# hyx1999/SAM-Decoding

Measured on AMD Instinct MI355X. Metric: tokens/sec (+ mean accepted tokens), Vicuna-7B bs=1, samd_sam_only draft+verify, higher is better.
Workload: dtype f16

## Files before the change

include/samd_hip.h:

```cpp
#ifndef SAMD_HIP_H
#define SAMD_HIP_H

#include <stdint.h>

#ifdef __cplusplus
extern "C" {
#endif

#define SAMD_OK 0
#define SAMD_E_INVALID (-1)
#define SAMD_E_CAPACITY (-2)
#define SAMD_E_HIP (-3)
#define SAMD_E_IO (-4)
#define SAMD_E_NODEVICE (-5)

#define SAMD_MAX_DRAFT 128
#define SAMD_TOPK 8

#define SAMD_REP_DMETA 0
#define SAMD_REP_VERDICT 16
#define SAMD_REP_TOKENS 24
#define SAMD_REP_KVINDEX 152
#define SAMD_REP_COUNTERS 280
#define SAMD_REP_META 288
// ... 123 lines not shown
int samd_report_wait(const int32_t *h_report, int32_t last_seq, int64_t timeout_us);

int samd_session_report_async(samd_session_t *s, int32_t *h_dst, void *stream);

int samd_session_device_views(samd_session_t *s, void *out[16]);

int samd_tree_buffers(const int32_t *d_parent, int32_t n, int32_t reverse_leaves, int32_t *d_position, uint64_t *d_mask,
                      uint8_t *d_mask_bool, int32_t *d_retrieve, int32_t *d_shape, void *stream);


int samd_argmax_rows(const void *d_logits, int32_t dtype, int32_t rows, int64_t vocab, int64_t row_stride,
                     const int32_t *d_rows, int32_t *d_out, void *stream);

int samd_session_accept(samd_session_t *s, const int32_t *d_node_argmax, void *stream);
int samd_session_candidates(samd_session_t *s, int64_t *d_candidates, int32_t *d_rowmap, int32_t capacity, void *stream);
int samd_session_step_given(samd_session_t *s, const samd_static_t *sam, const samd_params_t *p, const int32_t *d_best_accept,
                            const int32_t *d_next_token, void *stream);
int samd_session_read_verdict(samd_session_t *s, samd_verdict_host_t *out, void *stream);
int samd_session_commit(samd_session_t *s, const samd_static_t *sam, void *stream);
int samd_session_step(samd_session_t *s, const samd_static_t *sam, const samd_params_t *p,
                      const int32_t *d_node_argmax, void *stream);

int samd_posterior_sampled(const void *d_probs, int32_t dtype, const int64_t *d_candidates, int32_t n_candidates, int32_t depth, int64_t vocab,
                           const double *d_uniforms, int32_t n_uniforms, void *d_work, int32_t *d_out, void *stream);
int samd_posterior_sampled_nodes(const void *d_probs, int32_t dtype, const int32_t *d_rowmap, int32_t n_rows, const int64_t *d_candidates,
                                 int32_t n_candidates, int32_t depth, int64_t vocab, const double *d_uniforms, int32_t n_uniforms,
                                 void *d_work, int32_t *d_out, void *stream);
int samd_kv_compact(samd_session_t *s, void *const *d_tensors, int32_t n_tensors, int32_t n_heads, int64_t max_len,
                    int32_t head_dim, int32_t elem_bytes, void *stream);

int samd_kv_compact_indices(void *const *d_tensors, int32_t n_tensors, int32_t n_heads, int64_t max_len, int32_t head_dim,
                            int32_t elem_bytes, int32_t start, const int32_t *d_indices, int32_t accept, void *stream);

int samd_session_set_cache_length(samd_session_t *s, int32_t length, void *stream);
int samd_session_get_cache_length(samd_session_t *s, int32_t *h_out, void *stream);

typedef struct samd_warm {
    const void *d_packed_w;
    int32_t N, K, splits;
    int32_t kb_per_workgroup;
    int32_t delay;
    int32_t where;
} samd_warm_t;

int64_t samd_tree_attention_workspace(int32_t n_q_pad, int32_t n_heads, int32_t head_dim);
int samd_tree_attention(const void *d_q, const void *d_k_cache, const void *d_v_cache, void *d_out, int32_t dtype,
                        int32_t n_q_pad, int32_t n_heads, int32_t n_kv_heads, int32_t head_dim, int64_t max_len,
                        const uint64_t *d_mask, const int32_t *d_cache_length, const int32_t *d_n, float scale,
                        void *d_workspace, int64_t workspace_bytes, void *stream);
int samd_tree_attention_vt(const void *d_q, const void *d_k_cache, const void *d_vt_cache, void *d_out, int32_t dtype,
                           int32_t n_q_pad, int32_t n_heads, int32_t n_kv_heads, int32_t head_dim, int64_t max_len,
                           const uint64_t *d_mask, const int32_t *d_cache_length, const int32_t *d_n, float scale,
                           void *d_workspace, int64_t workspace_bytes, const samd_warm_t *next, void *stream);
int samd_tree_attention_warm(const void *d_q, const void *d_k_cache, const void *d_v_cache, void *d_out, int32_t dtype,
                             int32_t n_q_pad, int32_t n_heads, int32_t n_kv_heads, int32_t head_dim, int64_t max_len,
                             const uint64_t *d_mask, const int32_t *d_cache_length, const int32_t *d_n, float scale,
                             void *d_workspace, int64_t workspace_bytes, const samd_warm_t *next, void *stream);

int samd_rope_rows(const int32_t *d_rel_pos, const int32_t *d_base, const float *d_cos, const float *d_sin, float *d_cs, int32_t rows,
                   int32_t head_dim, int32_t max_pos, void *stream);
int samd_attention_block(const void *d_qkv, int32_t n_partials, int64_t partial_stride, const float *d_cs, void *d_k_cache, void *d_vt_cache,
                         void *d_out, int32_t dtype, int32_t n_q_pad, int32_t n_heads, int32_t n_kv_heads, int32_t head_dim, int64_t max_len,
                         const uint64_t *d_mask, const int32_t *d_write_pos, const int32_t *d_visible_len, const int32_t *d_n, float scale,
                         void *stream);
int samd_rope_kv_write_cs(const void *d_qkv, const int32_t *d_rel_pos, const int32_t *d_cache_length, const int32_t *d_n,
                          const float *d_cs, void *d_q_out, void *d_k_cache, void *d_v_cache, int32_t rows,
                          int32_t n_heads, int32_t n_kv_heads, int32_t head_dim, int64_t max_len, int32_t dtype,
                          int32_t n_partials, int64_t partial_stride, void *stream);
int samd_rope_kv_write_cs_vt(const void *d_qkv, const int32_t *d_rel_pos, const int32_t *d_cache_length, const int32_t *d_n,
                             const float *d_cs, void *d_q_out, void *d_k_cache, void *d_vt_cache, int32_t rows,
                             int32_t n_heads, int32_t n_kv_heads, int32_t head_dim, int64_t max_len, int32_t dtype,
                             int32_t n_partials, int64_t partial_stride, void *stream);
int64_t samd_tree_attention_rope_workspace(int32_t n_q_pad, int32_t n_heads, int32_t head_dim);
int samd_tree_attention_rope(const void *d_qkv, int32_t n_partials, int64_t partial_stride, const float *d_cs, void *d_k_cache, void *d_v_cache,
                             void *d_out, int32_t dtype, int32_t n_q_pad, int32_t n_heads, int32_t n_kv_heads, int32_t head_dim, int64_t max_len,
                             const uint64_t *d_mask, const int32_t *d_cache_length, const int32_t *d_n, float scale, void *d_workspace,
                             int64_t workspace_bytes, void *stream);
int samd_rope_kv_write_vt(const void *d_qkv, const int32_t *d_rel_pos, const int32_t *d_cache_length, const int32_t *d_n,
                          const float *d_cos, const float *d_sin, void *d_q_out, void *d_k_cache, void *d_vt_cache, int32_t rows,
                          int32_t n_heads, int32_t n_kv_heads, int32_t head_dim, int64_t max_len, int32_t max_pos, int32_t dtype,
                          int32_t n_partials, int64_t partial_stride, void *stream);
typedef struct samd_qkv_epilogue {
    const void *d_bias;
    const void *d_q_norm;
    const void *d_k_norm;
    float eps;
} samd_qkv_epilogue_t;
int samd_rope_kv_write_epi(const void *d_qkv, const int32_t *d_rel_pos, const int32_t *d_cache_length, const int32_t *d_n,
                           const float *d_cos, const float *d_sin, const float *d_cs, void *d_q_out, void *d_k_cache, void *d_v_cache,
                           int32_t v_transposed, int32_t rows, int32_t n_heads, int32_t n_kv_heads, int32_t head_dim, int64_t max_len,
                           int32_t max_pos, int32_t dtype, int32_t n_partials, int64_t partial_stride, const samd_qkv_epilogue_t *epi, void *stream);
int samd_kv_compact_vt(samd_session_t *s, void *const *d_tensors, int32_t n_tensors, int32_t n_transposed, int32_t n_heads, int64_t max_len,
                       int32_t head_dim, int32_t elem_bytes, void *stream);
int samd_kv_compact_indices_vt(void *const *d_tensors, int32_t n_tensors, int32_t n_transposed, int32_t n_heads, int64_t max_len, int32_t head_dim,
                               int32_t elem_bytes, int32_t start, const int32_t *d_indices, int32_t accept, void *stream);

typedef struct samd_e2_state {
    float *row_lse; float *top_logp; int32_t *top_idx; float *scores; int32_t *cs_index; float *all_scores; int32_t *all_tokens;
    int32_t *parents_list; uint64_t *mask_rows; int32_t *row_src; int32_t *ids;
    float *rec_top_vals; int32_t *rec_top_idx; float *rec_best_vals; int32_t *rec_best_idx; float *rec_final_vals; int32_t *rec_final_idx;
} samd_e2_state_t;
int64_t samd_e2_rowstats_workspace(int64_t vocab);
int samd_e2_rowstats(const void *d_logits, int32_t dtype, int32_t rows, int64_t vocab, int64_t row_stride, const samd_e2_state_t *st, void *d_workspace,
                     int64_t workspace_bytes, void *stream);
int samd_e2_select(const samd_e2_state_t *st, int32_t level, const void *d_hidden, const void *d_embed, int32_t hidden, int32_t vocab, void *d_fc_in,
                   int32_t *d_rel_pos , int32_t *d_L, int32_t *d_Lw , int32_t *d_n ,
                   int32_t advance_L, int32_t dtype, void *stream);
int samd_e2_stage_extend(const void *d_hidden_rows, const int32_t *d_kv_index, const int32_t *d_acc_tokens, const int32_t *d_start_token, int32_t n_accepted,
                         int32_t n_rows, const void *d_embed, int32_t hidden, int32_t vocab, void *d_fc_in, int32_t *d_rel_pos, uint64_t *d_mask_rows, int32_t *d_n,
                         int64_t *d_sample_token, int32_t dtype, void *stream);
int samd_e2_finish(const samd_e2_state_t *st, int32_t depth, int32_t keep, const int64_t *d_sample_token, int32_t *d_tokens, int32_t *d_parents, void *stream);
int samd_sum_partials_bias(const float *d_part, int32_t n_partials, int64_t partial_stride, const void *d_bias, void *d_out, int32_t rows, int32_t N,
                           int32_t dtype, void *stream);

int samd_embed_rows(const int32_t *d_tokens, const void *d_table, void *d_out, int32_t rows, int32_t hidden, int32_t vocab,
                    int32_t dtype, void *stream);
int samd_rmsnorm(void *d_x, const void *d_delta, const void *d_weight, void *d_out, int32_t rows, int32_t hidden, float eps,
                 int32_t dtype, int32_t n_partials, int64_t partial_stride, void *stream);
int samd_rmsnorm_warm(void *d_x, const void *d_delta, const void *d_weight, void *d_out, int32_t rows, int32_t hidden, float eps,
                      int32_t dtype, int32_t n_partials, int64_t partial_stride, const samd_warm_t *next, void *stream);
int samd_rope_kv_write(const void *d_qkv, const int32_t *d_rel_pos, const int32_t *d_cache_length, const int32_t *d_n,
                       const float *d_cos, const float *d_sin, void *d_q_out, void *d_k_cache, void *d_v_cache, int32_t rows,
                       int32_t n_heads, int32_t n_kv_heads, int32_t head_dim, int64_t max_len, int32_t max_pos, int32_t dtype,
                       int32_t n_partials, int64_t partial_stride, void *stream);
int samd_prefill_attention(const void *d_q, const void *d_k_cache, const void *d_v_cache, void *d_out, int32_t dtype, int32_t rows, int32_t pos0,
                           int32_t n_heads, int32_t n_kv_heads, int32_t head_dim, int64_t max_len, float scale, void *stream);
int samd_prefill_attention_vt(const void *d_q, const void *d_k_cache, const void *d_vt_cache, void *d_out, int32_t dtype, int32_t rows, int32_t pos0,
                              int32_t n_heads, int32_t n_kv_heads, int32_t head_dim, int64_t max_len, float scale, void *stream);
int samd_silu_mul(const void *d_gate_up, void *d_out, int32_t rows, int32_t inter, int32_t dtype, int32_t n_partials,
                  int64_t partial_stride, void *stream);

int samd_gemm_pack_weights(const void *d_W, void *d_packed, int32_t N, int32_t K, void *stream);
int samd_gemm_skinny_silu(const void *d_A, const void *d_W, int32_t rows_pad, int32_t N, int32_t K, void *d_out, int32_t dtype,
                          void *stream);
int samd_gemm_splits(int32_t N, int32_t K, int32_t rows_pad);
int64_t samd_gemm_workspace(int32_t rows_pad, int32_t N, int32_t splits);
int samd_gemm_pack_groups(const void *d_W, void *d_packed, int32_t N, int32_t K, void *stream);
int samd_gemm_pairs_silu(const void *d_A, const void *d_Wg, int32_t rows_pad, int32_t inter, int32_t K, void *d_out, int32_t dtype, void *stream);
int samd_gemm_pack_qkv64(const void *d_W, void *d_packed, int32_t n_heads_total, int32_t K, void *stream);
int samd_embed_rows_ssq_rope(const int32_t *d_tokens, const void *d_table, void *d_out, float *d_ssq, int32_t rows, int32_t hidden, int32_t vocab,
                             int32_t dtype, const int32_t *d_rel_pos, const int32_t *d_base, const float *d_cos, const float *d_sin, float *d_cs,
                             int32_t rope_rows, int32_t head_dim, int32_t max_pos, void *stream);
int samd_embed_rows_ssq(const int32_t *d_tokens, const void *d_table, void *d_out, float *d_ssq, int32_t rows, int32_t hidden, int32_t vocab,
                        int32_t dtype, void *stream);
int samd_gemm_qkv_rope_norm(const void *d_x, const float *d_ssq, const void *d_norm_weight, float eps, const void *d_W64, int32_t rows_pad, int32_t K,
                            const float *d_cs, const int32_t *d_cache_length, const int32_t *d_n, void *d_q_out, void *d_k_cache, void *d_v_cache,
                            int32_t n_heads, int32_t n_kv_heads, int32_t head_dim, int64_t max_len, int32_t dtype, void *stream);
int samd_gemm_pairs_silu_norm(const void *d_x, const float *d_ssq, const void *d_norm_weight, float eps, const void *d_Wg, int32_t rows_pad, int32_t inter,
                              int32_t K, void *d_out, int32_t dtype, void *stream);
int samd_gemm_cs_residual(const void *d_A, const void *d_Wg, int32_t rows_pad, int32_t N, int32_t K, void *d_x, float *d_ssq, int32_t dtype, void *stream);
int samd_gemm_qkv_rope(const void *d_A, const void *d_W64, int32_t rows_pad, int32_t K, const float *d_cs, const int32_t *d_cache_length,
                       const int32_t *d_n, void *d_q_out, void *d_k_cache, void *d_v_cache, int32_t n_heads, int32_t n_kv_heads,
                       int32_t head_dim, int64_t max_len, int32_t dtype, void *stream);
int samd_gemm_qkv_rope_norm_vt(const void *d_x, const float *d_ssq, const void *d_norm_weight, float eps, const void *d_W64, int32_t rows_pad, int32_t K,
                               const float *d_cs, const int32_t *d_cache_length, const int32_t *d_n, void *d_q_out, void *d_k_cache, void *d_vt_cache,
                               int32_t n_heads, int32_t n_kv_heads, int32_t head_dim, int64_t max_len, int32_t dtype, void *stream);
int samd_gemm_qkv_rope_vt(const void *d_A, const void *d_W64, int32_t rows_pad, int32_t K, const float *d_cs, const int32_t *d_cache_length,
                          const int32_t *d_n, void *d_q_out, void *d_k_cache, void *d_vt_cache, int32_t n_heads, int32_t n_kv_heads,
                          int32_t head_dim, int64_t max_len, int32_t dtype, void *stream);
int samd_gemm_skinny(const void *d_A, const void *d_W, int32_t rows_pad, int32_t N, int32_t K, int32_t splits, float *d_partial,
                     void *d_out, int32_t dtype, void *stream);
int samd_gemm_skinny_groups(const void *d_A, const void *d_Wg, int32_t rows_pad, int32_t N, int32_t K, int32_t splits, float *d_partial,
                            void *d_out, int32_t dtype, void *stream);
int samd_gemm_pack_f8(const void *d_W8, void *d_out, int32_t N, int32_t K, void *stream);
int samd_gemm_skinny_f8(const void *d_A, const void *d_W8p, const float *d_scale, int32_t rows_pad, int32_t N, int32_t K, int32_t splits,
                        float *d_partial, void *d_out, int32_t dtype, void *stream);
int samd_gemm_pack_f4(const void *d_q, const void *d_e8, void *d_out, int32_t N, int32_t K, void *stream);
int samd_gemm_skinny_f4(const void *d_A, const void *d_W4p, int32_t rows_pad, int32_t N, int32_t K, int32_t splits, float *d_partial, void *d_out,
                        int32_t dtype, void *stream);
int32_t samd_moe_workspace_layout(int32_t field);
int64_t samd_moe_workspace(int32_t rows_pad, int32_t hidden, int32_t n_experts, int32_t top_k, int32_t dtype);
int samd_moe_pack_experts(const void *d_W, void *d_packed, int32_t n_experts, int32_t N, int32_t K, int32_t gate_up, void *stream);
int samd_moe_route(const void *d_h, const void *d_router, const int32_t *d_n, int32_t rows_pad, int32_t hidden, int32_t n_experts, int32_t top_k,
                   int32_t norm_topk, int32_t *d_topk_idx, void *d_topk_w, void *d_ws, int32_t dtype, void *stream);
int samd_moe_lists(const int32_t *d_topk_idx, const int32_t *d_n, int32_t rows_pad, int32_t n_experts, int32_t top_k, void *d_ws, void *stream);
int samd_moe_gate_up_silu(const void *d_h, const void *d_Wgu, const void *d_ws, int32_t rows_pad, int32_t hidden, int32_t moe_inter, int32_t n_experts,
                          int32_t top_k, void *d_act, int32_t dtype, void *stream);
int samd_moe_down_combine(const void *d_act, const void *d_Wdown, const int32_t *d_topk_idx, const void *d_topk_w, const int32_t *d_n, void *d_ws,
                          int32_t rows_pad, int32_t hidden, int32_t moe_inter, int32_t n_experts, int32_t top_k, void *d_out, int32_t dtype, void *stream);
int samd_moe_gate_up_silu_f4(const void *d_h, const void *d_Wgu4, const void *d_ws, int32_t rows_pad, int32_t hidden, int32_t moe_inter, int32_t n_experts,
                             int32_t top_k, void *d_act, int32_t dtype, void *stream);
int samd_moe_down_combine_f4(const void *d_act, const void *d_Wdown4, const int32_t *d_topk_idx, const void *d_topk_w, const int32_t *d_n, void *d_ws,
                             int32_t rows_pad, int32_t hidden, int32_t moe_inter, int32_t n_experts, int32_t top_k, void *d_out, int32_t dtype, void *stream);

int samd_scripted_argmax(samd_session_t *s, const int32_t *d_target, int32_t n_target, int32_t vocab, int32_t *d_out,
                         void *stream);

int samd_scripted_logits(samd_session_t *s, const int32_t *d_argmax, void *d_logits, int32_t dtype, int32_t rows, int64_t row_stride,
                         int32_t markov_vocab, void *stream);
int samd_scripted_logits_order1(samd_session_t *s, const int32_t *d_argmax, void *d_logits, int32_t dtype, int32_t rows, int64_t row_stride,
                                int32_t hot_vocab, void *stream);

int samd_recycle_create(int32_t vocab, const int32_t *h_child_offsets, const int32_t *h_children, int32_t n_nodes,
                        samd_recycle_t **out);
void samd_recycle_free(samd_recycle_t *t);
int samd_recycle_update(samd_recycle_t *t, const int32_t *d_tokens, const void *d_logits, int32_t dtype, int32_t n,
                        const int32_t *d_n, int64_t vocab, int64_t row_stride, void *stream);
int samd_recycle_draft(samd_recycle_t *t, const int32_t *d_start_token, int32_t *d_out, void *stream);
int samd_recycle_export(samd_recycle_t *t, int32_t *h_table, uint8_t *h_present, void *stream);

#ifdef __cplusplus
}
#endif
#endif
```

sam-decoding_amd/csrc/gemm_kernels.hip:

```cpp
#include <hip/hip_runtime.h>
#include <cstdlib>
#include "samd_common.h"

#define LAUNCHCHK() do { hipError_t e_ = hipGetLastError(); if (e_ != hipSuccess) { samd_set_error("kernel launch: %s", hipGetErrorString(e_)); return SAMD_E_HIP; } } while (0)

static int samd_cu_count() { return samd_device_cus(); }

typedef _Float16 half8 __attribute__((ext_vector_type(8)));
typedef __bf16 bf16x8 __attribute__((ext_vector_type(8)));
typedef float floatx4 __attribute__((ext_vector_type(4)));
typedef unsigned u32x4 __attribute__((ext_vector_type(4)));

struct GF16 { typedef _Float16 elem; typedef half8 vec8;
    static __device__ __forceinline__ floatx4 mfma(half8 a, half8 b, floatx4 c) { return __builtin_amdgcn_mfma_f32_16x16x32_f16(a, b, c, 0, 0, 0); } };
struct GBF16 { typedef __bf16 elem; typedef bf16x8 vec8;
    static __device__ __forceinline__ floatx4 mfma(bf16x8 a, bf16x8 b, floatx4 c) { return __builtin_amdgcn_mfma_f32_16x16x32_bf16(a, b, c, 0, 0, 0); } };

#define GEMM_KC 256
#define GEMM_WAVES 8
#define GEMM_COLS (16 * GEMM_WAVES)

typedef __attribute__((address_space(1))) const void *gptr_t;
typedef __attribute__((address_space(3))) void *lptr_t;

// ... 54 lines not shown
        if (DEPTH > 2 && younger_in_flight >= 2) asm volatile("s_waitcnt vmcnt(%0)" : : "n"(2 * (8 + XV)) : "memory");
        else if (younger_in_flight >= 1) asm volatile("s_waitcnt vmcnt(%0)" : : "n"(8 + XV) : "memory");
        else asm volatile("s_waitcnt vmcnt(0)" : : : "memory");
        __builtin_amdgcn_s_barrier();
        asm volatile("" ::: "memory");
    };
    auto phase = [&](u32x4 (&cur)[4][2], int c, int buf) {
        landed(c1 - 1 - c);
        const uint32_t xbase = lds_base + (uint32_t)buf * (R * GEMM_KC * 2) + (uint32_t)n * (GEMM_KC * 2);
#pragma unroll
        for (int b = 0; b < 4; b++) {
            const uint32_t u0 = (uint32_t)((8 * b + 2 * g) ^ n) * 16, u1 = (uint32_t)((8 * b + 2 * g + 1) ^ n) * 16;
            const uint32_t a0 = xbase + u0, a1 = xbase + u1;
            u32x4 r[RT][2];
            if constexpr (RT == 1)
                asm volatile("ds_read_b128 %0, %2\n\tds_read_b128 %1, %3\n\ts_waitcnt lgkmcnt(0)" : "=&v"(r[0][0]), "=&v"(r[0][1]) : "v"(a0), "v"(a1));
            else if constexpr (RT == 2)
                asm volatile("ds_read_b128 %0, %4\n\tds_read_b128 %1, %5\n\tds_read_b128 %2, %4 offset:8192\n\tds_read_b128 %3, %5 offset:8192\n\t"
                             "s_waitcnt lgkmcnt(0)" : "=&v"(r[0][0]), "=&v"(r[0][1]), "=&v"(r[1][0]), "=&v"(r[1][1]) : "v"(a0), "v"(a1));
            else if constexpr (RT == 3)
                asm volatile("ds_read_b128 %0, %6\n\tds_read_b128 %1, %7\n\tds_read_b128 %2, %6 offset:8192\n\tds_read_b128 %3, %7 offset:8192\n\t"
                             "ds_read_b128 %4, %6 offset:16384\n\tds_read_b128 %5, %7 offset:16384\n\ts_waitcnt lgkmcnt(0)"
                             : "=&v"(r[0][0]), "=&v"(r[0][1]), "=&v"(r[1][0]), "=&v"(r[1][1]), "=&v"(r[2][0]), "=&v"(r[2][1]) : "v"(a0), "v"(a1));
            else
                asm volatile("ds_read_b128 %0, %8\n\tds_read_b128 %1, %9\n\tds_read_b128 %2, %8 offset:8192\n\tds_read_b128 %3, %9 offset:8192\n\t"
                             "ds_read_b128 %4, %8 offset:16384\n\tds_read_b128 %5, %9 offset:16384\n\tds_read_b128 %6, %8 offset:24576\n\t"
                             "ds_read_b128 %7, %9 offset:24576\n\ts_waitcnt lgkmcnt(0)"
                             : "=&v"(r[0][0]), "=&v"(r[0][1]), "=&v"(r[1][0]), "=&v"(r[1][1]), "=&v"(r[2][0]), "=&v"(r[2][1]), "=&v"(r[3][0]), "=&v"(r[3][1])
                             : "v"(a0), "v"(a1));
#pragma unroll
            for (int mt = 0; mt < RT; mt++) {
                acc[mt] = TT::mfma(__builtin_bit_cast(V8, r[mt][0]), __builtin_bit_cast(V8, cur[b][0]), acc[mt]);
                acc[mt] = TT::mfma(__builtin_bit_cast(V8, r[mt][1]), __builtin_bit_cast(V8, cur[b][1]), acc[mt]);
            }
            if (RT >= 3 && c + DEPTH < c1) {
                load_wb(cur, c + DEPTH, b);
                if (b < XV) stage_xi(c + DEPTH, buf == 0 ? NB - 1 : buf - 1, b);
            }
        }
        if (RT < 3 && c + DEPTH < c1) { load_w(cur, c + DEPTH); stage_x(c + DEPTH, buf == 0 ? NB - 1 : buf - 1); }
    };
    if (c0 < c1) {
#pragma unroll
        for (int d = 0; d < DEPTH; d++)
            if (c0 + d < c1) { load_w(wr[d], c0 + d); stage_x(c0 + d, d); }
        int buf = 0;
        for (int c = c0; c < c1; c += DEPTH) {
#pragma unroll
            for (int d = 0; d < DEPTH; d++)
                if (c + d < c1) { phase(wr[d], c + d, buf); buf = buf == NB - 1 ? 0 : buf + 1; }
        }
    }
    if constexpr (EPI == 1) {
        float *ex = reinterpret_cast<float *>(gemm_lds);
        __syncthreads();
        if (w >= 4) {
#pragma unroll
            for (int mt = 0; mt < RT; mt++)
#pragma unroll
                for (int r = 0; r < 4; r++) ex[(16 * mt + 4 * g + r) * 64 + 16 * (w - 4) + n] = acc[mt][r];
        }
        __syncthreads();
        if (w < 4) {
#pragma unroll
            for (int mt = 0; mt < RT; mt++)
#pragma unroll
                for (int r = 0; r < 4; r++) {
                    const int m = 16 * mt + 4 * g + r;
                    const float gf = (float)(E)acc[mt][r], uf = (float)(E)ex[m * 64 + 16 * w + n];
                    const E sv = (E)(gf / (1.f + __expf(-gf)));
                    out[(size_t)m * (N / 2) + blockIdx.x * 64 + 16 * w + n] = (E)((float)sv * uf);
                }
        }
        return;
    }
#pragma unroll
    for (int mt = 0; mt < RT; mt++) {
#pragma unroll
        for (int r = 0; r < 4; r++) {
            const int m = 16 * mt + 4 * g + r;
            if (out) out[(size_t)m * N + n0 + n] = (E)acc[mt][r];
            else __hip_atomic_store(&partial[((size_t)split * R + m) * N + n0 + n], acc[mt][r], __ATOMIC_RELAXED, __HIP_MEMORY_SCOPE_AGENT);
        }
    }
}

struct NormArgs { const float *ssq; const void *g; int tiles; float inv_hidden; float eps; };

#define NORM_NS 16
template <int NT>
__device__ __forceinline__ void norm_issue(const NormArgs &na, float (&sv)[NORM_NS]) {
    const int tid = threadIdx.x, row = tid & 15, p = tid >> 4;
#pragma unroll
    for (int k = 0; k < NORM_NS; k++) {
        sv[k] = 0.f;
        if ((NT / 16) * k >= na.tiles) continue;
        int t = p + (NT / 16) * k;
        t = t < na.tiles ? t : na.tiles - 1;
        const float *src = na.ssq + (size_t)t * 16 + row;
        asm volatile("global_load_dword %0, %1, off" : "=v"(sv[k]) : "v"(src) : "memory");
    }
}
template <int NT>
__device__ __forceinline__ void norm_finish(const NormArgs &na, float (&sv)[NORM_NS], float *part , float *rs ) {
    const int tid = threadIdx.x, row = tid & 15, p = tid >> 4;
    static_assert(NORM_NS == 16, "");
    asm volatile("" : "+v"(sv[0]), "+v"(sv[1]), "+v"(sv[2]), "+v"(sv[3]), "+v"(sv[4]), "+v"(sv[5]), "+v"(sv[6]), "+v"(sv[7]),
                      "+v"(sv[8]), "+v"(sv[9]), "+v"(sv[10]), "+v"(sv[11]), "+v"(sv[12]), "+v"(sv[13]), "+v"(sv[14]), "+v"(sv[15]) : : "memory");
    float s = 0.f;
#pragma unroll
    for (int k = 0; k < NORM_NS; k++) s += (p + (NT / 16) * k < na.tiles) ? sv[k] : 0.f;
    part[p * 16 + row] = s;
    asm volatile("s_waitcnt lgkmcnt(0)" ::: "memory");
    __builtin_amdgcn_s_barrier();
    asm volatile("" ::: "memory");
    if (tid < 16) {
        float tot = 0.f;
        for (int k = 0; k < NT / 16; k++) tot += part[k * 16 + tid];
        rs[tid] = rsqrtf(tot * na.inv_hidden + na.eps);
    }
    asm volatile("s_waitcnt lgkmcnt(0)" ::: "memory");
    __builtin_amdgcn_s_barrier();
    asm volatile("" ::: "memory");
}

template <typename E>
__device__ __forceinline__ u32x4 norm_scale8(u32x4 xraw, u32x4 graw, float rs) {
    const E *xe = reinterpret_cast<const E *>(&xraw);
    const E *ge = reinterpret_cast<const E *>(&graw);
    u32x4 out;
    E *oe = reinterpret_cast<E *>(&out);
#pragma unroll
    for (int j = 0; j < 8; j++) { const E h = (E)((float)xe[j] * rs); oe[j] = (E)((float)ge[j] * (float)h); }
    return out;
}


template <int DEPTH, int PC>
__device__ __forceinline__ void gemm_wait_younger(int younger) {
    if constexpr (PC == 0) asm volatile("s_waitcnt vmcnt(0)" : : : "memory");
    else {
        if (DEPTH > 3 && younger >= 3) asm volatile("s_waitcnt vmcnt(%0)" : : "n"(3 * PC) : "memory");
        else if (DEPTH > 2 && younger >= 2) asm volatile("s_waitcnt vmcnt(%0)" : : "n"(2 * PC) : "memory");
        else if (younger >= 1) asm volatile("s_waitcnt vmcnt(%0)" : : "n"(PC) : "memory");
        else asm volatile("s_waitcnt vmcnt(0)" : : : "memory");
    }
}

template <typename TT, int RT, int DEPTH, int CG, bool NORM, int AR = 16>
__global__ __launch_bounds__(64 * GEMM_WAVES, RT >= 3 || NORM ? 2 : GEMM_WAVES / 2) void k_gemm_qkv_rope(
        const typename TT::elem *__restrict__ A, const typename TT::elem *__restrict__ W, int K, int n_chunks,
        const float *__restrict__ cs, const int *__restrict__ d_L, const int *__restrict__ d_n,
        typename TT::elem *__restrict__ q_out, typename TT::elem *__restrict__ k_cache, typename TT::elem *__restrict__ v_cache,
        int H, int Hkv, long long max_len, NormArgs na, int v_t) {
    typedef typename TT::elem E;
    typedef typename TT::vec8 V8;
    constexpr int R = 16 * RT;
    constexpr int NT = 64 * GEMM_WAVES;
    constexpr int XV = (R * 32) / NT;
    constexpr int NB = DEPTH + 1;
    constexpr int WL = 4;
    constexpr int TW = 16 * CG, PP = 8 * CG;
    constexpr int CH = CG * 8192;
    extern __shared__ __attribute__((aligned(1024))) char gemm_lds[];
    E (*xs)[R][GEMM_KC] = reinterpret_cast<E (*)[R][GEMM_KC]>(gemm_lds);

    const int tid = threadIdx.x, w = tid >> 6, l = tid & 63, n = l & 15, g = l >> 4;
    const bool streams = CG == 4 || w < 2 * CG;
    static_assert(AR == 16 || (AR == 8 && NORM && RT == 1), "8 activation rows: the norm-fold kernels only");
    const bool stager = AR == 16 || w < GEMM_WAVES / 2;
    const int cg = CG == 4 ? (w & 3) : (streams ? w % CG : 0), kh = CG == 4 ? (w >> 2) : (streams ? w / CG : 0);
    const char *wtile = reinterpret_cast<const char *>(W) + (size_t)blockIdx.x * n_chunks * CH;
    const uint32_t wlane = (uint32_t)(64 * (CG * kh + cg) + l) * 16;
    const uint32_t lds_base = (uint32_t)(uintptr_t)(lptr_t)&xs[0][0][0];
    const int n_rows = d_n[0], L = d_L[0];

    floatx4 acc[RT];
#pragma unroll
    for (int mt = 0; mt < RT; mt++) acc[mt] = (floatx4){0.f, 0.f, 0.f, 0.f};

    u32x4 wr[DEPTH][2][2];
    auto load_wb = [&](u32x4 (&dst)[2][2], int c, int bl) {
        const char *p = wtile + (size_t)c * CH;
#pragma unroll
        for (int j = 0; j < 2; j++)
            asm volatile("global_load_dwordx4 %0, %1, %2 nt" : "=v"(dst[bl][j]) : "v"(wlane), "s"(p + (CH / 4) * (2 * bl + j)) : "memory");
    };
    static_assert(!NORM || RT == 1, "the norm-fold path is built for the 16-row tile");
    constexpr int XL = NORM ? 2 * XV : XV;
    u32x4 xr[NORM ? DEPTH : 1][NORM ? XV : 1], gr[NORM ? DEPTH : 1][NORM ? XV : 1];
    __shared__ float norm_part[NORM ? (NT / 16) * 16 : 1], norm_rs[NORM ? 16 : 1];
    auto stage_xi = [&](int c, int buf, int i, int d) {
        const int slot = tid + NT * i, row = slot >> 5, pos = slot & 31, unit = pos ^ (row & 15);
        const E *src = A + (size_t)row * K + (size_t)c * GEMM_KC + 8 * unit;
        if constexpr (NORM) {
            const E *gsrc = reinterpret_cast<const E *>(na.g) + (size_t)c * GEMM_KC + 8 * unit;
            asm volatile("global_load_dwordx4 %0, %1, off" : "=v"(xr[d][i]) : "v"(src) : "memory");
            asm volatile("global_load_dwordx4 %0, %1, off" : "=v"(gr[d][i]) : "v"(gsrc) : "memory");
        } else {
            E *dst = &xs[buf][0][0] + (size_t)(NT * i + 64 * w) * 8;
            __builtin_amdgcn_global_load_lds((gptr_t)src, (lptr_t)dst, 16, 0, 0);
            asm volatile("" ::: "memory");
        }
    };
    auto issue = [&](u32x4 (&dst)[2][2], int c, int buf, int d) {
        if (streams) { load_wb(dst, c, 0); load_wb(dst, c, 1); }
        if (stager) {
#pragma unroll
            for (int i = 0; i < XV; i++) stage_xi(c, buf, i, d);
        }
    };
    auto scale_to_lds = [&](int buf, int d) {
        if constexpr (NORM) {
            if (!stager) return;
#pragma unroll
            for (int i = 0; i < XV; i++) {
                const int slot = tid + NT * i, row = slot >> 5;
                asm volatile("" : "+v"(xr[d][i]), "+v"(gr[d][i]) : : "memory");
                const u32x4 v = norm_scale8<E>(xr[d][i], gr[d][i], norm_rs[row]);
                *reinterpret_cast<u32x4 *>(&xs[buf][0][0] + (size_t)slot * 8) = v;
            }
        }
    };
    auto landed = [&](int younger, int buf, int d) {
        if (streams) { if (stager) gemm_wait_younger<DEPTH, WL + XL>(younger); else gemm_wait_younger<DEPTH, WL>(younger); }
        else { if (stager) gemm_wait_younger<DEPTH, XL>(younger); else gemm_wait_younger<DEPTH, 0>(younger); }
        if constexpr (NORM) { scale_to_lds(buf, d); asm volatile("s_waitcnt lgkmcnt(0)" ::: "memory"); }
        __builtin_amdgcn_s_barrier();
        asm volatile("" ::: "memory");
    };
    auto phase = [&](u32x4 (&cur)[2][2], int c, int buf, int d) {
        landed(n_chunks - 1 - c, buf, d);
        const uint32_t xbase = lds_base + (uint32_t)buf * (R * GEMM_KC * 2) + (uint32_t)n * (GEMM_KC * 2);
#pragma unroll
        for (int bl = 0; bl < 2; bl++) {
            if (!streams) break;
            const int b = 2 * kh + bl;
            const uint32_t a0 = xbase + (uint32_t)((8 * b + 2 * g) ^ n) * 16, a1 = xbase + (uint32_t)((8 * b + 2 * g + 1) ^ n) * 16;
            u32x4 r[RT][2];
            if constexpr (RT == 1)
                asm volatile("ds_read_b128 %0, %2\n\tds_read_b128 %1, %3\n\ts_waitcnt lgkmcnt(0)" : "=&v"(r[0][0]), "=&v"(r[0][1]) : "v"(a0), "v"(a1));
            else if constexpr (RT == 2)
                asm volatile("ds_read_b128 %0, %4\n\tds_read_b128 %1, %5\n\tds_read_b128 %2, %4 offset:8192\n\tds_read_b128 %3, %5 offset:8192\n\t"
                             "s_waitcnt lgkmcnt(0)" : "=&v"(r[0][0]), "=&v"(r[0][1]), "=&v"(r[1][0]), "=&v"(r[1][1]) : "v"(a0), "v"(a1));
            else if constexpr (RT == 3)
                asm volatile("ds_read_b128 %0, %6\n\tds_read_b128 %1, %7\n\tds_read_b128 %2, %6 offset:8192\n\tds_read_b128 %3, %7 offset:8192\n\t"
                             "ds_read_b128 %4, %6 offset:16384\n\tds_read_b128 %5, %7 offset:16384\n\ts_waitcnt lgkmcnt(0)"
                             : "=&v"(r[0][0]), "=&v"(r[0][1]), "=&v"(r[1][0]), "=&v"(r[1][1]), "=&v"(r[2][0]), "=&v"(r[2][1]) : "v"(a0), "v"(a1));
            else
                asm volatile("ds_read_b128 %0, %8\n\tds_read_b128 %1, %9\n\tds_read_b128 %2, %8 offset:8192\n\tds_read_b128 %3, %9 offset:8192\n\t"
                             "ds_read_b128 %4, %8 offset:16384\n\tds_read_b128 %5, %9 offset:16384\n\tds_read_b128 %6, %8 offset:24576\n\t"
                             "ds_read_b128 %7, %9 offset:24576\n\ts_waitcnt lgkmcnt(0)"
                             : "=&v"(r[0][0]), "=&v"(r[0][1]), "=&v"(r[1][0]), "=&v"(r[1][1]), "=&v"(r[2][0]), "=&v"(r[2][1]), "=&v"(r[3][0]), "=&v"(r[3][1])
                             : "v"(a0), "v"(a1));
#pragma unroll
            for (int mt = 0; mt < RT; mt++) {
                acc[mt] = TT::mfma(__builtin_bit_cast(V8, r[mt][0]), __builtin_bit_cast(V8, cur[bl][0]), acc[mt]);
                acc[mt] = TT::mfma(__builtin_bit_cast(V8, r[mt][1]), __builtin_bit_cast(V8, cur[bl][1]), acc[mt]);
            }
        }
        if (c + DEPTH < n_chunks) issue(cur, c + DEPTH, buf == 0 ? NB - 1 : buf - 1, d);
    };
    float norm_sv[NORM ? NORM_NS : 1];
    if constexpr (NORM) norm_issue<NT>(na, norm_sv);
#pragma unroll
    for (int d = 0; d < DEPTH; d++)
        if (d < n_chunks) issue(wr[d], d, d, d);
    if constexpr (AR == 8) {
        if (!stager) {
#pragma unroll
            for (int bz = 0; bz < NB; bz++) *reinterpret_cast<u32x4 *>(&xs[bz][0][0] + (size_t)tid * 8) = (u32x4){0u, 0u, 0u, 0u};
        }
    }
    if constexpr (NORM) {
        if (n_chunks >= DEPTH) {
            if (streams) { if (stager) asm volatile("s_waitcnt vmcnt(%0)" : : "n"(DEPTH * (WL + XL)) : "memory"); else asm volatile("s_waitcnt vmcnt(%0)" : : "n"(DEPTH * WL) : "memory"); }
            else { if (stager) asm volatile("s_waitcnt vmcnt(%0)" : : "n"(DEPTH * XL) : "memory"); else asm volatile("s_waitcnt vmcnt(0)" : : : "memory"); }
        } else asm volatile("s_waitcnt vmcnt(0)" : : : "memory");
        norm_finish<NT>(na, norm_sv, norm_part, norm_rs);
    }
    {
        int buf = 0;
        for (int c = 0; c < n_chunks; c += DEPTH) {
#pragma unroll
            for (int d = 0; d < DEPTH; d++)
                if (c + d < n_chunks) { phase(wr[d], c + d, buf, d); buf = buf == NB - 1 ? 0 : buf + 1; }
        }
    }
    float *ex = reinterpret_cast<float *>(gemm_lds);
    __syncthreads();
    if (streams) {
#pragma unroll
        for (int mt = 0; mt < RT; mt++)
#pragma unroll
            for (int r = 0; r < 4; r++) ex[(kh * R + 16 * mt + 4 * g + r) * TW + 16 * cg + n] = acc[mt][r];
    }
    __syncthreads();
    const bool vt_tile = v_t && ((PP * (int)blockIdx.x) >> 6) >= H + Hkv;
    for (int i = tid; i < R * PP; i += NT) {
        const int row = vt_tile ? i % R : i / PP, p = vt_tile ? i / R : i % PP;
        if (row >= n_rows || L + row >= max_len) continue;
        const float x1 = (float)(E)(ex[row * TW + p] + ex[(R + row) * TW + p]);
        const float x2 = (float)(E)(ex[row * TW + PP + p] + ex[(R + row) * TW + PP + p]);
        const int pair = PP * (int)blockIdx.x + p, head = pair >> 6, j = pair & 63;
        if (head >= H + Hkv) {
            if (v_t) {
                E *dst = v_cache + (size_t)(head - H - Hkv) * max_len * 128 + L + row;
                dst[(size_t)j * max_len] = (E)x1; dst[(size_t)(j + 64) * max_len] = (E)x2;
                continue;
            }
            E *dst = v_cache + ((size_t)(head - H - Hkv) * max_len + L + row) * 128;
            dst[j] = (E)x1; dst[j + 64] = (E)x2;
            continue;
        }
        const float c = cs[(size_t)row * 128 + j], sn = cs[(size_t)row * 128 + 64 + j];
        const E o1 = (E)(x1 * c - x2 * sn), o2 = (E)(x2 * c + x1 * sn);
        E *dst = head < H ? q_out + ((size_t)row * H + head) * 128 : k_cache + ((size_t)(head - H) * max_len + L + row) * 128;
        dst[j] = o1; dst[j + 64] = o2;
    }
}

template <int CG>
__global__ __launch_bounds__(256) void k_gemm_pack_qkv(const uint4 *__restrict__ W, uint4 *__restrict__ out, int N, int K) {
    const long long u = (long long)blockIdx.x * 256 + threadIdx.x;
    const long long total = (long long)N * K / 8;
    if (u >= total) return;
    constexpr int PP = 8 * CG;
    const int n_chunks = K / GEMM_KC;
    const long long blk = u / (512 * CG);
    const int in = (int)(u % (512 * CG)), jj = in / (128 * CG), x = in % (128 * CG), w = x >> 6, g = (x >> 4) & 3, n = x & 15, cg = w % CG, kh = w / CG;
    const int t = (int)(blk / n_chunks), c = (int)(blk % n_chunks), bl = jj >> 1, j = jj & 1;
    const int q = 16 * cg + n, pair = PP * t + (q < PP ? q : q - PP);
    const long long row = 128LL * (pair >> 6) + (pair & 63) + (q < PP ? 0 : 64), col = 256LL * c + 64 * (2 * kh + bl) + 16 * g + 8 * j;
    out[u] = W[(row * K + col) / 8];
}

static int qkv_tile_groups(int n_heads_total) {
    static const int env = [] { const char *e = getenv("SAMD_QKV_TILE"); return e ? atoi(e) : 0; }();
    const int n_cu = samd_cu_count();
    const int N = n_heads_total * 128;
    if (N % 48 != 0 || env == 64) return 4;
    if (env == 48) return 3;
    const int t48 = N / 48, t64 = N / 64;
    return ((t48 + n_cu - 1) / n_cu) * 48 < ((t64 + n_cu - 1) / n_cu) * 64 ? 3 : 4;
}

template <typename TT, int RT, int DEPTH, bool NORM, int AR = 16>
__global__ __launch_bounds__(64 * GEMM_WAVES, RT >= 3 || DEPTH > 2 ? 2 : GEMM_WAVES / 2) void k_gemm_pairs_silu(const typename TT::elem *__restrict__ A, const typename TT::elem *__restrict__ W,
                                                                                                     typename TT::elem *__restrict__ out, int K, int inter, int n_chunks, int n_pairs, NormArgs na) {
    typedef typename TT::elem E;
    typedef typename TT::vec8 V8;
    constexpr int R = 16 * RT;
    constexpr int NT = 64 * GEMM_WAVES;
    constexpr int XV = (R * 32) / NT;
    constexpr int NB = DEPTH + 1;
    extern __shared__ __attribute__((aligned(1024))) char gemm_lds[];
    E (*xs)[R][GEMM_KC] = reinterpret_cast<E (*)[R][GEMM_KC]>(gemm_lds);

    const int tid = threadIdx.x, w = __builtin_amdgcn_readfirstlane(tid >> 6), l = tid & 63, n = l & 15, g = l >> 4;
#ifdef SAMD_GEMM_ABLATE
    const int abl = samd_abl_flag;
#else
    constexpr int abl = 0;
#endif
    const int p0 = (int)((long long)blockIdx.x * n_pairs / gridDim.x), p1 = (int)((long long)(blockIdx.x + 1) * n_pairs / gridDim.x);
    const bool active = w < 2 * (p1 - p0);
    static_assert(AR == 16 || (AR == 8 && NORM && RT == 1), "8 activation rows: the norm-fold kernels only");
    const bool stager = AR == 16 || w < GEMM_WAVES / 2;
    const int gi = 2 * p0 + w;
    const char *wgrp = reinterpret_cast<const char *>(W) + (size_t)(active ? gi : 0) * n_chunks * 8192;
    const uint32_t wlane = (uint32_t)l * 16;
    const uint32_t lds_base = (uint32_t)(uintptr_t)(lptr_t)&xs[0][0][0];

    floatx4 acc[RT];
#pragma unroll
    for (int mt = 0; mt < RT; mt++) acc[mt] = (floatx4){0.f, 0.f, 0.f, 0.f};
    u32x4 wr[DEPTH][4][2];
    auto load_w = [&](u32x4 (&dst)[4][2], int c) {
        const char *p = wgrp + (size_t)c * 8192;
#pragma unroll
        for (int b = 0; b < 4; b++)
#pragma unroll
            for (int j = 0; j < 2; j++)
                asm volatile("global_load_dwordx4 %0, %1, %2 nt" : "=v"(dst[b][j]) : "v"(wlane), "s"(p + 1024 * (2 * b + j)) : "memory");
    };
    static_assert(!NORM || RT == 1, "the norm-fold path is built for the 16-row tile");
    constexpr int XL = NORM ? 2 * XV : XV;
    u32x4 xr[NORM ? DEPTH : 1][NORM ? XV : 1], gr[NORM ? DEPTH : 1][NORM ? XV : 1];
    __shared__ float norm_part[NORM ? (NT / 16) * 16 : 1], norm_rs[NORM ? 16 : 1];
    auto stage_x = [&](int c, int buf, int d) {
        if (!stager || (abl & 4)) return;
#pragma unroll
        for (int i = 0; i < XV; i++) {
            const int slot = tid + NT * i, row = slot >> 5, pos = slot & 31, unit = pos ^ (row & 15);
            const E *src = A + (size_t)((abl & 8) ? (row & 15) : row) * K + (size_t)c * GEMM_KC + 8 * unit;
            if constexpr (NORM) {
                const E *gsrc = reinterpret_cast<const E *>(na.g) + (size_t)c * GEMM_KC + 8 * unit;
                asm volatile("global_load_dwordx4 %0, %1, off" : "=v"(xr[d][i]) : "v"(src) : "memory");
                asm volatile("global_load_dwordx4 %0, %1, off" : "=v"(gr[d][i]) : "v"(gsrc) : "memory");
            } else {
                E *dst = &xs[buf][0][0] + (size_t)(NT * i + 64 * w) * 8;
                __builtin_amdgcn_global_load_lds((gptr_t)src, (lptr_t)dst, 16, 0, 0);
                asm volatile("" ::: "memory");
            }
        }
    };
    auto landed = [&](int younger, int buf, int d) {
        const bool stg = stager && !(abl & 4);
        if (active) { if (stg) gemm_wait_younger<DEPTH, 8 + XL>(younger); else gemm_wait_younger<DEPTH, 8>(younger); }
        else { if (stg) gemm_wait_younger<DEPTH, XL>(younger); else gemm_wait_younger<DEPTH, 0>(younger); }
        if constexpr (NORM) {
            if (stager) {
#pragma unroll
                for (int i = 0; i < XV; i++) {
                    const int slot = tid + NT * i, row = slot >> 5;
                    asm volatile("" : "+v"(xr[d][i]), "+v"(gr[d][i]) : : "memory");
                    const u32x4 v = norm_scale8<E>(xr[d][i], gr[d][i], norm_rs[row]);
                    *reinterpret_cast<u32x4 *>(&xs[buf][0][0] + (size_t)slot * 8) = v;
                }
            }
            asm volatile("s_waitcnt lgkmcnt(0)" ::: "memory");
        }
        if (!(abl & 1)) __builtin_amdgcn_s_barrier();
        asm volatile("" ::: "memory");
    };
    auto phase = [&](u32x4 (&cur)[4][2], int c, int buf, int d) {
        landed(n_chunks - 1 - c, buf, d);
        if (active && !(abl & 2)) {
            const uint32_t xbase = lds_base + (uint32_t)buf * (R * GEMM_KC * 2) + (uint32_t)n * (GEMM_KC * 2);
#pragma unroll
            for (int b = 0; b < 4; b++) {
                const uint32_t a0 = xbase + (uint32_t)((8 * b + 2 * g) ^ n) * 16, a1 = xbase + (uint32_t)((8 * b + 2 * g + 1) ^ n) * 16;
                u32x4 r[RT][2];
                if constexpr (RT == 1)
                    asm volatile("ds_read_b128 %0, %2\n\tds_read_b128 %1, %3\n\ts_waitcnt lgkmcnt(0)" : "=&v"(r[0][0]), "=&v"(r[0][1]) : "v"(a0), "v"(a1));
                else if constexpr (RT == 2)
                    asm volatile("ds_read_b128 %0, %4\n\tds_read_b128 %1, %5\n\tds_read_b128 %2, %4 offset:8192\n\tds_read_b128 %3, %5 offset:8192\n\t"
                                 "s_waitcnt lgkmcnt(0)" : "=&v"(r[0][0]), "=&v"(r[0][1]), "=&v"(r[1][0]), "=&v"(r[1][1]) : "v"(a0), "v"(a1));
                else if constexpr (RT == 3)
                    asm volatile("ds_read_b128 %0, %6\n\tds_read_b128 %1, %7\n\tds_read_b128 %2, %6 offset:8192\n\tds_read_b128 %3, %7 offset:8192\n\t"
                                 "ds_read_b128 %4, %6 offset:16384\n\tds_read_b128 %5, %7 offset:16384\n\ts_waitcnt lgkmcnt(0)"
                                 : "=&v"(r[0][0]), "=&v"(r[0][1]), "=&v"(r[1][0]), "=&v"(r[1][1]), "=&v"(r[2][0]), "=&v"(r[2][1]) : "v"(a0), "v"(a1));
                else
                    asm volatile("ds_read_b128 %0, %8\n\tds_read_b128 %1, %9\n\tds_read_b128 %2, %8 offset:8192\n\tds_read_b128 %3, %9 offset:8192\n\t"
                                 "ds_read_b128 %4, %8 offset:16384\n\tds_read_b128 %5, %9 offset:16384\n\tds_read_b128 %6, %8 offset:24576\n\t"
                                 "ds_read_b128 %7, %9 offset:24576\n\ts_waitcnt lgkmcnt(0)"
                                 : "=&v"(r[0][0]), "=&v"(r[0][1]), "=&v"(r[1][0]), "=&v"(r[1][1]), "=&v"(r[2][0]), "=&v"(r[2][1]), "=&v"(r[3][0]), "=&v"(r[3][1])
                                 : "v"(a0), "v"(a1));
#pragma unroll
                for (int mt = 0; mt < RT; mt++) {
                    acc[mt] = TT::mfma(__builtin_bit_cast(V8, r[mt][0]), __builtin_bit_cast(V8, cur[b][0]), acc[mt]);
                    acc[mt] = TT::mfma(__builtin_bit_cast(V8, r[mt][1]), __builtin_bit_cast(V8, cur[b][1]), acc[mt]);
                }
            }
        }
        if (c + DEPTH < n_chunks) { if (active) load_w(cur, c + DEPTH); stage_x(c + DEPTH, buf == 0 ? NB - 1 : buf - 1, d); }
    };
    float norm_sv[NORM ? NORM_NS : 1];
    if constexpr (NORM) norm_issue<NT>(na, norm_sv);
#pragma unroll
    for (int d = 0; d < DEPTH; d++)
        if (d < n_chunks) { if (active) load_w(wr[d], d); stage_x(d, d, d); }
    if constexpr (AR == 8) {
        if (!stager) {
#pragma unroll
            for (int bz = 0; bz < NB; bz++) *reinterpret_cast<u32x4 *>(&xs[bz][0][0] + (size_t)tid * 8) = (u32x4){0u, 0u, 0u, 0u};
        }
    }
    if constexpr (NORM) {
        if (n_chunks >= DEPTH) {
            if (active) { if (stager) asm volatile("s_waitcnt vmcnt(%0)" : : "n"(DEPTH * (8 + XL)) : "memory"); else asm volatile("s_waitcnt vmcnt(%0)" : : "n"(DEPTH * 8) : "memory"); }
            else { if (stager) asm volatile("s_waitcnt vmcnt(%0)" : : "n"(DEPTH * XL) : "memory"); else asm volatile("s_waitcnt vmcnt(0)" : : : "memory"); }
        } else asm volatile("s_waitcnt vmcnt(0)" : : : "memory");
        norm_finish<NT>(na, norm_sv, norm_part, norm_rs);
    }
    {
        int buf = 0;
        for (int c = 0; c < n_chunks; c += DEPTH) {
#pragma unroll
            for (int d = 0; d < DEPTH; d++)
                if (c + d < n_chunks) { phase(wr[d], c + d, buf, d); buf = buf == NB - 1 ? 0 : buf + 1; }
        }
    }
    float *ex = reinterpret_cast<float *>(gemm_lds);
    __syncthreads();
    if (active && (w & 1)) {
#pragma unroll
        for (int mt = 0; mt < RT; mt++)
#pragma unroll
            for (int r = 0; r < 4; r++) ex[((w >> 1) * R + 16 * mt + 4 * g + r) * 16 + n] = acc[mt][r];
    }
    __syncthreads();
    if (active && !(w & 1)) {
        const int col = 16 * (p0 + (w >> 1)) + n;
#pragma unroll
        for (int mt = 0; mt < RT; mt++)
#pragma unroll
            for (int r = 0; r < 4; r++) {
                const int m = 16 * mt + 4 * g + r;
                const float gf = (float)(E)acc[mt][r], uf = (float)(E)ex[((w >> 1) * R + m) * 16 + n];
                const E sv = (E)(gf / (1.f + __expf(-gf)));
                out[(size_t)m * inter + col] = (E)((float)sv * uf);
            }
    }
}

template <typename TT, int ROWS, bool EARLY = false>
__global__ __launch_bounds__(64 * GEMM_WAVES, 2) void k_gemm_cs_residual(const typename TT::elem *__restrict__ A, const typename TT::elem *__restrict__ W,
                                                                           typename TT::elem *__restrict__ x, float *__restrict__ ssq, int K, int N, int n_chunks,
                                                                           const int *__restrict__ counter = nullptr, int *__restrict__ epoch = nullptr,
                                                                           int arrivals = 0) {
    typedef typename TT::elem E;
    typedef typename TT::vec8 V8;
    constexpr int CSD = 2;
    extern __shared__ __attribute__((aligned(1024))) char gemm_lds[];
    const int tid = threadIdx.x, w = __builtin_amdgcn_readfirstlane(tid >> 6), l = tid & 63, n = l & 15, g = l >> 4;
    E *xs = reinterpret_cast<E *>(gemm_lds) + (size_t)w * CSD * 16 * GEMM_KC;
    const uint32_t lds_base = (uint32_t)(uintptr_t)(lptr_t)xs;
    const char *wgrp = reinterpret_cast<const char *>(W) + (size_t)blockIdx.x * n_chunks * 8192;
    const uint32_t wlane = (uint32_t)l * 16;

    static_assert(ROWS == 8 || ROWS == 16, "");
    constexpr int AL = ROWS / 2;
    if constexpr (ROWS == 8) {
#pragma unroll
        for (int buf = 0; buf < CSD; buf++)
#pragma unroll
            for (int i = 4; i < 8; i++)
                *reinterpret_cast<u32x4 *>(xs + (size_t)buf * 16 * GEMM_KC + (size_t)(64 * i + l) * 8) = (u32x4){0u, 0u, 0u, 0u};
        asm volatile("s_waitcnt lgkmcnt(0)" ::: "memory");
    }
    floatx4 acc = (floatx4){0.f, 0.f, 0.f, 0.f};
    u32x4 wr[CSD][4][2];
    auto issue_w = [&](u32x4 (&dst)[4][2], int c) {
        const char *p = wgrp + (size_t)c * 8192;
#pragma unroll
        for (int b = 0; b < 4; b++)
#pragma unroll
            for (int j = 0; j < 2; j++)
                asm volatile("global_load_dwordx4 %0, %1, %2 nt" : "=v"(dst[b][j]) : "v"(wlane), "s"(p + 1024 * (2 * b + j)) : "memory");
    };
    auto issue_a = [&](int c, int buf) {
#pragma unroll
        for (int i = 0; i < AL; i++) {
            const int slot = l + 64 * i, row = slot >> 5, pos = slot & 31, unit = pos ^ (row & 15);
            const E *src = A + (size_t)row * K + (size_t)c * GEMM_KC + 8 * unit;
            E *dst_l = xs + (size_t)buf * 16 * GEMM_KC + (size_t)(64 * i) * 8;
            __builtin_amdgcn_global_load_lds((gptr_t)src, (lptr_t)dst_l, 16, 0, 0);
            asm volatile("" ::: "memory");
        }
    };
    auto issue = [&](u32x4 (&dst)[4][2], int c, int buf) { issue_w(dst, c); issue_a(c, buf); };
    auto phase = [&](u32x4 (&cur)[4][2], int c, int buf, bool more) {
        if (more) { if constexpr (EARLY) asm volatile("s_waitcnt vmcnt(%0)" : : "n"(AL) : "memory"); else asm volatile("s_waitcnt vmcnt(%0)" : : "n"(8 + AL) : "memory"); }
        else asm volatile("s_waitcnt vmcnt(0)" ::: "memory");
        const uint32_t xbase = lds_base + (uint32_t)buf * (16 * GEMM_KC * 2) + (uint32_t)n * (GEMM_KC * 2);
#pragma unroll
        for (int b = 0; b < 4; b++) {
            const uint32_t a0 = xbase + (uint32_t)((8 * b + 2 * g) ^ n) * 16, a1 = xbase + (uint32_t)((8 * b + 2 * g + 1) ^ n) * 16;
            u32x4 r0, r1;
            asm volatile("ds_read_b128 %0, %2\n\tds_read_b128 %1, %3\n\ts_waitcnt lgkmcnt(0)" : "=&v"(r0), "=&v"(r1) : "v"(a0), "v"(a1));
            acc = TT::mfma(__builtin_bit_cast(V8, r0), __builtin_bit_cast(V8, cur[b][0]), acc);
            acc = TT::mfma(__builtin_bit_cast(V8, r1), __builtin_bit_cast(V8, cur[b][1]), acc);
        }
    };
    const int mine = (n_chunks - w + GEMM_WAVES - 1) / GEMM_WAVES;
    if constexpr (EARLY) {
        if (mine > 0) issue_w(wr[0], w);
        if (mine > 1) issue_w(wr[1], w + GEMM_WAVES);
        __shared__ int my_epoch;
        if (tid == 0) {
            const int e = epoch[blockIdx.x];
            const int target = (e + 1) * arrivals;
            for (int spin = 0; spin < (1 << 22); spin++) {
                if (__hip_atomic_load(counter, __ATOMIC_RELAXED, __HIP_MEMORY_SCOPE_AGENT) >= target) break;
                __builtin_amdgcn_s_sleep(4);
            }
            my_epoch = e;
        }
        __syncthreads();
        __builtin_amdgcn_fence(__ATOMIC_ACQUIRE, "agent");
        if (mine > 0) issue_a(w, 0);
        if (mine > 1) issue_a(w + GEMM_WAVES, 1);
        if (mine > 0) phase(wr[0], w, 0, mine > 1);
        if (mine > 1) phase(wr[1], w + GEMM_WAVES, 1, false);
        if (tid == 0) epoch[blockIdx.x] = my_epoch + 1;
    } else {
        if (mine > 0) issue(wr[0], w, 0);
        if (mine > 1) issue(wr[1], w + GEMM_WAVES, 1);
        for (int i = 0; i < mine; i += 2) {
            phase(wr[0], w + GEMM_WAVES * i, 0, i + 1 < mine);
            if (i + 2 < mine) issue(wr[0], w + GEMM_WAVES * (i + 2), 0);
            if (i + 1 < mine) {
                phase(wr[1], w + GEMM_WAVES * (i + 1), 1, i + 2 < mine);
                if (i + 3 < mine) issue(wr[1], w + GEMM_WAVES * (i + 3), 1);
            }
        }
    }
    __syncthreads();
    float *ex = reinterpret_cast<float *>(gemm_lds);
#pragma unroll
    for (int r = 0; r < 4; r++) ex[(w * 16 + 4 * g + r) * 16 + n] = acc[r];
    __syncthreads();
    if (tid < 16 * ROWS) {
        const int row = tid >> 4, col = tid & 15;
        float sum = 0.f;
#pragma unroll
        for (int k = 0; k < GEMM_WAVES; k++) sum += ex[(k * 16 + row) * 16 + col];
        E *xp = x + (size_t)row * N + 16 * blockIdx.x + col;
        const E o = (E)sum;
        const E y = (E)((float)*xp + (float)o);
        *xp = y;
        float q = (float)y * (float)y;
        q += __shfl_xor(q, 1); q += __shfl_xor(q, 2); q += __shfl_xor(q, 4); q += __shfl_xor(q, 8);
        if (col == 0) ssq[(size_t)blockIdx.x * 16 + row] = q;
    }
}

__global__ __launch_bounds__(256) void k_gemm_pack_groups(const uint4 *__restrict__ W, uint4 *__restrict__ out, int N, int K) {
    const long long u = (long long)blockIdx.x * 256 + threadIdx.x;
    const long long total = (long long)N * K / 8;
    if (u >= total) return;
    const int n_chunks = K / GEMM_KC;
    const long long blk = u >> 9;
    const int in = (int)(u & 511), jj = in >> 6, lane = in & 63, g = lane >> 4, n = lane & 15, b = jj >> 1, j = jj & 1;
    const long long gi = blk / n_chunks; const int c = (int)(blk % n_chunks);
    const long long row = 16 * gi + n, col = 256LL * c + 64 * b + 16 * g + 8 * j;
    out[u] = W[(row * K + col) / 8];
}

__global__ __launch_bounds__(256) void k_gemm_pack(const uint4 *__restrict__ W, uint4 *__restrict__ out, int N, int K) {
    const long long u = (long long)blockIdx.x * 256 + threadIdx.x;
    const long long total = (long long)N * K / 8;
    if (u >= total) return;
    const int n_chunks = K / GEMM_KC;
    const long long blk = u >> 12;
    const int in = (int)(u & 4095), jj = in >> 9, tid = in & 511, w = tid >> 6, g = (tid >> 4) & 3, n = tid & 15;
    const int t = (int)(blk / n_chunks), c = (int)(blk % n_chunks), b = jj >> 1, j = jj & 1;
    const long long row = 128LL * t + 16 * w + n, col = 256LL * c + 64 * b + 16 * g + 8 * j;
    out[u] = W[(row * K + col) / 8];
}

template <typename TT, int RT, int EPI, int DEPTH, bool GM = false>
static hipError_t gemm_launch(dim3 grid, hipStream_t st, const void *A, const void *W, float *partial, void *out, int K, int N, int chunks, int splits) {
    constexpr int lds = (DEPTH + 1) * 16 * RT * GEMM_KC * 2;
    if constexpr (lds > 65536) {
        static unsigned long long done = 0ull;
        const hipError_t attr = samd_reserve_lds((const void *)k_gemm_skinny<TT, RT, EPI, DEPTH, GM>, lds, &done);
        if (attr != hipSuccess) return attr;
    }
    hipLaunchKernelGGL((k_gemm_skinny<TT, RT, EPI, DEPTH, GM>), grid, dim3(64 * GEMM_WAVES), lds, st, (const typename TT::elem *)A, (const typename TT::elem *)W, partial,
                       (typename TT::elem *)out, K, N, chunks, splits);
    return hipSuccess;
}

template <int EPI, bool GM = false>
static hipError_t gemm_dispatch(int dtype, int rows_pad, dim3 grid, hipStream_t st, const void *A, const void *W, float *partial, void *out, int K, int N, int chunks,
                                int splits) {
#define GO(TT, RT, D) return gemm_launch<TT, RT, EPI, D, GM>(grid, st, A, W, partial, out, K, N, chunks, splits)
#define ROWS(TT) do { if (rows_pad == 16) GO(TT, 1, 2); else if (rows_pad == 32) GO(TT, 2, 2); else if (rows_pad == 48) GO(TT, 3, 2); else GO(TT, 4, 2); } while (0)
    if (dtype == SAMD_F16) ROWS(GF16); else ROWS(GBF16);
#undef ROWS
#undef GO
}

template <typename TT, int RT, int DEPTH, int CG, bool NORM = false, int AR = 16>
static hipError_t qkv_rope_launch(hipStream_t st, const void *A, const void *W, int K, int tiles, const float *cs, const int *d_L, const int *d_n, void *q, void *k, void *v,
                                  int H, int Hkv, long long max_len, int v_t, NormArgs na = NormArgs{nullptr, nullptr, 0, 0.f, 0.f}) {
    constexpr int lds_a = (DEPTH + 1) * 16 * RT * GEMM_KC * 2, lds_e = 2 * 16 * RT * 16 * CG * 4, lds = lds_a > lds_e ? lds_a : lds_e;
    if constexpr (lds > 60000) {
        static unsigned long long done = 0ull;
        const hipError_t attr = samd_reserve_lds((const void *)k_gemm_qkv_rope<TT, RT, DEPTH, CG, NORM, AR>, lds + 4096, &done);
        if (attr != hipSuccess) return attr;
    }
    hipLaunchKernelGGL((k_gemm_qkv_rope<TT, RT, DEPTH, CG, NORM, AR>), dim3(tiles), dim3(64 * GEMM_WAVES), lds, st, (const typename TT::elem *)A, (const typename TT::elem *)W, K, K / GEMM_KC,
                       cs, d_L, d_n, (typename TT::elem *)q, (typename TT::elem *)k, (typename TT::elem *)v, H, Hkv, max_len, na, v_t);
    return hipSuccess;
}

template <typename TT, int RT, int DEPTH, bool NORM = false, int AR = 16>
static hipError_t pairs_silu_launch(hipStream_t st, int grid, const void *A, const void *W, void *out, int K, int inter, int n_pairs,
                                    NormArgs na = NormArgs{nullptr, nullptr, 0, 0.f, 0.f}) {
    constexpr int lds_a = (DEPTH + 1) * 16 * RT * GEMM_KC * 2, lds_e = 4 * 16 * RT * 16 * 4, lds = lds_a > lds_e ? lds_a : lds_e;
    if constexpr (lds > 60000) {
        static unsigned long long done = 0ull;
        const hipError_t attr = samd_reserve_lds((const void *)k_gemm_pairs_silu<TT, RT, DEPTH, NORM, AR>, lds + 4096, &done);
        if (attr != hipSuccess) return attr;
    }
    hipLaunchKernelGGL((k_gemm_pairs_silu<TT, RT, DEPTH, NORM, AR>), dim3(grid), dim3(64 * GEMM_WAVES), lds, st, (const typename TT::elem *)A, (const typename TT::elem *)W,
                       (typename TT::elem *)out, K, inter, K / GEMM_KC, n_pairs, na);
    return hipSuccess;
}

extern "C" {

int samd_gemm_splits(int32_t N, int32_t K, int32_t rows_pad) {
    static const int env_cap = [] { const char *e = getenv("SAMD_GEMM_SPLIT_CAP"); const int v = e ? atoi(e) : 8; return v < 1 ? 1 : (v > 8 ? 8 : v); }();
    static const int env_fixed = [] { const char *e = getenv("SAMD_GEMM_SPLITS"); const int v = e ? atoi(e) : 0; return v < 0 ? 0 : (v > 8 ? 8 : v); }();
    const int cols = N / GEMM_COLS, chunks = K / GEMM_KC;
    (void)rows_pad;
    if (env_fixed) return env_fixed > chunks ? (chunks < 1 ? 1 : chunks) : env_fixed;
    int s = 256 / (cols > 0 ? cols : 1);
    if (s > env_cap) s = env_cap;
    if (s > chunks) s = chunks;
    return s < 1 ? 1 : s;
}

int64_t samd_gemm_workspace(int32_t rows_pad, int32_t N, int32_t splits) { return (int64_t)splits * rows_pad * N * 4; }

int samd_gemm_skinny_silu(const void *d_A, const void *d_W, int32_t rows_pad, int32_t N, int32_t K, void *d_out, int32_t dtype, void *stream) {
    if (!d_A || !d_W || !d_out || (rows_pad != 16 && rows_pad != 32 && rows_pad != 48 && rows_pad != 64) || N < GEMM_COLS || N % GEMM_COLS != 0 || K < GEMM_KC ||
        K % GEMM_KC != 0 || (dtype != SAMD_F16 && dtype != SAMD_BF16)) {
        samd_set_error("samd_gemm_skinny_silu: unsupported shape (rows 16/32/48/64, N %% 128 == 0, K %% 256 == 0) or null pointer"); return SAMD_E_INVALID;
    }
    const hipError_t e = gemm_dispatch<1>(dtype, rows_pad, dim3(N / GEMM_COLS, 1), (hipStream_t)stream, d_A, d_W, nullptr, d_out, K, N, K / GEMM_KC, 1);
    if (e != hipSuccess) { samd_set_error("samd_gemm_skinny_silu: %s", hipGetErrorString(e)); return SAMD_E_HIP; }
    LAUNCHCHK();
    return SAMD_OK;
}

int samd_gemm_pack_weights(const void *d_W, void *d_packed, int32_t N, int32_t K, void *stream) {
    if (!d_W || !d_packed || d_W == d_packed || N < GEMM_COLS || N % GEMM_COLS != 0 || K < GEMM_KC || K % GEMM_KC != 0) {
        samd_set_error("samd_gemm_pack_weights: needs N %% 128 == 0, K %% 256 == 0 and distinct buffers"); return SAMD_E_INVALID;
    }
    const long long units = (long long)N * K / 8;
    hipLaunchKernelGGL(k_gemm_pack, dim3((unsigned)((units + 255) / 256)), dim3(256), 0, (hipStream_t)stream, (const uint4 *)d_W, (uint4 *)d_packed, N, K);
    LAUNCHCHK();
    return SAMD_OK;
}

int samd_gemm_pack_groups(const void *d_W, void *d_packed, int32_t N, int32_t K, void *stream) {
    if (!d_W || !d_packed || d_W == d_packed || N < 16 || N % 16 != 0 || K < GEMM_KC || K % GEMM_KC != 0) {
        samd_set_error("samd_gemm_pack_groups: needs N %% 16 == 0, K %% 256 == 0 and distinct buffers"); return SAMD_E_INVALID;
    }
    const long long units = (long long)N * K / 8;
    hipLaunchKernelGGL(k_gemm_pack_groups, dim3((unsigned)((units + 255) / 256)), dim3(256), 0, (hipStream_t)stream, (const uint4 *)d_W, (uint4 *)d_packed, N, K);
    LAUNCHCHK();
    return SAMD_OK;
}

int samd_gemm_pairs_silu_norm(const void *d_x, const float *d_ssq, const void *d_norm_weight, float eps, const void *d_Wg, int32_t rows_pad, int32_t inter, int32_t K,
                              void *d_out, int32_t dtype, void *stream) {
    if (!d_x || !d_ssq || !d_norm_weight || !d_Wg || !d_out || (rows_pad != 16 && rows_pad != 8) || inter < 16 || inter % 16 != 0 || K < GEMM_KC || K % GEMM_KC != 0 ||
        K / 16 > 32 * NORM_NS || (dtype != SAMD_F16 && dtype != SAMD_BF16)) {
        samd_set_error("samd_gemm_pairs_silu_norm: unsupported shape (8 or 16 rows, inter %% 16 == 0, K %% 256 == 0, K <= 8192, f16/bf16) or null pointer"); return SAMD_E_INVALID;
    }
    const int n_cu = samd_cu_count();
    const int n_pairs = inter / 16;
    int grid = n_pairs < n_cu ? n_pairs : n_cu;
    while ((n_pairs + grid - 1) / grid > 4) grid += n_cu;
    const NormArgs na{d_ssq, d_norm_weight, K / 16, 1.f / (float)K, eps};
    hipStream_t st = (hipStream_t)stream;
    const hipError_t e = rows_pad == 8
        ? (dtype == SAMD_F16 ? pairs_silu_launch<GF16, 1, 3, true, 8>(st, grid, d_x, d_Wg, d_out, K, inter, n_pairs, na)
                             : pairs_silu_launch<GBF16, 1, 3, true, 8>(st, grid, d_x, d_Wg, d_out, K, inter, n_pairs, na))
        : (dtype == SAMD_F16 ? pairs_silu_launch<GF16, 1, 3, true>(st, grid, d_x, d_Wg, d_out, K, inter, n_pairs, na)
                             : pairs_silu_launch<GBF16, 1, 3, true>(st, grid, d_x, d_Wg, d_out, K, inter, n_pairs, na));
    if (e != hipSuccess) { samd_set_error("samd_gemm_pairs_silu_norm: %s", hipGetErrorString(e)); return SAMD_E_HIP; }
    LAUNCHCHK();
    return SAMD_OK;
}

int samd_gemm_cs_residual(const void *d_A, const void *d_Wg, int32_t rows_pad, int32_t N, int32_t K, void *d_x, float *d_ssq, int32_t dtype, void *stream) {
    if (!d_A || !d_Wg || !d_x || !d_ssq || (rows_pad != 16 && rows_pad != 8) || N < 16 || N % 16 != 0 || K < GEMM_KC || K % GEMM_KC != 0 || (dtype != SAMD_F16 && dtype != SAMD_BF16)) {
        samd_set_error("samd_gemm_cs_residual: unsupported shape (8 or 16 rows, N %% 16 == 0, K %% 256 == 0, f16/bf16) or null pointer"); return SAMD_E_INVALID;
    }
    constexpr int lds = GEMM_WAVES * 2 * 16 * GEMM_KC * 2;
    hipStream_t st = (hipStream_t)stream;
    hipError_t e = hipSuccess;
#define GO(TT, ROWS, ET) do { static unsigned long long done = 0ull; \
        e = samd_reserve_lds((const void *)k_gemm_cs_residual<TT, ROWS>, lds, &done); \
        if (e == hipSuccess) hipLaunchKernelGGL((k_gemm_cs_residual<TT, ROWS>), dim3(N / 16), dim3(64 * GEMM_WAVES), lds, st, (const ET *)d_A, (const ET *)d_Wg, (ET *)d_x, d_ssq, K, N, K / GEMM_KC, (const int *)nullptr, (int *)nullptr, 0); } while (0)
    if (dtype == SAMD_F16) { if (rows_pad == 8) GO(GF16, 8, _Float16); else GO(GF16, 16, _Float16); }
    else { if (rows_pad == 8) GO(GBF16, 8, __bf16); else GO(GBF16, 16, __bf16); }
#undef GO
    if (e != hipSuccess) { samd_set_error("samd_gemm_cs_residual: %s", hipGetErrorString(e)); return SAMD_E_HIP; }
    LAUNCHCHK();
    return SAMD_OK;
}

int samd_gemm_cs_residual_early(const void *d_A, const void *d_Wg, int32_t N, int32_t K, void *d_x, float *d_ssq, int32_t dtype, const int32_t *d_counter,
                                int32_t *d_epoch, int32_t arrivals, void *stream) {
    if (!d_A || !d_Wg || !d_x || !d_ssq || !d_counter || !d_epoch || arrivals < 1 || N < 16 || N % 16 != 0 || K != 2 * GEMM_WAVES * GEMM_KC ||
        (dtype != SAMD_F16 && dtype != SAMD_BF16)) {
        samd_set_error("samd_gemm_cs_residual_early: unsupported shape (K must be 4096, N %% 16 == 0, f16/bf16) or null pointer"); return SAMD_E_INVALID;
    }
    constexpr int lds = GEMM_WAVES * 2 * 16 * GEMM_KC * 2;
    hipStream_t st = (hipStream_t)stream;
    hipError_t e = hipSuccess;
    if (dtype == SAMD_F16) {
        static unsigned long long done = 0ull;
        e = samd_reserve_lds((const void *)k_gemm_cs_residual<GF16, 8, true>, lds, &done);
        if (e == hipSuccess) hipLaunchKernelGGL((k_gemm_cs_residual<GF16, 8, true>), dim3(N / 16), dim3(64 * GEMM_WAVES), lds, st, (const _Float16 *)d_A, (const _Float16 *)d_Wg,
                                                (_Float16 *)d_x, d_ssq, K, N, K / GEMM_KC, d_counter, d_epoch, arrivals);
    } else {
        static unsigned long long done = 0ull;
        e = samd_reserve_lds((const void *)k_gemm_cs_residual<GBF16, 8, true>, lds, &done);
        if (e == hipSuccess) hipLaunchKernelGGL((k_gemm_cs_residual<GBF16, 8, true>), dim3(N / 16), dim3(64 * GEMM_WAVES), lds, st, (const __bf16 *)d_A, (const __bf16 *)d_Wg,
                                                (__bf16 *)d_x, d_ssq, K, N, K / GEMM_KC, d_counter, d_epoch, arrivals);
    }
    if (e != hipSuccess) { samd_set_error("samd_gemm_cs_residual_early: %s", hipGetErrorString(e)); return SAMD_E_HIP; }
    LAUNCHCHK();
    return SAMD_OK;
}

int samd_gemm_pairs_silu(const void *d_A, const void *d_Wg, int32_t rows_pad, int32_t inter, int32_t K, void *d_out, int32_t dtype, void *stream) {
    if (!d_A || !d_Wg || !d_out || (rows_pad != 16 && rows_pad != 32 && rows_pad != 48 && rows_pad != 64) || inter < 16 || inter % 16 != 0 || K < GEMM_KC ||
        K % GEMM_KC != 0 || (dtype != SAMD_F16 && dtype != SAMD_BF16)) {
        samd_set_error("samd_gemm_pairs_silu: unsupported shape (rows 16/32/48/64, inter %% 16 == 0, K %% 256 == 0, f16/bf16) or null pointer"); return SAMD_E_INVALID;
    }
    const int n_cu = samd_cu_count();
    const int n_pairs = inter / 16;
    int grid = n_pairs < n_cu ? n_pairs : n_cu;
    while ((n_pairs + grid - 1) / grid > 4) grid += n_cu;
    hipStream_t st = (hipStream_t)stream;
    hipError_t e;
    static const int depth_env = [] { const char *e = getenv("SAMD_PAIRS_DEPTH"); return e ? atoi(e) : 0; }();
#ifdef SAMD_GEMM_ABLATE
    static const int abl_set = [] { const char *e = getenv("SAMD_GEMM_ABL"); const int v = e ? atoi(e) : 0; return hipMemcpyToSymbol(HIP_SYMBOL(samd_abl_flag), &v, 4) == hipSuccess ? 1 : -1; }();
    (void)abl_set;
#endif
#define ARGS st, grid, d_A, d_Wg, d_out, K, inter, n_pairs
#define GO(TT) (rows_pad == 16 ? (depth_env == 2 ? pairs_silu_launch<TT, 1, 2>(ARGS) : depth_env == 4 ? pairs_silu_launch<TT, 1, 4>(ARGS) : pairs_silu_launch<TT, 1, 3>(ARGS)) \
                : rows_pad == 32 ? (depth_env == 2 ? pairs_silu_launch<TT, 2, 2>(ARGS) : pairs_silu_launch<TT, 2, 3>(ARGS)) \
                : rows_pad == 48 ? pairs_silu_launch<TT, 3, 2>(ARGS) : pairs_silu_launch<TT, 4, 2>(ARGS))
    e = dtype == SAMD_F16 ? GO(GF16) : GO(GBF16);
#undef GO
#undef ARGS
    if (e != hipSuccess) { samd_set_error("samd_gemm_pairs_silu: %s", hipGetErrorString(e)); return SAMD_E_HIP; }
    LAUNCHCHK();
    return SAMD_OK;
}

int samd_gemm_pack_qkv64(const void *d_W, void *d_packed, int32_t n_heads_total, int32_t K, void *stream) {
    if (!d_W || !d_packed || d_W == d_packed || n_heads_total < 1 || K < GEMM_KC || K % GEMM_KC != 0) {
        samd_set_error("samd_gemm_pack_qkv64: needs K %% 256 == 0, whole 128-column heads and distinct buffers"); return SAMD_E_INVALID;
    }
    const long long units = (long long)n_heads_total * 128 * K / 8;
    if (qkv_tile_groups(n_heads_total) == 3)
        hipLaunchKernelGGL(k_gemm_pack_qkv<3>, dim3((unsigned)((units + 255) / 256)), dim3(256), 0, (hipStream_t)stream, (const uint4 *)d_W, (uint4 *)d_packed, n_heads_total * 128, K);
    else
        hipLaunchKernelGGL(k_gemm_pack_qkv<4>, dim3((unsigned)((units + 255) / 256)), dim3(256), 0, (hipStream_t)stream, (const uint4 *)d_W, (uint4 *)d_packed, n_heads_total * 128, K);
    LAUNCHCHK();
    return SAMD_OK;
}

static int gemm_qkv_rope_impl(const void *d_A, const void *d_W64, int32_t rows_pad, int32_t K, const float *d_cs, const int32_t *d_cache_length, const int32_t *d_n,
                              void *d_q_out, void *d_k_cache, void *d_v_cache, int32_t n_heads, int32_t n_kv_heads, int32_t head_dim, int64_t max_len,
                              int32_t dtype, void *stream, int v_t) {
    if (!d_A || !d_W64 || !d_cs || !d_cache_length || !d_n || !d_q_out || !d_k_cache || !d_v_cache || head_dim != 128 || n_heads < 1 || n_kv_heads < 1 ||
        (rows_pad != 16 && rows_pad != 32 && rows_pad != 48 && rows_pad != 64) || K < GEMM_KC || K % GEMM_KC != 0 || (dtype != SAMD_F16 && dtype != SAMD_BF16)) {
        samd_set_error("samd_gemm_qkv_rope: unsupported shape (rows 16/32/48/64, head_dim 128, K %% 256 == 0, f16/bf16) or null pointer"); return SAMD_E_INVALID;
    }
    static const int depth_env = [] { const char *e = getenv("SAMD_QKV_DEPTH"); return e ? atoi(e) : 0; }();
    const int groups = qkv_tile_groups(n_heads + 2 * n_kv_heads);
    const int tiles = (n_heads + 2 * n_kv_heads) * 128 / (16 * groups);
    hipStream_t st = (hipStream_t)stream;
    hipError_t e = hipSuccess;
#define GO(TT, RT, D, CG) e = qkv_rope_launch<TT, RT, D, CG>(st, d_A, d_W64, K, tiles, d_cs, d_cache_length, d_n, d_q_out, d_k_cache, d_v_cache, n_heads, n_kv_heads, (long long)max_len, v_t)
#define ROWS(TT, CG) do { if (rows_pad == 16) { if (depth_env == 2) GO(TT, 1, 2, CG); else if (depth_env == 3) GO(TT, 1, 3, CG); else GO(TT, 1, 4, CG); } \
                          else if (rows_pad == 32) { if (depth_env == 2) GO(TT, 2, 2, CG); else GO(TT, 2, 4, CG); } \
                          else if (rows_pad == 48) GO(TT, 3, 3, CG); else GO(TT, 4, 3, CG); } while (0)
    if (groups == 3) { if (dtype == SAMD_F16) ROWS(GF16, 3); else ROWS(GBF16, 3); }
    else { if (dtype == SAMD_F16) ROWS(GF16, 4); else ROWS(GBF16, 4); }
#undef ROWS
#undef GO
    if (e != hipSuccess) { samd_set_error("samd_gemm_qkv_rope: %s", hipGetErrorString(e)); return SAMD_E_HIP; }
    LAUNCHCHK();
    return SAMD_OK;
}

int samd_gemm_qkv_rope(const void *d_A, const void *d_W64, int32_t rows_pad, int32_t K, const float *d_cs, const int32_t *d_cache_length, const int32_t *d_n,
                       void *d_q_out, void *d_k_cache, void *d_v_cache, int32_t n_heads, int32_t n_kv_heads, int32_t head_dim, int64_t max_len,
                       int32_t dtype, void *stream) {
    return gemm_qkv_rope_impl(d_A, d_W64, rows_pad, K, d_cs, d_cache_length, d_n, d_q_out, d_k_cache, d_v_cache, n_heads, n_kv_heads, head_dim, max_len, dtype, stream, 0);
}

int samd_gemm_qkv_rope_vt(const void *d_A, const void *d_W64, int32_t rows_pad, int32_t K, const float *d_cs, const int32_t *d_cache_length, const int32_t *d_n,
                          void *d_q_out, void *d_k_cache, void *d_vt_cache, int32_t n_heads, int32_t n_kv_heads, int32_t head_dim, int64_t max_len,
                          int32_t dtype, void *stream) {
    return gemm_qkv_rope_impl(d_A, d_W64, rows_pad, K, d_cs, d_cache_length, d_n, d_q_out, d_k_cache, d_vt_cache, n_heads, n_kv_heads, head_dim, max_len, dtype, stream, 1);
}

static int gemm_qkv_rope_norm_impl(const void *d_x, const float *d_ssq, const void *d_norm_weight, float eps, const void *d_W64, int32_t rows_pad, int32_t K,
                                   const float *d_cs, const int32_t *d_cache_length, const int32_t *d_n, void *d_q_out, void *d_k_cache, void *d_v_cache,
                                   int32_t n_heads, int32_t n_kv_heads, int32_t head_dim, int64_t max_len, int32_t dtype, void *stream, int v_t) {
    if (!d_x || !d_ssq || !d_norm_weight || !d_W64 || !d_cs || !d_cache_length || !d_n || !d_q_out || !d_k_cache || !d_v_cache || head_dim != 128 || n_heads < 1 ||
        n_kv_heads < 1 || (rows_pad != 16 && rows_pad != 8) || K < GEMM_KC || K % GEMM_KC != 0 || K / 16 > 32 * NORM_NS || (dtype != SAMD_F16 && dtype != SAMD_BF16)) {
        samd_set_error("samd_gemm_qkv_rope_norm: unsupported shape (8 or 16 rows, head_dim 128, K %% 256 == 0, K <= 8192, f16/bf16) or null pointer"); return SAMD_E_INVALID;
    }
    const int groups = qkv_tile_groups(n_heads + 2 * n_kv_heads);
    const int tiles = (n_heads + 2 * n_kv_heads) * 128 / (16 * groups);
    const NormArgs na{d_ssq, d_norm_weight, K / 16, 1.f / (float)K, eps};
    hipStream_t st = (hipStream_t)stream;
    hipError_t e = hipSuccess;
#define GO(TT, CG, AR) e = qkv_rope_launch<TT, 1, 4, CG, true, AR>(st, d_x, d_W64, K, tiles, d_cs, d_cache_length, d_n, d_q_out, d_k_cache, d_v_cache, n_heads, n_kv_heads, (long long)max_len, v_t, na)
    if (rows_pad == 8) {
        if (groups == 3) { if (dtype == SAMD_F16) GO(GF16, 3, 8); else GO(GBF16, 3, 8); }
        else { if (dtype == SAMD_F16) GO(GF16, 4, 8); else GO(GBF16, 4, 8); }
    } else {
        if (groups == 3) { if (dtype == SAMD_F16) GO(GF16, 3, 16); else GO(GBF16, 3, 16); }
        else { if (dtype == SAMD_F16) GO(GF16, 4, 16); else GO(GBF16, 4, 16); }
    }
#undef GO
    if (e != hipSuccess) { samd_set_error("samd_gemm_qkv_rope_norm: %s", hipGetErrorString(e)); return SAMD_E_HIP; }
    LAUNCHCHK();
    return SAMD_OK;
}

int samd_gemm_qkv_rope_norm(const void *d_x, const float *d_ssq, const void *d_norm_weight, float eps, const void *d_W64, int32_t rows_pad, int32_t K,
                            const float *d_cs, const int32_t *d_cache_length, const int32_t *d_n, void *d_q_out, void *d_k_cache, void *d_v_cache,
                            int32_t n_heads, int32_t n_kv_heads, int32_t head_dim, int64_t max_len, int32_t dtype, void *stream) {
    return gemm_qkv_rope_norm_impl(d_x, d_ssq, d_norm_weight, eps, d_W64, rows_pad, K, d_cs, d_cache_length, d_n, d_q_out, d_k_cache, d_v_cache, n_heads, n_kv_heads, head_dim,
                                   max_len, dtype, stream, 0);
}

int samd_gemm_qkv_rope_norm_vt(const void *d_x, const float *d_ssq, const void *d_norm_weight, float eps, const void *d_W64, int32_t rows_pad, int32_t K,
                               const float *d_cs, const int32_t *d_cache_length, const int32_t *d_n, void *d_q_out, void *d_k_cache, void *d_vt_cache,
                               int32_t n_heads, int32_t n_kv_heads, int32_t head_dim, int64_t max_len, int32_t dtype, void *stream) {
    return gemm_qkv_rope_norm_impl(d_x, d_ssq, d_norm_weight, eps, d_W64, rows_pad, K, d_cs, d_cache_length, d_n, d_q_out, d_k_cache, d_vt_cache, n_heads, n_kv_heads, head_dim,
                                   max_len, dtype, stream, 1);
}

int samd_gemm_skinny(const void *d_A, const void *d_W, int32_t rows_pad, int32_t N, int32_t K, int32_t splits, float *d_partial,
                     void *d_out, int32_t dtype, void *stream) {
    if (!d_A || !d_W || (rows_pad != 16 && rows_pad != 32 && rows_pad != 48 && rows_pad != 64) || N < GEMM_COLS || N % GEMM_COLS != 0 || K < GEMM_KC ||
        K % GEMM_KC != 0 || splits < 1 || splits > K / GEMM_KC || (splits == 1 ? !d_out : !d_partial) || (dtype != SAMD_F16 && dtype != SAMD_BF16)) {
        samd_set_error("samd_gemm_skinny: unsupported shape (rows 16/32/48/64, N %% 128 == 0, K %% 256 == 0) or null pointer"); return SAMD_E_INVALID;
    }
    const hipError_t e = gemm_dispatch<0>(dtype, rows_pad, dim3(N / GEMM_COLS, splits), (hipStream_t)stream, d_A, d_W, d_partial, splits == 1 ? d_out : nullptr, K, N,
                                          K / GEMM_KC, splits);
    if (e != hipSuccess) { samd_set_error("samd_gemm_skinny: %s", hipGetErrorString(e)); return SAMD_E_HIP; }
    LAUNCHCHK();
    return SAMD_OK;
}

int samd_gemm_skinny_groups(const void *d_A, const void *d_Wg, int32_t rows_pad, int32_t N, int32_t K, int32_t splits, float *d_partial,
                            void *d_out, int32_t dtype, void *stream) {
    if (!d_A || !d_Wg || (rows_pad != 16 && rows_pad != 32 && rows_pad != 48 && rows_pad != 64) || N < GEMM_COLS || N % GEMM_COLS != 0 || K < GEMM_KC ||
        K % GEMM_KC != 0 || splits < 1 || splits > K / GEMM_KC || (splits == 1 ? !d_out : !d_partial) || (dtype != SAMD_F16 && dtype != SAMD_BF16)) {
        samd_set_error("samd_gemm_skinny_groups: unsupported shape (rows 16/32/48/64, N %% 128 == 0, K %% 256 == 0) or null pointer"); return SAMD_E_INVALID;
    }
    const hipError_t e = gemm_dispatch<0, true>(dtype, rows_pad, dim3(N / GEMM_COLS, splits), (hipStream_t)stream, d_A, d_Wg, d_partial, splits == 1 ? d_out : nullptr, K, N,
                                                K / GEMM_KC, splits);
    if (e != hipSuccess) { samd_set_error("samd_gemm_skinny_groups: %s", hipGetErrorString(e)); return SAMD_E_HIP; }
    LAUNCHCHK();
    return SAMD_OK;
}

}

template <typename TT> struct F8Widen;
template <> struct F8Widen<GF16> {
    static __device__ __forceinline__ half8 cvt(unsigned w0, unsigned w1) {
        const auto a = __builtin_amdgcn_cvt_scalef32_pk_f16_fp8(w0, 1.0f, false), b = __builtin_amdgcn_cvt_scalef32_pk_f16_fp8(w0, 1.0f, true);
        const auto c = __builtin_amdgcn_cvt_scalef32_pk_f16_fp8(w1, 1.0f, false), d = __builtin_amdgcn_cvt_scalef32_pk_f16_fp8(w1, 1.0f, true);
        return __builtin_bit_cast(half8, (u32x4){__builtin_bit_cast(unsigned, a), __builtin_bit_cast(unsigned, b), __builtin_bit_cast(unsigned, c), __builtin_bit_cast(unsigned, d)});
    }
};
template <> struct F8Widen<GBF16> {
    static __device__ __forceinline__ bf16x8 cvt(unsigned w0, unsigned w1) {
        const auto a = __builtin_amdgcn_cvt_scalef32_pk_bf16_fp8(w0, 1.0f, false), b = __builtin_amdgcn_cvt_scalef32_pk_bf16_fp8(w0, 1.0f, true);
        const auto c = __builtin_amdgcn_cvt_scalef32_pk_bf16_fp8(w1, 1.0f, false), d = __builtin_amdgcn_cvt_scalef32_pk_bf16_fp8(w1, 1.0f, true);
        return __builtin_bit_cast(bf16x8, (u32x4){__builtin_bit_cast(unsigned, a), __builtin_bit_cast(unsigned, b), __builtin_bit_cast(unsigned, c), __builtin_bit_cast(unsigned, d)});
    }
};

template <typename TT, int RT, int DEPTH>
__global__ __launch_bounds__(64 * GEMM_WAVES, 2) void k_gemm_skinny_f8(const typename TT::elem *__restrict__ A, const unsigned char *__restrict__ W8,
                                                                     const float *__restrict__ scale, float *__restrict__ partial,
                                                                     typename TT::elem *__restrict__ out, int K, int N, int n_chunks, int n_splits) {
    typedef typename TT::elem E;
    constexpr int R = 16 * RT;
    constexpr int NT = 64 * GEMM_WAVES;
    constexpr int XV = (R * 32) / NT;
    constexpr int NB = DEPTH + 1;
    constexpr int PC = 4 + XV;
    constexpr size_t WCH = 32768, WU = 8192;
    extern __shared__ __attribute__((aligned(1024))) char gemm_lds[];
    E (*xs)[R][GEMM_KC] = reinterpret_cast<E (*)[R][GEMM_KC]>(gemm_lds);

    const int tid = threadIdx.x, w = tid >> 6, l = tid & 63, n = l & 15, g = l >> 4;
    const int n0 = blockIdx.x * GEMM_COLS + 16 * w;
    const int split = blockIdx.y;
    const int c0 = (int)((long long)split * n_chunks / n_splits), c1 = (int)((long long)(split + 1) * n_chunks / n_splits);
    const char *wtile = reinterpret_cast<const char *>(W8) + (size_t)blockIdx.x * n_chunks * WCH;
    const uint32_t wlane = (uint32_t)tid * 16;
    const uint32_t lds_base = (uint32_t)(uintptr_t)(lptr_t)&xs[0][0][0];
    const float sc = scale[n0 + n];

    floatx4 acc[RT];
#pragma unroll
    for (int mt = 0; mt < RT; mt++) acc[mt] = (floatx4){0.f, 0.f, 0.f, 0.f};

    u32x4 wr[DEPTH][4];
    auto load_wb = [&](u32x4 (&dst)[4], int c, int b) {
        const char *p = wtile + (size_t)c * WCH;
        asm volatile("global_load_dwordx4 %0, %1, %2 nt" : "=v"(dst[b]) : "v"(wlane), "s"(p + WU * b) : "memory");
    };
    auto stage_xi = [&](int c, int buf, int i) {
        const int slot = tid + NT * i, row = slot >> 5, pos = slot & 31, unit = pos ^ (row & 15);
        const E *src = A + (size_t)row * K + (size_t)c * GEMM_KC + 8 * unit;
        E *dst = &xs[buf][0][0] + (size_t)(NT * i + 64 * w) * 8;
        __builtin_amdgcn_global_load_lds((gptr_t)src, (lptr_t)dst, 16, 0, 0);
        asm volatile("" ::: "memory");
    };
    auto load_w = [&](u32x4 (&dst)[4], int c) {
#pragma unroll
        for (int b = 0; b < 4; b++) load_wb(dst, c, b);
    };
    auto stage_x = [&](int c, int buf) {
#pragma unroll
        for (int i = 0; i < XV; i++) stage_xi(c, buf, i);
    };
    auto phase = [&](u32x4 (&cur)[4], int c, int buf) {
        gemm_wait_younger<DEPTH, PC>(c1 - 1 - c);
        __builtin_amdgcn_s_barrier();
        asm volatile("" ::: "memory");
        const uint32_t xbase = lds_base + (uint32_t)buf * (R * GEMM_KC * 2) + (uint32_t)n * (GEMM_KC * 2);
#pragma unroll
        for (int b = 0; b < 4; b++) {
            const uint32_t a0 = xbase + (uint32_t)((8 * b + 2 * g) ^ n) * 16, a1 = xbase + (uint32_t)((8 * b + 2 * g + 1) ^ n) * 16;
            u32x4 r[RT][2];
            if constexpr (RT == 1)
                asm volatile("ds_read_b128 %0, %2\n\tds_read_b128 %1, %3\n\ts_waitcnt lgkmcnt(0)" : "=&v"(r[0][0]), "=&v"(r[0][1]) : "v"(a0), "v"(a1));
            else if constexpr (RT == 2)
                asm volatile("ds_read_b128 %0, %4\n\tds_read_b128 %1, %5\n\tds_read_b128 %2, %4 offset:8192\n\tds_read_b128 %3, %5 offset:8192\n\t"
                             "s_waitcnt lgkmcnt(0)" : "=&v"(r[0][0]), "=&v"(r[0][1]), "=&v"(r[1][0]), "=&v"(r[1][1]) : "v"(a0), "v"(a1));
            else if constexpr (RT == 3)
                asm volatile("ds_read_b128 %0, %6\n\tds_read_b128 %1, %7\n\tds_read_b128 %2, %6 offset:8192\n\tds_read_b128 %3, %7 offset:8192\n\t"
                             "ds_read_b128 %4, %6 offset:16384\n\tds_read_b128 %5, %7 offset:16384\n\ts_waitcnt lgkmcnt(0)"
                             : "=&v"(r[0][0]), "=&v"(r[0][1]), "=&v"(r[1][0]), "=&v"(r[1][1]), "=&v"(r[2][0]), "=&v"(r[2][1]) : "v"(a0), "v"(a1));
            else
                asm volatile("ds_read_b128 %0, %8\n\tds_read_b128 %1, %9\n\tds_read_b128 %2, %8 offset:8192\n\tds_read_b128 %3, %9 offset:8192\n\t"
                             "ds_read_b128 %4, %8 offset:16384\n\tds_read_b128 %5, %9 offset:16384\n\tds_read_b128 %6, %8 offset:24576\n\t"
                             "ds_read_b128 %7, %9 offset:24576\n\ts_waitcnt lgkmcnt(0)"
                             : "=&v"(r[0][0]), "=&v"(r[0][1]), "=&v"(r[1][0]), "=&v"(r[1][1]), "=&v"(r[2][0]), "=&v"(r[2][1]), "=&v"(r[3][0]), "=&v"(r[3][1])
                             : "v"(a0), "v"(a1));
            asm volatile("" : "+v"(cur[b]) : : "memory");
            const auto lo = F8Widen<TT>::cvt(cur[b][0], cur[b][1]), hi = F8Widen<TT>::cvt(cur[b][2], cur[b][3]);
#pragma unroll
            for (int mt = 0; mt < RT; mt++) {
                acc[mt] = TT::mfma(__builtin_bit_cast(typename TT::vec8, r[mt][0]), lo, acc[mt]);
                acc[mt] = TT::mfma(__builtin_bit_cast(typename TT::vec8, r[mt][1]), hi, acc[mt]);
            }
            if (RT >= 3 && c + DEPTH < c1) {
                load_wb(cur, c + DEPTH, b);
                if (b < XV) stage_xi(c + DEPTH, buf == 0 ? NB - 1 : buf - 1, b);
            }
        }
        if (RT < 3 && c + DEPTH < c1) { load_w(cur, c + DEPTH); stage_x(c + DEPTH, buf == 0 ? NB - 1 : buf - 1); }
    };
    if (c0 < c1) {
#pragma unroll
        for (int d = 0; d < DEPTH; d++)
            if (c0 + d < c1) { load_w(wr[d], c0 + d); stage_x(c0 + d, d); }
        int buf = 0;
        for (int c = c0; c < c1; c += DEPTH) {
#pragma unroll
            for (int d = 0; d < DEPTH; d++)
                if (c + d < c1) { phase(wr[d], c + d, buf); buf = buf == NB - 1 ? 0 : buf + 1; }
        }
    }
#pragma unroll
    for (int mt = 0; mt < RT; mt++) {
#pragma unroll
        for (int r = 0; r < 4; r++) {
            const int m = 16 * mt + 4 * g + r;
            const float v = acc[mt][r] * sc;
            if (out) out[(size_t)m * N + n0 + n] = (E)v;
            else __hip_atomic_store(&partial[((size_t)split * R + m) * N + n0 + n], v, __ATOMIC_RELAXED, __HIP_MEMORY_SCOPE_AGENT);
        }
    }
}
// ... 940 lines not shown
```

sam-decoding_amd/samd_hip/__init__.py:

```python
import ctypes as C
import os

import numpy as np

_HERE = os.path.dirname(os.path.abspath(__file__))
LIB_PATH = os.environ.get("SAMD_HIP_LIB") or os.path.join(_HERE, "libsamd_hip.so")
MAX_DRAFT = 128
TILE_ROWS = 64
TOPK = 8
REP_DMETA, REP_VERDICT, REP_TOKENS, REP_KVINDEX, REP_COUNTERS, REP_META, REPORT_INTS = 0, 16, 24, 152, 280, 288, 304
KIND_COUNT, KIND_ENDPOS = 0, 1
F16, BF16, F32 = 0, 1, 2

_lib = None


class SamdError(RuntimeError):
    pass


class Params(C.Structure):
    _fields_ = [("variant", C.c_int32), ("max_predicts", C.c_int32), ("alpha", C.c_double), ("K", C.c_int32),
                ("len_bias", C.c_int32), ("n_predicts", C.c_int32), ("len_threshold", C.c_int32),
                ("static_null", C.c_int32), ("reserved", C.c_int32)]


class DraftHost(C.Structure):
    _fields_ = [("type", C.c_int32), ("n", C.c_int32), ("n_leaves", C.c_int32), ("max_depth", C.c_int32),
                ("index_dyn", C.c_int32), ("match_dyn", C.c_int32), ("index_static", C.c_int32),
                ("match_static", C.c_int32), ("tokens", C.c_int32 * MAX_DRAFT), ("parent", C.c_int32 * MAX_DRAFT),
                ("position", C.c_int32 * MAX_DRAFT), ("mask", C.c_uint64 * MAX_DRAFT), ("mask_hi", C.c_uint64 * MAX_DRAFT),
                ("retrieve", C.c_int32 * (MAX_DRAFT * MAX_DRAFT))]


class E2State(C.Structure):
    _NAMES = ("row_lse", "top_logp", "top_idx", "scores", "cs_index", "all_scores", "all_tokens", "parents_list", "mask_rows", "row_src", "ids",
              "rec_top_vals", "rec_top_idx", "rec_best_vals", "rec_best_idx", "rec_final_vals", "rec_final_idx")
    _fields_ = [(n, C.c_void_p) for n in _NAMES]


class Warm(C.Structure):
    _fields_ = [("d_packed_w", C.c_void_p), ("N", C.c_int32), ("K", C.c_int32), ("splits", C.c_int32), ("kb_per_workgroup", C.c_int32),
                ("delay", C.c_int32), ("where", C.c_int32)]


class QkvEpilogue(C.Structure):
    _fields_ = [("d_bias", C.c_void_p), ("d_q_norm", C.c_void_p), ("d_k_norm", C.c_void_p), ("eps", C.c_float)]


class VerdictHost(C.Structure):
    _fields_ = [("best", C.c_int32), ("accept", C.c_int32), ("next_node", C.c_int32), ("next_token", C.c_int32),
                ("tokens", C.c_int32 * MAX_DRAFT), ("kv_index", C.c_int32 * MAX_DRAFT)]


_VP, _I32, _I64, _F32 = C.c_void_p, C.c_int32, C.c_int64, C.c_float
_PROTOS = {
    "samd_last_error": (C.c_char_p, []),
    "samd_device_count": (C.c_int, []),
    "samd_host_wait_spin": (C.c_int, [_I32]),
    "samd_device_info": (C.c_int, [_VP]),
    "samd_static_build": (C.c_int, [_VP, _VP, _I64, _I32, _I32, _VP]),
    "samd_static_from_tables": (C.c_int, [_I32, _I64, _VP, _VP, _VP, _VP, _VP, _VP, _VP, _I64, _VP]),
    "samd_static_save": (C.c_int, [_VP, C.c_char_p]),
    "samd_static_load": (C.c_int, [C.c_char_p, _VP]),
    "samd_static_free": (None, [_VP]),
    "samd_static_upload": (C.c_int, [_VP]),
    "samd_static_info": (C.c_int, [_VP, _VP]),
    "samd_static_from_pickle": (C.c_int, [C.c_char_p, _I32, _VP, _VP]),
    "samd_static_derived_info": (C.c_int, [_VP, _VP]),
    "samd_static_edge_blocks_info": (C.c_int, [_VP, _VP]),
    "samd_static_set_bigram_slots": (C.c_int, [_VP, _I32, _VP]),
    "samd_static_export": (C.c_int, [_VP, _VP, _VP, _VP, _VP, _VP, _VP]),
    "samd_static_device_image": (C.c_int, [_VP, _VP, _VP]),
    "samd_static_alloc_like": (C.c_int, [_VP, _VP]),
    "samd_static_host_image": (C.c_int, [_VP, _VP, _VP]),
    "samd_static_from_host_image": (C.c_int, [_VP, _VP, _VP]),
    "samd_static_adopt_device": (C.c_int, [_VP, _VP, _VP]),
    "samd_static_walk": (C.c_int, [_VP, _VP, _VP, _I32, _I32, _I32, _VP, _VP]),
    "samd_static_walk_counted": (C.c_int, [_VP, _VP, _VP, _I32, _I32, _I32, _VP, _VP]),
    "samd_static_lookup_batch": (C.c_int, [_VP, _VP, _VP, _I32, _I32, _VP, _VP, _VP]),
    "samd_static_walk_streams": (C.c_int, [_VP, _VP, _VP, _I32, _I32, _I32, _VP, _VP]),
    "samd_static_walk_streams_counted": (C.c_int, [_VP, _VP, _VP, _I32, _I32, _I32, _VP, _VP]),
    "samd_session_create": (C.c_int, [_I32, _VP]),
    "samd_session_free": (None, [_VP]),
    "samd_session_reset": (C.c_int, [_VP, _VP]),
    "samd_dyn_add_tokens": (C.c_int, [_VP, _VP, _I32, _VP, _VP]),
    "samd_dyn_walk": (C.c_int, [_VP, _VP, _I32, _I32, _VP, _VP]),
    "samd_session_static_walk": (C.c_int, [_VP, _VP, _VP, _I32, _VP, _I32, _VP, _VP]),
    "samd_session_export": (C.c_int, [_VP, _VP, _VP, _VP, _VP, _VP, _VP, _VP, _VP, _VP]),
    "samd_session_set_cursors": (C.c_int, [_VP, _I32, _I32, _I32, _I32, _VP]),
    "samd_session_draft": (C.c_int, [_VP, _VP, _VP, _VP, _VP]),
    "samd_session_draft_seq": (C.c_int, [_VP, _VP, _I32, _I32, _I32, _VP]),
    "samd_session_draft_tree": (C.c_int, [_VP, _VP, _VP, _I32, _I32, _I32, _VP]),
    "samd_session_draft_fixed": (C.c_int, [_VP, _VP, _VP, _I32, _I32, _I32, _VP]),
    "samd_session_set_draft": (C.c_int, [_VP, _VP, _VP, _I32, _I32, _VP]),
    "samd_session_read_draft": (C.c_int, [_VP, _VP, _VP]),
    "samd_session_set_draft_if_deferred": (C.c_int, [_VP, _VP, _VP, _I32, _I32, _VP]),
    "samd_session_report_async": (C.c_int, [_VP, _VP, _VP]),
    "samd_session_set_start_token": (C.c_int, [_VP, _VP, _VP]),
    "samd_scripted_argmax": (C.c_int, [_VP, _VP, _I32, _I32, _VP, _VP]),
    "samd_embed_rows_ssq": (C.c_int, [_VP, _VP, _VP, _VP, _I32, _I32, _I32, _I32, _VP]),
    "samd_embed_rows_ssq_rope": (C.c_int, [_VP, _VP, _VP, _VP, _I32, _I32, _I32, _I32, _VP, _VP, _VP, _VP, _VP, _I32, _I32, _I32, _VP]),
    "samd_gemm_qkv_rope_norm": (C.c_int, [_VP, _VP, _VP, C.c_float, _VP, _I32, _I32, _VP, _VP, _VP, _VP, _VP, _VP, _I32, _I32, _I32, _I64, _I32, _VP]),
    "samd_gemm_qkv_rope_norm_vt": (C.c_int, [_VP, _VP, _VP, C.c_float, _VP, _I32, _I32, _VP, _VP, _VP, _VP, _VP, _VP, _I32, _I32, _I32, _I64, _I32, _VP]),
    "samd_gemm_pairs_silu_norm": (C.c_int, [_VP, _VP, _VP, C.c_float, _VP, _I32, _I32, _I32, _VP, _I32, _VP]),
    "samd_gemm_cs_residual": (C.c_int, [_VP, _VP, _I32, _I32, _I32, _VP, _VP, _I32, _VP]),
    "samd_gemm_cs_residual_early": (C.c_int, [_VP, _VP, _I32, _I32, _VP, _VP, _I32, _VP, _VP, _I32, _VP]),
    "samd_tree_attention_signal": (C.c_int, [_VP, _VP, _VP, _VP, _I32, _I32, _I32, _I32, _I32, _I64, _VP, _VP, _VP, _F32, _VP, _I64, _VP, _VP]),
    "samd_session_report_target": (C.c_int, [_VP, C.POINTER(_VP)]),
    "samd_report_wait": (C.c_int, [_VP, _I32, _I64]),
    "samd_scripted_logits": (C.c_int, [_VP, _VP, _VP, _I32, _I32, _I64, _I32, _VP]),
    "samd_scripted_logits_order1": (C.c_int, [_VP, _VP, _VP, _I32, _I32, _I64, _I32, _VP]),
    "samd_session_device_views": (C.c_int, [_VP, _VP]),
    "samd_tree_buffers": (C.c_int, [_VP, _I32, _I32, _VP, _VP, _VP, _VP, _VP, _VP]),
    "samd_argmax_rows": (C.c_int, [_VP, _I32, _I32, _I64, _I64, _VP, _VP, _VP]),
    "samd_session_accept": (C.c_int, [_VP, _VP, _VP]),
    "samd_session_read_verdict": (C.c_int, [_VP, _VP, _VP]),
    "samd_session_commit": (C.c_int, [_VP, _VP, _VP]),
    "samd_session_step": (C.c_int, [_VP, _VP, _VP, _VP, _VP]),
    "samd_session_step_given": (C.c_int, [_VP, _VP, _VP, _VP, _VP, _VP]),
    "samd_session_candidates": (C.c_int, [_VP, _VP, _VP, _I32, _VP]),
    "samd_session_set_cache_length": (C.c_int, [_VP, _I32, _VP]),
    "samd_session_get_cache_length": (C.c_int, [_VP, _VP, _VP]),
    "samd_kv_compact": (C.c_int, [_VP, _VP, _I32, _I32, _I64, _I32, _I32, _VP]),
    "samd_kv_compact_indices": (C.c_int, [_VP, _I32, _I32, _I64, _I32, _I32, _I32, _VP, _I32, _VP]),
    "samd_tree_attention_workspace": (_I64, [_I32, _I32, _I32]),
    "samd_tree_attention": (C.c_int, [_VP, _VP, _VP, _VP, _I32, _I32, _I32, _I32, _I32, _I64, _VP, _VP, _VP, _F32,
                                      _VP, _I64, _VP]),
    "samd_tree_attention_vt": (C.c_int, [_VP, _VP, _VP, _VP, _I32, _I32, _I32, _I32, _I32, _I64, _VP, _VP, _VP, _F32,
                                         _VP, _I64, _VP, _VP]),
    "samd_tree_attention_warm": (C.c_int, [_VP, _VP, _VP, _VP, _I32, _I32, _I32, _I32, _I32, _I64, _VP, _VP, _VP, _F32,
                                           _VP, _I64, _VP, _VP]),
    "samd_rope_rows": (C.c_int, [_VP, _VP, _VP, _VP, _VP, _I32, _I32, _I32, _VP]),
    "samd_attention_block": (C.c_int, [_VP, _I32, _I64, _VP, _VP, _VP, _VP, _I32, _I32, _I32, _I32, _I32, _I64, _VP, _VP, _VP, _VP, _F32, _VP]),
    "samd_tree_attention_rope_workspace": (_I64, [_I32, _I32, _I32]),
    "samd_tree_attention_rope": (C.c_int, [_VP, _I32, _I64, _VP, _VP, _VP, _VP, _I32, _I32, _I32, _I32, _I32, _I64, _VP, _VP, _VP, _F32, _VP, _I64, _VP]),
    "samd_rope_kv_write_cs": (C.c_int, [_VP, _VP, _VP, _VP, _VP, _VP, _VP, _VP, _I32, _I32, _I32, _I32, _I64, _I32, _I32, _I64, _VP]),
    "samd_rope_kv_write_cs_vt": (C.c_int, [_VP, _VP, _VP, _VP, _VP, _VP, _VP, _VP, _I32, _I32, _I32, _I32, _I64, _I32, _I32, _I64, _VP]),
    "samd_rope_kv_write_vt": (C.c_int, [_VP, _VP, _VP, _VP, _VP, _VP, _VP, _VP, _VP, _I32, _I32, _I32, _I32, _I64, _I32, _I32, _I32, _I64, _VP]),
    "samd_rope_kv_write_epi": (C.c_int, [_VP, _VP, _VP, _VP, _VP, _VP, _VP, _VP, _VP, _VP, _I32, _I32, _I32, _I32, _I32, _I64, _I32, _I32, _I32, _I64,
                                         _VP, _VP]),
    "samd_kv_compact_vt": (C.c_int, [_VP, _VP, _I32, _I32, _I32, _I64, _I32, _I32, _VP]),
    "samd_kv_compact_indices_vt": (C.c_int, [_VP, _I32, _I32, _I32, _I64, _I32, _I32, _I32, _VP, _I32, _VP]),
    "samd_posterior_sampled": (C.c_int, [_VP, _I32, _VP, _I32, _I32, _I64, _VP, _I32, _VP, _VP, _VP]),
    "samd_posterior_sampled_nodes": (C.c_int, [_VP, _I32, _VP, _I32, _VP, _I32, _I32, _I64, _VP, _I32, _VP, _VP, _VP]),
    "samd_e2_rowstats_workspace": (C.c_int64, [_I64]),
    "samd_e2_stage_extend": (C.c_int, [_VP, _VP, _VP, _VP, _I32, _I32, _VP, _I32, _I32, _VP, _VP, _VP, _VP, _VP, _I32, _VP]),
    "samd_e2_rowstats": (C.c_int, [_VP, _I32, _I32, _I64, _I64, _VP, _VP, _I64, _VP]),
    "samd_e2_select": (C.c_int, [_VP, _I32, _VP, _VP, _I32, _I32, _VP, _VP, _VP, _VP, _VP, _I32, _I32, _VP]),
    "samd_e2_finish": (C.c_int, [_VP, _I32, _I32, _VP, _VP, _VP, _VP]),
    "samd_sum_partials_bias": (C.c_int, [_VP, _I32, _I64, _VP, _VP, _I32, _I32, _I32, _VP]),
    "samd_embed_rows": (C.c_int, [_VP, _VP, _VP, _I32, _I32, _I32, _I32, _VP]),
    "samd_rmsnorm": (C.c_int, [_VP, _VP, _VP, _VP, _I32, _I32, _F32, _I32, _I32, _I64, _VP]),
    "samd_rmsnorm_warm": (C.c_int, [_VP, _VP, _VP, _VP, _I32, _I32, _F32, _I32, _I32, _I64, _VP, _VP]),
    "samd_rope_kv_write": (C.c_int, [_VP, _VP, _VP, _VP, _VP, _VP, _VP, _VP, _VP, _I32, _I32, _I32, _I32, _I64, _I32, _I32, _I32, _I64, _VP]),
    "samd_silu_mul": (C.c_int, [_VP, _VP, _I32, _I32, _I32, _I32, _I64, _VP]),
    "samd_prefill_attention": (C.c_int, [_VP, _VP, _VP, _VP, _I32, _I32, _I32, _I32, _I32, _I32, _I64, C.c_float, _VP]),
    "samd_prefill_attention_vt": (C.c_int, [_VP, _VP, _VP, _VP, _I32, _I32, _I32, _I32, _I32, _I32, _I64, C.c_float, _VP]),
    "samd_gemm_splits": (C.c_int, [_I32, _I32, _I32]),
    "samd_gemm_workspace": (_I64, [_I32, _I32, _I32]),
    "samd_gemm_pack_weights": (C.c_int, [_VP, _VP, _I32, _I32, _VP]),
    "samd_gemm_skinny_silu": (C.c_int, [_VP, _VP, _I32, _I32, _I32, _VP, _I32, _VP]),
    "samd_gemm_skinny": (C.c_int, [_VP, _VP, _I32, _I32, _I32, _I32, _VP, _VP, _I32, _VP]),
    "samd_gemm_skinny_groups": (C.c_int, [_VP, _VP, _I32, _I32, _I32, _I32, _VP, _VP, _I32, _VP]),
    "samd_gemm_pack_f8": (C.c_int, [_VP, _VP, _I32, _I32, _VP]),
    "samd_gemm_skinny_f8": (C.c_int, [_VP, _VP, _VP, _I32, _I32, _I32, _I32, _VP, _VP, _I32, _VP]),
    "samd_gemm_pack_f4": (C.c_int, [_VP, _VP, _VP, _I32, _I32, _VP]),
    "samd_gemm_skinny_f4": (C.c_int, [_VP, _VP, _I32, _I32, _I32, _I32, _VP, _VP, _I32, _VP]),
    "samd_moe_workspace_layout": (_I32, [_I32]),
    "samd_moe_workspace": (_I64, [_I32, _I32, _I32, _I32, _I32]),
    "samd_moe_pack_experts": (C.c_int, [_VP, _VP, _I32, _I32, _I32, _I32, _VP]),
    "samd_moe_route": (C.c_int, [_VP, _VP, _VP, _I32, _I32, _I32, _I32, _I32, _VP, _VP, _VP, _I32, _VP]),
    "samd_moe_lists": (C.c_int, [_VP, _VP, _I32, _I32, _I32, _VP, _VP]),
    "samd_moe_gate_up_silu": (C.c_int, [_VP, _VP, _VP, _I32, _I32, _I32, _I32, _I32, _VP, _I32, _VP]),
    "samd_moe_down_combine": (C.c_int, [_VP, _VP, _VP, _VP, _VP, _VP, _I32, _I32, _I32, _I32, _I32, _VP, _I32, _VP]),
    "samd_moe_gate_up_silu_f4": (C.c_int, [_VP, _VP, _VP, _I32, _I32, _I32, _I32, _I32, _VP, _I32, _VP]),
    "samd_moe_down_combine_f4": (C.c_int, [_VP, _VP, _VP, _VP, _VP, _VP, _I32, _I32, _I32, _I32, _I32, _VP, _I32, _VP]),
    "samd_gemm_pack_qkv64": (C.c_int, [_VP, _VP, _I32, _I32, _VP]),
    "samd_gemm_pack_groups": (C.c_int, [_VP, _VP, _I32, _I32, _VP]),
    "samd_gemm_pairs_silu": (C.c_int, [_VP, _VP, _I32, _I32, _I32, _VP, _I32, _VP]),
    "samd_gemm_qkv_rope": (C.c_int, [_VP, _VP, _I32, _I32, _VP, _VP, _VP, _VP, _VP, _VP, _I32, _I32, _I32, _I64, _I32, _VP]),
    "samd_gemm_qkv_rope_vt": (C.c_int, [_VP, _VP, _I32, _I32, _VP, _VP, _VP, _VP, _VP, _VP, _I32, _I32, _I32, _I64, _I32, _VP]),
    "samd_recycle_create": (C.c_int, [_I32, _VP, _VP, _I32, _VP]),
    "samd_recycle_free": (None, [_VP]),
    "samd_recycle_update": (C.c_int, [_VP, _VP, _VP, _I32, _I32, _VP, _I64, _I64, _VP]),
    "samd_recycle_draft": (C.c_int, [_VP, _VP, _VP, _VP]),
    "samd_recycle_export": (C.c_int, [_VP, _VP, _VP, _VP]),
}


def lib():
    global _lib
    if _lib is None:
        if not os.path.exists(LIB_PATH):
            raise SamdError(f"{LIB_PATH} is missing: build it with `python __graft_entry__.py build` "
                            "(hipcc --offload-arch=gfx950); there is no CPU fallback")
        L = C.CDLL(LIB_PATH)
        for name, (res, args) in _PROTOS.items():
            fn = getattr(L, name)
            fn.restype = res
            fn.argtypes = args
        _lib = L
    return _lib


def check(rc):
    if rc != 0:
        msg = lib().samd_last_error()
        raise SamdError(f"libsamd_hip error {rc}: {msg.decode() if msg else ''}")


def host_waits_by_spinning(device_index=None):
    if os.environ.get("SAMD_SPIN_WAIT", "1") == "0":
        return False
    import logging
    log = logging.getLogger("samd_hip")
    try:
        import torch
        rc = lib().samd_host_wait_spin(-1 if device_index is None else int(device_index))
    except (ImportError, OSError, AttributeError, SamdError) as e:
        log.warning("host_waits_by_spinning: not applied (%s)", e)
        return False
    if rc != 0:
        msg = lib().samd_last_error()
        log.warning("host_waits_by_spinning: not applied (rc %d: %s)", rc, msg.decode() if msg else "")
    return rc == 0


def require_gpu():
    if lib().samd_device_count() < 1:
        raise SamdError("no MI355X / HIP device visible: the SAM-Decoding hot path has no CPU fallback")


def _np_i32(a):
    return np.ascontiguousarray(a, dtype=np.int32)


def _ptr(a):
    if a is None:
        return None
    if isinstance(a, C.c_void_p):
        return a
    if isinstance(a, np.ndarray):
        return a.ctypes.data_as(C.c_void_p)
    if hasattr(a, "data_ptr"):
        return C.c_void_p(a.data_ptr())
    return C.c_void_p(int(a))


def current_stream():
    import torch
    return C.c_void_p(torch.cuda.current_stream().cuda_stream)


def torch_dtype_code(dtype):
    import torch
    return {torch.float16: F16, torch.bfloat16: BF16, torch.float32: F32}[dtype]


# ... 319 lines not shown
```

sam-decoding_amd/samd_hip/llama.py:

```python
import ctypes as C
import math
import os

import torch

from . import (F16, BF16, MAX_DRAFT, TILE_ROWS, QkvEpilogue, SamdError, Session, Warm, _ptr, check, current_stream, lib, require_gpu,
               torch_dtype_code)
from . import fp8 as F8
from . import mxfp4 as MX
from . import moe as MOE


def _env_weight_format(weight_format):
    return weight_format if weight_format is not None else (os.environ.get("SAMD_WEIGHT_FORMAT") or None)


def _weight_format(weight_format, weights, dtype):
    has_f8 = any(l[k].dtype == torch.float8_e4m3fn for l in weights["layers"] for k in F8.PROJECTIONS if k in l)
    has_f4 = any(_is_f4_tensor(l[k]) for l in weights["layers"] for k in MX.PROJECTIONS if k in l)
    names = {torch.float16: ("fp16", "float16", "half"), torch.bfloat16: ("bf16", "bfloat16")}.get(dtype, ())
    if weight_format is None:
        fmt = "fp8" if has_f8 else ("mxfp4" if has_f4 else None)
    elif weight_format in ("fp8", "mxfp4"):
        fmt = weight_format
    elif weight_format == dtype or (isinstance(weight_format, str) and weight_format.lower() in names):
        fmt = None
    else:
        raise SamdError(f"weight_format {weight_format!r}: expected None, 'fp8', 'mxfp4' or the model dtype ({dtype})")
    if has_f8 and fmt != "fp8":
        raise SamdError(f"the weights carry float8_e4m3fn projections; weight_format {weight_format!r} would need them dequantised (pass None or 'fp8')")
    if has_f4 and fmt != "mxfp4":
        raise SamdError(f"the weights carry MXFP4 projections; weight_format {weight_format!r} would need them dequantised (pass None or 'mxfp4')")
    return fmt


def _is_f4_tensor(t):
    return t.dtype == torch.uint8 or MX.is_fp4_dtype(t.dtype)


def _cfg_get(cfg, name, default=None):
    if isinstance(cfg, dict):
        return cfg.get(name, default)
    return getattr(cfg, name, default)


class LlamaShape:

    def __init__(self, cfg, qkv_bias=None, qk_norm=None):
        self.hidden = int(_cfg_get(cfg, "hidden_size"))
        self.inter = int(_cfg_get(cfg, "intermediate_size"))
        self.layers = int(_cfg_get(cfg, "num_hidden_layers"))
        self.heads = int(_cfg_get(cfg, "num_attention_heads"))
        kv = _cfg_get(cfg, "num_key_value_heads")
        self.kv_heads = int(kv) if kv is not None else self.heads
        hd = _cfg_get(cfg, "head_dim")
        self.head_dim = int(hd) if hd else self.hidden // self.heads
        self.vocab = int(_cfg_get(cfg, "vocab_size"))
        self.eps = float(_cfg_get(cfg, "rms_norm_eps", 1e-6))
        self.max_pos = int(_cfg_get(cfg, "max_position_embeddings", 2048))
        rp = _cfg_get(cfg, "rope_parameters") or _cfg_get(cfg, "rope_scaling") or {}
        theta = _cfg_get(cfg, "rope_theta")
        if theta is None and isinstance(rp, dict):
            theta = rp.get("rope_theta")
        self.rope_theta = float(theta if theta is not None else 10000.0)
        self.rope_scaling = dict(rp) if isinstance(rp, dict) else {}
        if self.head_dim != 128:
            raise SamdError("the gfx950 tree-attention kernel is specialised for head_dim 128 (Vicuna-7B / Llama-3-8B)")
        self.model_type = str(_cfg_get(cfg, "model_type", None) or "llama")
        layer_types = _cfg_get(cfg, "layer_types", None) or ()
        if _cfg_get(cfg, "use_sliding_window", False) or any(t != "full_attention" for t in layer_types):
            raise SamdError("sliding-window attention layers are not supported (use_sliding_window / layer_types)")
        if _cfg_get(cfg, "attention_bias", False):
            raise SamdError("attention_bias=True puts a bias on o_proj, which the runner does not support (q|k|v biases alone are)")
        if _cfg_get(cfg, "mlp_bias", False):
            raise SamdError("MLP projection biases (mlp_bias=True) are not supported")
        self.qkv_bias = (self.model_type == "qwen2") if qkv_bias is None else bool(qkv_bias)
        self.qk_norm = (self.model_type in ("qwen3", "qwen3_moe")) if qk_norm is None else bool(qk_norm)
        self.n_experts = self.top_k = self.moe_inter = 0
        self.norm_topk = False
        self.sparse = [False] * self.layers
        if self.model_type == "qwen3_moe":
            self.n_experts = int(_cfg_get(cfg, "num_experts", 0) or 0)
            self.top_k = int(_cfg_get(cfg, "num_experts_per_tok", 0) or 0)
            self.moe_inter = int(_cfg_get(cfg, "moe_intermediate_size", 0) or 0)
            self.norm_topk = bool(_cfg_get(cfg, "norm_topk_prob", False))
            self.sparse = MOE.sparse_layer_map(self.layers, self.n_experts, _cfg_get(cfg, "mlp_only_layers"), _cfg_get(cfg, "decoder_sparse_step", 1))
        self.moe = any(self.sparse)
        if self.moe:
            MOE.check_shape(self.hidden, self.moe_inter, self.n_experts, self.top_k)

    def inv_freq(self):
        d = self.head_dim
        inv = 1.0 / (self.rope_theta ** (torch.arange(0, d, 2, dtype=torch.float64) / d))
        rs = self.rope_scaling
        kind = rs.get("rope_type", rs.get("type", "default")) if rs else "default"
        if kind == "llama3":
            factor, lo, hi = rs["factor"], rs["low_freq_factor"], rs["high_freq_factor"]
            old = rs["original_max_position_embeddings"]
            wavelen = 2 * math.pi / inv
            scaled = torch.where(wavelen > old / lo, inv / factor, inv)
            smooth = (old / wavelen - lo) / (hi - lo)
            mid = (1 - smooth) * inv / factor + smooth * inv
            is_mid = (wavelen <= old / lo) & (wavelen >= old / hi)
            inv = torch.where(is_mid, mid, scaled)
        elif kind == "linear":
            inv = inv / rs["factor"]
        elif kind not in ("default", None):
            raise SamdError(f"unsupported rope scaling '{kind}'")
        return inv


class LlamaRunner:

    BUCKETS = (1, 8, 16, 32, 48, 64, 128)

    def __init__(self, shape, weights, max_cache_len, dtype=torch.float16, device="cuda", kv=None, native_gemm=True, packed_lm_head=None,
                 attention=None, weight_format=None, draft_head=False, expert_format=MOE.AUTO):
        experts4 = [MOE.is_4bit(l["experts_gu"]) or MOE.is_4bit(l["experts_down"]) for l in weights["layers"] if "experts_gu" in l]
        self.expert_format = MOE.resolve_expert_format(expert_format, any(experts4), shape.moe)
        if shape.moe:
            MOE.reject_unsupported(_weight_format(weight_format, weights, dtype), native_gemm, draft_head)
        if any(experts4):
            if not all(experts4):
                raise SamdError(f"a mix of 4-bit and model-dtype sparse layers ({sum(experts4)} of {len(experts4)} carry MXFP4 experts): "
                                "the runner takes the experts of all sparse layers in one format")
            for i, l in enumerate(weights["layers"]):
                if "experts_gu" in l:
                    MOE.check_quantised_experts(l["experts_gu"], l.get("experts_gu_scale"), l["experts_down"], l.get("experts_down_scale"), dtype,
                                                f"layer {i} experts")
        self.draft_head = bool(draft_head)
        require_gpu()
        self.shape, self.dtype, self.device = shape, dtype, torch.device(device)
        self.dt = torch_dtype_code(dtype)
        if self.dt not in (F16, BF16):
            raise SamdError("LlamaRunner computes in fp16 or bf16")
        self.weight_format = _weight_format(weight_format, weights, dtype)
        f8, f4 = self.weight_format == "fp8", self.weight_format == "mxfp4"
        quant = f8 or f4
        if f8 and not native_gemm:
            raise SamdError("FP8 projections exist only in the streaming kernel's packed form: native_gemm=False is not available with weight_format 'fp8'")
        if f4 and not native_gemm:
            raise SamdError("MXFP4 projections exist only in the streaming kernel's packed form: native_gemm=False is not available with weight_format 'mxfp4'")
        s = shape
        self.w = weights
        streams = lambda t: bool(native_gemm) and t.shape[0] % 128 == 0 and t.shape[1] % 256 == 0
        self.native_gemm_max_rows = int(os.environ.get("SAMD_NATIVE_GEMM_MAX_ROWS", 64))
        moe = shape.moe
        self.route_log = None
        if quant or moe:
            self.native_gemm_max_rows = TILE_ROWS
        self.layer_hook = None
        self.warm_kb = int(os.environ.get("SAMD_L2_WARM_KB", 0))
        self.warm_delay = int(os.environ.get("SAMD_L2_WARM_DELAY", 0))
        self.warm_where = int(os.environ.get("SAMD_L2_WARM_WHERE", 0))
        self.attention = attention or os.environ.get("SAMD_ATTENTION", "split")
        if self.attention not in ("split", "split2", "split3", "block"):
            raise SamdError(f"unknown attention mode '{self.attention}'")
        self.qkv_epilogue = bool(s.qkv_bias or s.qk_norm)
        if self.qkv_epilogue and self.attention not in ("split", "split3"):
            raise SamdError(f"attention mode '{self.attention}' rotates q / k inside its own kernel, which has no q|k|v bias or q / k norm: "
                            f"use 'split' or 'split3' for this model")
        self.v_layout_t = self.attention == "block" or (self.attention in ("split", "split3") and s.head_dim == 128
                                                        and os.environ.get("SAMD_V_LAYOUT", "t") != "rows")
        self.v_transposed = self.v_layout_t
        def pack(t):
            if not streams(t):
                return None
            out = torch.empty_like(t)
            check(lib().samd_gemm_pack_weights(_ptr(t), _ptr(out), t.shape[0], t.shape[1], current_stream()))
            return out
        def pack_gate_up(t):
            if s.inter % 16 != 0 or not streams(t):
                return None
            gate, up = t[:s.inter].view(s.inter // 16, 16, -1), t[s.inter:].view(s.inter // 16, 16, -1)
            w = torch.stack([gate, up], dim=1).reshape(2 * s.inter, -1).contiguous()
            out = torch.empty_like(w)
            check(lib().samd_gemm_pack_groups(_ptr(w), _ptr(out), 2 * s.inter, w.shape[1], current_stream()))
            return out
        def pack_qkv64(t):
            heads_total = s.heads + 2 * s.kv_heads
            mode = os.environ.get("SAMD_QKV_FUSED", "1")
            n_cols = heads_total * 128
            enough = n_cols // 64 >= 128 or (n_cols % 48 == 0 and n_cols // 48 >= 128)
            if (not streams(t) or self.attention != "split" or (not enough and mode != "force") or s.head_dim != 128 or mode == "0"
                    or self.qkv_epilogue):
                return None
            out = torch.empty_like(t)
            check(lib().samd_gemm_pack_qkv64(_ptr(t), _ptr(out), heads_total, t.shape[1], current_stream()))
            return out
        def pack_groups(t, fold):
            if not fold or t.shape[0] % 16 != 0 or t.shape[1] % 256 != 0:
                return None
            out = torch.empty_like(t)
            check(lib().samd_gemm_pack_groups(_ptr(t), _ptr(out), t.shape[0], t.shape[1], current_stream()))
            return out
        def pack_f8(l, k):
            t = l[k]
            N, K = t.shape
            if N % 128 != 0 or K % 256 != 0:
                raise SamdError(f"FP8 projection {k} of shape {tuple(t.shape)}: the FP8 kernel needs N % 128 == 0 and K % 256 == 0")
            if t.dtype == torch.float8_e4m3fn:
                q, scale = t.to(self.device).contiguous(), l.pop(k + "_scale").to(device=self.device, dtype=torch.float32).contiguous()
            else:
                q, scale = F8.quantize_rows(t)
            l[k] = torch.empty(t.shape, dtype=torch.float8_e4m3fn, device="meta")
            del t
            out = torch.empty_like(q)
            check(lib().samd_gemm_pack_f8(_ptr(q), _ptr(out), N, K, current_stream()))
            return out, scale
        def pack_f4(l, k):
            t = l[k]
            N, K = (t.shape[0], 2 * t.shape[1]) if _is_f4_tensor(t) else t.shape
            if N % 128 != 0 or K % 256 != 0:
                raise SamdError(f"MXFP4 projection {k} of shape ({N}, {K}): the MXFP4 kernel needs N % 128 == 0 and K % 256 == 0")
            if _is_f4_tensor(t):
                q, e8 = MX.fuse_mxfp4([(t, l.pop(k + "_e8"))], self.device)
                if tuple(e8.shape) != (N, K // 32):
                    raise SamdError(f"MXFP4 projection {k}: block scales of shape {tuple(e8.shape)} for a ({N}, {K}) matrix")
                MX.check_exponents(e8, dtype, f"MXFP4 projection {k}")
            else:
                q, e8 = MX.quantize_blocks(t, dtype)
            l[k] = torch.empty((N, K), dtype=torch.uint8, device="meta")
            del t
            out = torch.empty(MX.packed_bytes(N, K), dtype=torch.uint8, device=self.device)
            check(lib().samd_gemm_pack_f4(_ptr(q), _ptr(e8), _ptr(out), N, K, current_stream()))
            return out
        layers = []
        for l in weights["layers"]:
            if f4:
                lp = dict(wqkv=None, wqkv64=None, wo=None, wo_g=None, wgu=None, wdown=None, wdown_g=None)
                for k in MX.PROJECTIONS:
                    lp[k + "_f4"] = pack_f4(l, k)
                layers.append(lp)
                continue
            if f8:
                lp = dict(wqkv=None, wqkv64=None, wo=None, wo_g=None, wgu=None, wdown=None, wdown_g=None)
                for k in F8.PROJECTIONS:
                    lp[k + "_f8"] = pack_f8(l, k)
                layers.append(lp)
                continue
            sparse = "experts_gu" in l
            lp = dict(wgu=None if sparse else pack_gate_up(l["wgu"]), wqkv64=pack_qkv64(l["wqkv"]))
            lp["wqkv"] = pack(l["wqkv"]) if lp["wqkv64"] is None else None
            fold = (lp["wqkv64"] is not None and lp["wgu"] is not None and s.hidden <= 8192 and os.environ.get("SAMD_NORM_FOLD", "1") != "0"
                    and not moe)
            if sparse:
                gu_cols = s.hidden // 2 if MOE.is_4bit(l["experts_gu"]) else s.hidden
                if tuple(l["router"].shape) != (s.n_experts, s.hidden) or tuple(l["experts_gu"].shape) != (s.n_experts, 2 * s.moe_inter, gu_cols):
                    raise SamdError(f"sparse layer weights of shapes {tuple(l['router'].shape)}, {tuple(l['experts_gu'].shape)} do not match the shape")
                if self.expert_format == "mxfp4":
                    ekeys = ("experts_gu", "experts_gu_scale", "experts_down", "experts_down_scale")
                    if MOE.is_4bit(l["experts_gu"]):
                        quad = tuple(MX._bytes(l[k]).to(self.device).contiguous() for k in ekeys)
                    else:
                        quad = MOE.quantize_experts(l["experts_gu"], l["experts_down"], dtype, f"layer {len(layers)} experts")
                    lp["moe_gu"], lp["moe_down"] = MOE.pack_experts_mxfp4(*quad)
                    for k, t in zip(ekeys, quad):
                        l[k] = torch.empty(t.shape, dtype=torch.uint8, device="meta")
                    del quad
                else:
                    lp["moe_gu"], lp["moe_down"] = MOE.pack_experts(l["experts_gu"], l["experts_down"])
                    for k in ("experts_gu", "experts_down"):
                        l[k] = torch.empty(l[k].shape, dtype=l[k].dtype, device="meta")
                lp["wo_g"], lp["wdown_g"], lp["wdown"] = pack_groups(l["wo"], fold), None, None
                lp["wo"] = pack(l["wo"])
                layers.append(lp)
                continue
            lp["wo_g"], lp["wdown_g"] = pack_groups(l["wo"], fold), pack_groups(l["wdown"], fold)
            both = os.environ.get("SAMD_GEMM_ONE_COPY", "0") != "1"
            for k in ("wo", "wdown"):
                gm_ok = lp[k + "_g"] is not None and l[k].shape[0] % 128 == 0
                lp[k] = pack(l[k]) if (both or not gm_ok) else None
            layers.append(lp)
        self.wp = dict(lm_head=packed_lm_head if packed_lm_head is not None else pack(weights["lm_head"]), layers=layers)
        self.native_gemm = self.wp["lm_head"] is not None or any(v is not None for l in self.wp["layers"] for v in l.values())
        if not self.native_gemm:
            self.wp = None
        self.fused_mlp = self.wp is not None and all(l["wgu"] is not None for l in self.wp["layers"] if "moe_gu" not in l)
        self.norm_fold = (self.wp is not None and self.attention == "split"
                          and all(l.get("wo_g") is not None and l.get("wdown_g") is not None for l in self.wp["layers"]))
        self.scale = 1.0 / math.sqrt(s.head_dim)
        self.epi = self.epi_nobias = None
        if self.qkv_epilogue:
            def epi(l, bias):
                return QkvEpilogue(l["bqkv"].data_ptr() if bias and l.get("bqkv") is not None else None,
                                   l["q_norm"].data_ptr() if l.get("q_norm") is not None else None,
                                   l["k_norm"].data_ptr() if l.get("k_norm") is not None else None, s.eps)
            for l in weights["layers"]:
                if s.qkv_bias != (l.get("bqkv") is not None) or s.qk_norm != (l.get("q_norm") is not None and l.get("k_norm") is not None):
                    raise SamdError("the layer weights do not match the shape's qkv_bias / qk_norm")
                if s.qkv_bias and tuple(l["bqkv"].shape) != ((s.heads + 2 * s.kv_heads) * s.head_dim,):
                    raise SamdError(f"q|k|v bias of shape {tuple(l['bqkv'].shape)}")
                if s.qk_norm and (tuple(l["q_norm"].shape) != (s.head_dim,) or tuple(l["k_norm"].shape) != (s.head_dim,)):
                    raise SamdError("q_norm / k_norm weights must have head_dim elements")
                for k in ("bqkv", "q_norm", "k_norm"):
                    t = l.get(k)
                    if t is not None and (t.dtype != dtype or t.device.type != self.device.type or not t.is_contiguous()):
                        raise SamdError(f"{k} must be a contiguous {dtype} tensor on the GPU")
            self.epi = [epi(l, True) for l in weights["layers"]]
            self.epi_nobias = [epi(l, False) for l in weights["layers"]]
        self.row_major_released = quant or moe
        if moe and self.wp:
            for l, lp in zip(self.w["layers"], self.wp["layers"]):
                for k in ("wqkv", "wo", "wgu", "wdown"):
# ... 331 lines not shown
                                cs=torch.zeros((MAX_DRAFT, s.head_dim), dtype=torch.float32, device=dev),
                                ssq=torch.zeros((max(s.hidden // 16, 1), 16), dtype=torch.float32, device=dev))
            if s.moe:
                self._buf[R]["moe"] = MOE.MoeBuffers(RP, s.hidden, s.moe_inter, s.n_experts, s.top_k, dt, self.dt, dev)
        return self._buf[R]

    def max_draft_rows(self):
        wide_ok = (not self.row_major_released) and self.attention in ("split", "split3") and not getattr(self, "draft_head", False)
        return MAX_DRAFT if wide_ok else min(MAX_DRAFT, 64)

    def bucket(self, n):
        for b in self.BUCKETS:
            if n <= b:
                return b
        raise SamdError(f"draft of {n} nodes exceeds {MAX_DRAFT}")

    def forward_rows(self, R, d_tokens, d_relpos, d_mask, d_L, d_n, x_in=None, d_vis=None):
        if self.shape.moe:
            MOE.reject_unsupported(draft_head=getattr(self, "draft_head", False))
        if self._rows_pad(R) > self.native_gemm_max_rows and self.row_major_released:
            raise SamdError(f"a {R}-row forward needs the row-major projection matrices (released: SAMD_RELEASE_ROW_MAJOR / release_row_major()); "
                            f"drafts above {self.native_gemm_max_rows} nodes and the library-GEMM path are unavailable on this runner")
        L, s, b, dt, st = lib(), self.shape, self._buffers(R), self.dt, current_stream()
        RP, part = b["rows_pad"], b["part"]
        if (self.norm_fold and RP == 16 and x_in is None and d_vis is None and not getattr(self, "draft_head", False)
                and RP <= self.native_gemm_max_rows):
            return self._forward_rows_fold(R, b, d_tokens, d_relpos, d_mask, d_L, d_n)

        def hint(w, wp, fused=False, is_head=False):
            if wp is None or RP > self.native_gemm_max_rows or self.warm_kb <= 0:
                return None
            n, k = w.shape
            sp = 1 if (fused or is_head) else L.samd_gemm_splits(n, k, RP)
            return C.byref(Warm(wp.data_ptr(), n, k, sp, self.warm_kb, self.warm_delay, self.warm_where))

        def gemm(a, w, wp, out, wg=None, f8=None, f4=None):
            n, k = w.shape
            if f4 is not None:
                sp = L.samd_gemm_splits(n, k, RP)
                check(L.samd_gemm_skinny_f4(_ptr(a), _ptr(f4), RP, n, k, sp, _ptr(part), _ptr(out), dt, st))
                return (out, 0, 0) if sp == 1 else (part, sp, RP * n)
            if f8 is not None:
                sp = L.samd_gemm_splits(n, k, RP)
                check(L.samd_gemm_skinny_f8(_ptr(a), _ptr(f8[0]), _ptr(f8[1]), RP, n, k, sp, _ptr(part), _ptr(out), dt, st))
                return (out, 0, 0) if sp == 1 else (part, sp, RP * n)
            if (wp is None and wg is None) or RP > self.native_gemm_max_rows:
                torch.mm(a[:R], w.t(), out=out[:R])
                return out, 0, 0
            sp = L.samd_gemm_splits(n, k, RP) if out is not b["logits"] else 1
            if wp is not None and os.environ.get("SAMD_GEMM_PREFER_GROUPS", "0") != "1":
                check(L.samd_gemm_skinny(_ptr(a), _ptr(wp), RP, n, k, sp, _ptr(part), _ptr(out), dt, st))
            else:
                check(L.samd_gemm_skinny_groups(_ptr(a), _ptr(wg if wg is not None else wp), RP, n, k, sp, _ptr(part), _ptr(out), dt, st))
            return (out, 0, 0) if sp == 1 else (part, sp, RP * n)

        if x_in is None:
            check(L.samd_embed_rows(_ptr(d_tokens), _ptr(self.w["embed"]), _ptr(b["x"]), R, s.hidden, s.vocab, dt, st))
        else:
            rows_in = min(R, x_in.shape[0])
            if x_in.data_ptr() != b["x"].data_ptr():
                b["x"][:rows_in].copy_(x_in[:rows_in])
        head = getattr(self, "draft_head", False)
        log_routes = s.moe and self.route_log is not None and not torch.cuda.is_current_stream_capturing()
        block = self.attention == "block"
        vt = self.v_transposed and not block
        if self.attention != "split3":
            check(L.samd_rope_rows(_ptr(d_relpos), _ptr(d_vis if d_vis is not None else d_L), _ptr(self.cos), _ptr(self.sin), _ptr(b["cs"]), R,
                                   s.head_dim, self.rope_rows, st))
        if d_vis is not None and not block:
            raise SamdError("a visible length different from the write position needs attention mode 'block'")
        delta, dn, dstride = None, 0, 0
        packed = self.wp["layers"] if self.wp else [{}] * len(self.w["layers"])
        for li, w in enumerate(self.w["layers"]):
            if self.layer_hook is not None:
                self.layer_hook(li)
            wp = packed[li]
            raw_in = head and li == 0
            if not raw_in:
                check(L.samd_rmsnorm_warm(_ptr(b["x"]), _ptr(delta), _ptr(w["ln1"]), _ptr(b["h"]), R, s.hidden, s.eps, dt, dn, dstride,
                                          hint(w["wqkv"], wp.get("wqkv")), st))
            fused_qkv = wp.get("wqkv64") is not None and self.attention == "split" and RP <= self.native_gemm_max_rows and d_vis is None
            if fused_qkv:
                check((L.samd_gemm_qkv_rope_vt if vt else L.samd_gemm_qkv_rope)(
                    _ptr(b["x"] if raw_in else b["h"]), _ptr(wp["wqkv64"]), RP, s.hidden, _ptr(b["cs"]), _ptr(d_L), _ptr(d_n),
                    _ptr(b["q"]), _ptr(self.kv[li, 0]), _ptr(self.kv[li, 1]), s.heads, s.kv_heads, s.head_dim, self.max_len, dt, st))
            else:
                src, n_p, stride = gemm(b["x"] if raw_in else b["h"], w["wqkv"], wp.get("wqkv"), b["qkv"], f8=wp.get("wqkv_f8"), f4=wp.get("wqkv_f4"))
            if block:
                check(L.samd_attention_block(_ptr(src), n_p, stride, _ptr(b["cs"]), _ptr(self.kv[li, 0]), _ptr(self.kv[li, 1]), _ptr(b["attn"]), dt, R,
                                             s.heads, s.kv_heads, s.head_dim, self.max_len, _ptr(d_mask), _ptr(d_L), _ptr(d_vis), _ptr(d_n), self.scale, st))
            elif self.attention == "split2":
                check(L.samd_tree_attention_rope(_ptr(src), n_p, stride, _ptr(b["cs"]), _ptr(self.kv[li, 0]), _ptr(self.kv[li, 1]), _ptr(b["attn"]), dt, R,
                                                 s.heads, s.kv_heads, s.head_dim, self.max_len, _ptr(d_mask), _ptr(d_L), _ptr(d_n), self.scale,
                                                 _ptr(b["ws"]), b["ws_bytes"], st))
            else:
                if fused_qkv:
                    pass
                elif self.epi is not None:
                    cs_form = self.attention == "split"
                    check(L.samd_rope_kv_write_epi(
                        _ptr(src), _ptr(d_relpos), _ptr(d_L), _ptr(d_n), None if cs_form else _ptr(self.cos), None if cs_form else _ptr(self.sin),
                        _ptr(b["cs"]) if cs_form else None, _ptr(b["q"]), _ptr(self.kv[li, 0]), _ptr(self.kv[li, 1]), int(vt), R, s.heads,
                        s.kv_heads, s.head_dim, self.max_len, self.rope_rows, dt, n_p, stride, C.byref(self.epi[li]), st))
                elif self.attention == "split":
                    check((L.samd_rope_kv_write_cs_vt if vt else L.samd_rope_kv_write_cs)(
                        _ptr(src), _ptr(d_relpos), _ptr(d_L), _ptr(d_n), _ptr(b["cs"]), _ptr(b["q"]), _ptr(self.kv[li, 0]),
                        _ptr(self.kv[li, 1]), R, s.heads, s.kv_heads, s.head_dim, self.max_len, dt, n_p, stride, st))
                else:
                    check((L.samd_rope_kv_write_vt if vt else L.samd_rope_kv_write)(
                        _ptr(src), _ptr(d_relpos), _ptr(d_L), _ptr(d_n), _ptr(self.cos), _ptr(self.sin),
                        _ptr(b["q"]), _ptr(self.kv[li, 0]), _ptr(self.kv[li, 1]), R, s.heads, s.kv_heads,
                        s.head_dim, self.max_len, self.rope_rows, dt, n_p, stride, st))
                check((L.samd_tree_attention_vt if vt else L.samd_tree_attention_warm)(
                    _ptr(b["q"]), _ptr(self.kv[li, 0]), _ptr(self.kv[li, 1]), _ptr(b["attn"]), dt, R, s.heads,
                    s.kv_heads, s.head_dim, self.max_len, _ptr(d_mask), _ptr(d_L), _ptr(d_n), self.scale,
                    _ptr(b["ws"]), b["ws_bytes"], hint(w["wo"], wp.get("wo")), st))
            src, n_p, stride = gemm(b["attn"].view(b["attn"].shape[0], -1), w["wo"], wp.get("wo"), b["o"], wg=wp.get("wo_g"), f8=wp.get("wo_f8"), f4=wp.get("wo_f4"))
            check(L.samd_rmsnorm_warm(_ptr(b["x"]), _ptr(src), _ptr(w["ln2"]), _ptr(b["h"]), R, s.hidden, s.eps, dt, n_p, stride,
                                      None, st))
            if "moe_gu" in wp:
                mb = b["moe"]
                mb.route(b["h"], w["router"], d_n, s.norm_topk)
                if log_routes:
                    idx = mb.topk_idx.clone()
                    self.route_log.append((li, int((idx[:, 0] >= 0).sum()), idx, mb.topk_w.clone()))
                delta, dn, dstride = mb.experts(b["h"], wp["moe_gu"], wp["moe_down"], d_n, self.expert_format), 0, 0
                continue
            if wp.get("wgu") is not None and RP <= self.native_gemm_max_rows:
                check(L.samd_gemm_pairs_silu(_ptr(b["h"]), _ptr(wp["wgu"]), RP, s.inter, s.hidden, _ptr(b["act"]), dt, st))
            else:
                src, n_p, stride = gemm(b["h"], w["wgu"], None, b["gu"], f8=wp.get("wgu_f8"), f4=wp.get("wgu_f4"))
                check(L.samd_silu_mul(_ptr(src), _ptr(b["act"]), R, s.inter, dt, n_p, stride, st))
            delta, dn, dstride = gemm(b["act"], w["wdown"], wp.get("wdown"), b["d"], wg=wp.get("wdown_g"), f8=wp.get("wdown_f8"), f4=wp.get("wdown_f4"))
        check(L.samd_rmsnorm_warm(_ptr(b["x"]), _ptr(delta), _ptr(self.w["norm"]), _ptr(b["h"]), R, s.hidden, s.eps, dt, dn, dstride,
                                  hint(self.w["lm_head"], self.wp["lm_head"] if self.wp else None, is_head=True), st))
        gemm(b["x"] if head else b["h"], self.w["lm_head"], self.wp["lm_head"] if self.wp else None, b["logits"])
        if not head:
            check(L.samd_argmax_rows(_ptr(b["logits"]), dt, R, s.vocab, s.vocab, None, _ptr(b["argmax"]), st))
        return b

    def _forward_rows_fold(self, R, b, d_tokens, d_relpos, d_mask, d_L, d_n):
        L, s, dt, st = lib(), self.shape, self.dt, current_stream()
        x, ssq = b["x"], b["ssq"]
        rows_cs = 8 if R <= 8 else 16
        rows_a = rows_cs if os.environ.get("SAMD_NORM_ROWS8", "1") != "0" else 16
        if s.head_dim == 128 and os.environ.get("SAMD_FUSE_EMBED_ROPE", "1") != "0":
            check(L.samd_embed_rows_ssq_rope(_ptr(d_tokens), _ptr(self.w["embed"]), _ptr(x), _ptr(ssq), 16, s.hidden, s.vocab, dt, _ptr(d_relpos), _ptr(d_L),
                                             _ptr(self.cos), _ptr(self.sin), _ptr(b["cs"]), R, s.head_dim, self.rope_rows, st))
        else:
            check(L.samd_embed_rows_ssq(_ptr(d_tokens), _ptr(self.w["embed"]), _ptr(x), _ptr(ssq), 16, s.hidden, s.vocab, dt, st))
            check(L.samd_rope_rows(_ptr(d_relpos), _ptr(d_L), _ptr(self.cos), _ptr(self.sin), _ptr(b["cs"]), R, s.head_dim, self.rope_rows, st))
        attn2d = b["attn"].view(b["attn"].shape[0], -1)
        qkv_launch = L.samd_gemm_qkv_rope_norm_vt if self.v_transposed else L.samd_gemm_qkv_rope_norm
        attn_launch = L.samd_tree_attention_vt if self.v_transposed else L.samd_tree_attention_warm
        for li, (w, wp) in enumerate(zip(self.w["layers"], self.wp["layers"])):
            if self.layer_hook is not None:
                self.layer_hook(li)
            check(qkv_launch(_ptr(x), _ptr(ssq), _ptr(w["ln1"]), s.eps, _ptr(wp["wqkv64"]), rows_a, s.hidden, _ptr(b["cs"]), _ptr(d_L), _ptr(d_n),
                             _ptr(b["q"]), _ptr(self.kv[li, 0]), _ptr(self.kv[li, 1]), s.heads, s.kv_heads, s.head_dim, self.max_len, dt, st))
            check(attn_launch(_ptr(b["q"]), _ptr(self.kv[li, 0]), _ptr(self.kv[li, 1]), _ptr(b["attn"]), dt, R, s.heads,
                              s.kv_heads, s.head_dim, self.max_len, _ptr(d_mask), _ptr(d_L), _ptr(d_n), self.scale,
                              _ptr(b["ws"]), b["ws_bytes"], None, st))
            check(L.samd_gemm_cs_residual(_ptr(attn2d), _ptr(wp["wo_g"]), rows_cs, s.hidden, attn2d.shape[1], _ptr(x), _ptr(ssq), dt, st))
            check(L.samd_gemm_pairs_silu_norm(_ptr(x), _ptr(ssq), _ptr(w["ln2"]), s.eps, _ptr(wp["wgu"]), rows_a, s.inter, s.hidden, _ptr(b["act"]), dt, st))
            check(L.samd_gemm_cs_residual(_ptr(b["act"]), _ptr(wp["wdown_g"]), rows_cs, s.hidden, s.inter, _ptr(x), _ptr(ssq), dt, st))
        check(L.samd_rmsnorm(_ptr(x), None, _ptr(self.w["norm"]), _ptr(b["h"]), R, s.hidden, s.eps, dt, 0, 0, st))
        wl = self.wp["lm_head"]
        if wl is not None:
            check(L.samd_gemm_skinny(_ptr(b["h"]), _ptr(wl), 16, s.vocab, s.hidden, 1, _ptr(b["part"]), _ptr(b["logits"]), dt, st))
        else:
            torch.mm(b["h"][:R], self.w["lm_head"].t(), out=b["logits"][:R])
        check(L.samd_argmax_rows(_ptr(b["logits"]), dt, R, s.vocab, s.vocab, None, _ptr(b["argmax"]), st))
        return b

    def prefill(self, session: Session, input_ids, on_chunk=None):
        ids = input_ids.reshape(-1).to(device=self.device, dtype=torch.int32)
        N = ids.numel()
        if N < 1 or N > self.max_len:
            raise SamdError(f"prompt of {N} tokens does not fit max_cache_len {self.max_len}")
        if N >= 2 * TILE_ROWS and os.environ.get("SAMD_PREFILL", "wide") != "chunked" and not self.row_major_released:
            return self._prefill_wide(session, ids, on_chunk)
        v = session.device_views()
        b = None
        for c0 in range(0, N, TILE_ROWS):
            n = min(TILE_ROWS, N - c0)
            self.pf_tokens.zero_()
            self.pf_tokens[:n] = ids[c0:c0 + n]
            self.pf_n.fill_(n)
            session.set_cache_length(c0)
            b = self.forward_rows(TILE_ROWS, self.pf_tokens, self.pf_relpos, self.pf_mask, v["cache_length"], self.pf_n)
            if on_chunk is not None:
                on_chunk(self.pf_tokens, b["logits"], n, b["h"])
        session.set_cache_length(N)
        session.set_start_token(b["argmax"][(N - 1) % TILE_ROWS:])
        return b["logits"][(N - 1) % TILE_ROWS]

    PF_SPLIT_MIN_ROWS = 1024
    PF_ATTN_PAD = 128

    def _is_gfx950(self):
        if not hasattr(self, "_gfx950"):
            name = getattr(torch.cuda.get_device_properties(self.device), "gcnArchName", "") or ""
            self._gfx950 = name.split(":")[0] == "gfx950"
        return self._gfx950

    def _time_mm(self, x, wt, out, reps=3):
        best = float("inf")
        torch.mm(x, wt, out=out)
        for _ in range(reps):
            e0, e1 = torch.cuda.Event(enable_timing=True), torch.cuda.Event(enable_timing=True)
            e0.record()
            torch.mm(x, wt, out=out)
            e1.record()
            e1.synchronize()
            best = min(best, e0.elapsed_time(e1))
        return best

    def tune_prefill(self, max_rows=None):
        self._pf_plan = {}
        if os.environ.get("SAMD_PREFILL_SPLIT", "1") == "0" or self.row_major_released:
            return self._pf_plan
        max_rows = min(int(max_rows or self.max_len), 4096)
        w0 = self.w["layers"][0]
        try:
            for key in ("wqkv", "wo", "wgu", "wdown"):
                wt = w0[key].t()
                K, N = wt.shape
                x = torch.zeros((max_rows + 64, K), dtype=self.dtype, device=self.device)
                out = torch.empty((max_rows + 64, N), dtype=self.dtype, device=self.device)
                small = {r: self._time_mm(x[:r], wt, out[:r]) for r in (64, 128, 192, 256)}
                plan = {}
                for R in range(max(256, (self.PF_SPLIT_MIN_ROWS // 256) * 256), max_rows, 256):
                    t_at = self._time_mm(x[:R], wt, out[:R])
                    t_past = self._time_mm(x[:R + 64], wt, out[:R + 64])
                    plan[R] = {r: t_at + small[r] < 0.95 * t_past for r in small}
                self._pf_plan[key] = plan
                del x, out
        except RuntimeError as e:
            import warnings
            warnings.warn(f"tune_prefill: measurement failed ({str(e)[:120]}); projections of long prompts stay single library calls", RuntimeWarning)
            self._pf_plan = {}
        return self._pf_plan

    def prefill_plan_summary(self):
        plan = getattr(self, "_pf_plan", None) or {}
        return {k: [R for R, d in sorted(v.items()) if any(d.values())] for k, v in plan.items()}

    def _pf_split(self, key, M):
        if M <= self.PF_SPLIT_MIN_ROWS:
            return 0
        if getattr(self, "_pf_plan", None) is None:
            self.tune_prefill()
        R = ((M - 1) // 256) * 256
        rest = -(-(M - R) // 64) * 64
        return R if self._pf_plan.get(key, {}).get(R, {}).get(rest, False) else 0

    def _pf_mm(self, x, w, out, key, bias=None):
        R = self._pf_split(key, x.shape[0])
        mm = torch.mm if bias is None else (lambda a, b, out: torch.addmm(bias, a, b, out=out))
        if R:
            mm(x[:R], w.t(), out=out[:R])
            mm(x[R:], w.t(), out=out[R:])
        else:
            mm(x, w.t(), out=out)

    def _prefill_wide(self, session: Session, ids, on_chunk=None):
        L, s, dt, st, N = lib(), self.shape, self.dt, current_stream(), ids.numel()
        dev, ty = self.device, self.dtype
        z = lambda *sz: torch.empty(sz, dtype=ty, device=dev)
        x, h = z(N, s.hidden), z(N, s.hidden)
        own_attn = (s.head_dim == 128 and os.environ.get("SAMD_PREFILL_ATTENTION", "own") != "sdpa"
                    and self._is_gfx950())
        Np = N if own_attn else -(-N // self.PF_ATTN_PAD) * self.PF_ATTN_PAD
        if Np > self.max_len:
            Np = N
        ao = z(N, s.heads * s.head_dim) if own_attn else None
        qkv_p, qp = z(Np, (s.heads + 2 * s.kv_heads) * s.head_dim), z(Np, s.heads, s.head_dim)
        qkv, q = qkv_p[:N], qp[:N]
        if Np > N:
            qp[N:].zero_()
            if self.v_transposed:
                qkv_p[N:].zero_()
                self.kv[:, 0, :, N:Np].zero_()
            else:
                self.kv[:, :, :, N:Np].zero_()
        o, gu, act, d = z(N, s.hidden), z(N, 2 * s.inter), z(N, s.inter), z(N, s.hidden)
        relpos = torch.arange(N, dtype=torch.int32, device=dev)
        d_L = torch.zeros(1, dtype=torch.int32, device=dev)
        d_n = torch.full((1,), N, dtype=torch.int32, device=dev)
        check(L.samd_embed_rows(_ptr(ids), _ptr(self.w["embed"]), _ptr(x), N, s.hidden, s.vocab, dt, st))
        delta = None
        for li, w in enumerate(self.w["layers"]):
            check(L.samd_rmsnorm(_ptr(x), _ptr(delta), _ptr(w["ln1"]), _ptr(h), N, s.hidden, s.eps, dt, 0, 0, st))
            self._pf_mm(h, w["wqkv"], qkv, "wqkv", bias=w.get("bqkv"))
            if self.epi is not None:
                check(L.samd_rope_kv_write_epi(_ptr(qkv), _ptr(relpos), _ptr(d_L), _ptr(d_n), _ptr(self.cos), _ptr(self.sin), None, _ptr(q),
                                               _ptr(self.kv[li, 0]), _ptr(self.kv[li, 1]), int(self.v_transposed), N, s.heads, s.kv_heads,
                                               s.head_dim, self.max_len, self.rope_rows, dt, 0, 0, C.byref(self.epi_nobias[li]), st))
                if self.v_transposed:
                    vv = qkv_p[:, (s.heads + s.kv_heads) * s.head_dim:].view(Np, s.kv_heads, s.head_dim).transpose(0, 1)
                else:
                    vv = self.kv[li, 1][:, :Np]
            elif self.v_transposed:
                check(L.samd_rope_kv_write_vt(_ptr(qkv), _ptr(relpos), _ptr(d_L), _ptr(d_n), _ptr(self.cos), _ptr(self.sin), _ptr(q),
                                              _ptr(self.kv[li, 0]), _ptr(self.kv[li, 1]), N, s.heads, s.kv_heads, s.head_dim, self.max_len,
                                              self.rope_rows, dt, 0, 0, st))
                vv = qkv_p[:, (s.heads + s.kv_heads) * s.head_dim:].view(Np, s.kv_heads, s.head_dim).transpose(0, 1)
            else:
                check(L.samd_rope_kv_write(_ptr(qkv), _ptr(relpos), _ptr(d_L), _ptr(d_n), _ptr(self.cos), _ptr(self.sin), _ptr(q),
                                           _ptr(self.kv[li, 0]), _ptr(self.kv[li, 1]), N, s.heads, s.kv_heads, s.head_dim, self.max_len,
                                           self.rope_rows, dt, 0, 0, st))
                vv = self.kv[li, 1][:, :Np]
            if own_attn:
                check((L.samd_prefill_attention_vt if self.v_transposed else L.samd_prefill_attention)(
                    _ptr(q), _ptr(self.kv[li, 0]), _ptr(self.kv[li, 1]), _ptr(ao), dt, N, 0, s.heads, s.kv_heads,
# ... 58 lines not shown
```

Baseline: 814.4.

## Size fused decode GEMM activation staging to the device-side live row count

Adds _n variants of the fused QKV-rope-norm, gate/up SiLU-norm and o/down residual GEMMs that read the live row count from device memory. They skip activation and norm-weight loads for padded rows and zero those LDS slots instead. The residual GEMM also issues weight loads before activation loads and dispatches on a compile-time activation-load count. The goal is to cut memory traffic and epilogue work when only a few draft rows are live, at the cost of more kernel variants and per-row branching. The new path is on by default through SAMD_ROWS_N.

```diff
diff --git a/include/samd_hip.h b/include/samd_hip.h
--- a/include/samd_hip.h
+++ b/include/samd_hip.h
@@ -299,6 +299,16 @@
 int samd_gemm_qkv_rope(const void *d_A, const void *d_W64, int32_t rows_pad, int32_t K, const float *d_cs, const int32_t *d_cache_length,
                        const int32_t *d_n, void *d_q_out, void *d_k_cache, void *d_v_cache, int32_t n_heads, int32_t n_kv_heads,
                        int32_t head_dim, int64_t max_len, int32_t dtype, void *stream);
+int samd_gemm_qkv_rope_norm_n(const void *d_x, const float *d_ssq, const void *d_norm_weight, float eps, const void *d_W64, int32_t rows_pad, int32_t K,
+                              const float *d_cs, const int32_t *d_cache_length, const int32_t *d_n, void *d_q_out, void *d_k_cache, void *d_v_cache,
+                              int32_t n_heads, int32_t n_kv_heads, int32_t head_dim, int64_t max_len, int32_t dtype, void *stream);
+int samd_gemm_qkv_rope_norm_n_vt(const void *d_x, const float *d_ssq, const void *d_norm_weight, float eps, const void *d_W64, int32_t rows_pad, int32_t K,
+                                 const float *d_cs, const int32_t *d_cache_length, const int32_t *d_n, void *d_q_out, void *d_k_cache, void *d_vt_cache,
+                                 int32_t n_heads, int32_t n_kv_heads, int32_t head_dim, int64_t max_len, int32_t dtype, void *stream);
+int samd_gemm_pairs_silu_norm_n(const void *d_x, const float *d_ssq, const void *d_norm_weight, float eps, const void *d_Wg, int32_t rows_pad, int32_t inter,
+                                int32_t K, const int32_t *d_n, void *d_out, int32_t dtype, void *stream);
+int samd_gemm_cs_residual_n(const void *d_A, const void *d_Wg, int32_t rows_pad, int32_t N, int32_t K, const int32_t *d_n, void *d_x, float *d_ssq,
+                            int32_t dtype, void *stream);
 int samd_gemm_qkv_rope_norm_vt(const void *d_x, const float *d_ssq, const void *d_norm_weight, float eps, const void *d_W64, int32_t rows_pad, int32_t K,
                                const float *d_cs, const int32_t *d_cache_length, const int32_t *d_n, void *d_q_out, void *d_k_cache, void *d_vt_cache,
                                int32_t n_heads, int32_t n_kv_heads, int32_t head_dim, int64_t max_len, int32_t dtype, void *stream);
diff --git a/sam-decoding_amd/csrc/gemm_kernels.hip b/sam-decoding_amd/csrc/gemm_kernels.hip
--- a/sam-decoding_amd/csrc/gemm_kernels.hip
+++ b/sam-decoding_amd/csrc/gemm_kernels.hip
@@ -230,7 +230,7 @@
         const typename TT::elem *__restrict__ A, const typename TT::elem *__restrict__ W, int K, int n_chunks,
         const float *__restrict__ cs, const int *__restrict__ d_L, const int *__restrict__ d_n,
         typename TT::elem *__restrict__ q_out, typename TT::elem *__restrict__ k_cache, typename TT::elem *__restrict__ v_cache,
-        int H, int Hkv, long long max_len, NormArgs na, int v_t) {
+        int H, int Hkv, long long max_len, NormArgs na, int v_t, int rows_cap) {
     typedef typename TT::elem E;
     typedef typename TT::vec8 V8;
     constexpr int R = 16 * RT;
@@ -245,13 +245,15 @@
 
     const int tid = threadIdx.x, w = tid >> 6, l = tid & 63, n = l & 15, g = l >> 4;
     const bool streams = CG == 4 || w < 2 * CG;
-    static_assert(AR == 16 || (AR == 8 && NORM && RT == 1), "8 activation rows: the norm-fold kernels only");
-    const bool stager = AR == 16 || w < GEMM_WAVES / 2;
+    static_assert(AR == 16 || ((AR == 8 || AR == 0) && NORM && RT == 1), "fewer than 16 activation rows: the norm-fold kernels only");
     const int cg = CG == 4 ? (w & 3) : (streams ? w % CG : 0), kh = CG == 4 ? (w >> 2) : (streams ? w / CG : 0);
     const char *wtile = reinterpret_cast<const char *>(W) + (size_t)blockIdx.x * n_chunks * CH;
     const uint32_t wlane = (uint32_t)(64 * (CG * kh + cg) + l) * 16;
     const uint32_t lds_base = (uint32_t)(uintptr_t)(lptr_t)&xs[0][0][0];
-    const int n_rows = d_n[0], L = d_L[0];
+    const int n_raw = d_n[0], L = d_L[0];
+    const int n_rows = AR == 0 ? (n_raw < 0 ? 0 : (n_raw > rows_cap ? rows_cap : n_raw)) : n_raw;
+    const int a_rows = AR == 0 ? n_rows : AR;
+    const bool stager = AR == 16 || 2 * w < a_rows;
 
     floatx4 acc[RT];
 #pragma unroll
@@ -273,8 +275,10 @@
         const E *src = A + (size_t)row * K + (size_t)c * GEMM_KC + 8 * unit;
         if constexpr (NORM) {
             const E *gsrc = reinterpret_cast<const E *>(na.g) + (size_t)c * GEMM_KC + 8 * unit;
-            asm volatile("global_load_dwordx4 %0, %1, off" : "=v"(xr[d][i]) : "v"(src) : "memory");
-            asm volatile("global_load_dwordx4 %0, %1, off" : "=v"(gr[d][i]) : "v"(gsrc) : "memory");
+            if (AR != 0 || row < a_rows) {
+                asm volatile("global_load_dwordx4 %0, %1, off" : "=v"(xr[d][i]) : "v"(src) : "memory");
+                asm volatile("global_load_dwordx4 %0, %1, off" : "=v"(gr[d][i]) : "v"(gsrc) : "memory");
+            }
         } else {
             E *dst = &xs[buf][0][0] + (size_t)(NT * i + 64 * w) * 8;
             __builtin_amdgcn_global_load_lds((gptr_t)src, (lptr_t)dst, 16, 0, 0);
@@ -296,7 +300,7 @@
                 const int slot = tid + NT * i, row = slot >> 5;
                 asm volatile("" : "+v"(xr[d][i]), "+v"(gr[d][i]) : : "memory");
                 const u32x4 v = norm_scale8<E>(xr[d][i], gr[d][i], norm_rs[row]);
-                *reinterpret_cast<u32x4 *>(&xs[buf][0][0] + (size_t)slot * 8) = v;
+                *reinterpret_cast<u32x4 *>(&xs[buf][0][0] + (size_t)slot * 8) = (AR != 0 || row < a_rows) ? v : (u32x4){0u, 0u, 0u, 0u};
             }
         }
     };
@@ -344,7 +348,7 @@
 #pragma unroll
     for (int d = 0; d < DEPTH; d++)
         if (d < n_chunks) issue(wr[d], d, d, d);
-    if constexpr (AR == 8) {
+    if constexpr (AR != 16) {
         if (!stager) {
 #pragma unroll
             for (int bz = 0; bz < NB; bz++) *reinterpret_cast<u32x4 *>(&xs[bz][0][0] + (size_t)tid * 8) = (u32x4){0u, 0u, 0u, 0u};
@@ -425,7 +429,8 @@
 
 template <typename TT, int RT, int DEPTH, bool NORM, int AR = 16>
 __global__ __launch_bounds__(64 * GEMM_WAVES, RT >= 3 || DEPTH > 2 ? 2 : GEMM_WAVES / 2) void k_gemm_pairs_silu(const typename TT::elem *__restrict__ A, const typename TT::elem *__restrict__ W,
-                                                                                                     typename TT::elem *__restrict__ out, int K, int inter, int n_chunks, int n_pairs, NormArgs na) {
+                                                                                                     typename TT::elem *__restrict__ out, int K, int inter, int n_chunks, int n_pairs, NormArgs na,
+                                                                                                     const int *__restrict__ d_n, int rows_cap) {
     typedef typename TT::elem E;
     typedef typename TT::vec8 V8;
     constexpr int R = 16 * RT;
@@ -443,8 +448,10 @@
 #endif
     const int p0 = (int)((long long)blockIdx.x * n_pairs / gridDim.x), p1 = (int)((long long)(blockIdx.x + 1) * n_pairs / gridDim.x);
     const bool active = w < 2 * (p1 - p0);
-    static_assert(AR == 16 || (AR == 8 && NORM && RT == 1), "8 activation rows: the norm-fold kernels only");
-    const bool stager = AR == 16 || w < GEMM_WAVES / 2;
+    static_assert(AR == 16 || ((AR == 8 || AR == 0) && NORM && RT == 1), "fewer than 16 activation rows: the norm-fold kernels only");
+    int a_rows = AR;
+    if constexpr (AR == 0) { const int n_raw = d_n[0]; a_rows = n_raw < 0 ? 0 : (n_raw > rows_cap ? rows_cap : n_raw); }
+    const bool stager = AR == 16 || 2 * w < a_rows;
     const int gi = 2 * p0 + w;
     const char *wgrp = reinterpret_cast<const char *>(W) + (size_t)(active ? gi : 0) * n_chunks * 8192;
     const uint32_t wlane = (uint32_t)l * 16;
@@ -474,8 +481,10 @@
             const E *src = A + (size_t)((abl & 8) ? (row & 15) : row) * K + (size_t)c * GEMM_KC + 8 * unit;
             if constexpr (NORM) {
                 const E *gsrc = reinterpret_cast<const E *>(na.g) + (size_t)c * GEMM_KC + 8 * unit;
-                asm volatile("global_load_dwordx4 %0, %1, off" : "=v"(xr[d][i]) : "v"(src) : "memory");
-                asm volatile("global_load_dwordx4 %0, %1, off" : "=v"(gr[d][i]) : "v"(gsrc) : "memory");
+                if (AR != 0 || row < a_rows) {
+                    asm volatile("global_load_dwordx4 %0, %1, off" : "=v"(xr[d][i]) : "v"(src) : "memory");
+                    asm volatile("global_load_dwordx4 %0, %1, off" : "=v"(gr[d][i]) : "v"(gsrc) : "memory");
+                }
             } else {
                 E *dst = &xs[buf][0][0] + (size_t)(NT * i + 64 * w) * 8;
                 __builtin_amdgcn_global_load_lds((gptr_t)src, (lptr_t)dst, 16, 0, 0);
@@ -494,7 +503,7 @@
                     const int slot = tid + NT * i, row = slot >> 5;
                     asm volatile("" : "+v"(xr[d][i]), "+v"(gr[d][i]) : : "memory");
                     const u32x4 v = norm_scale8<E>(xr[d][i], gr[d][i], norm_rs[row]);
-                    *reinterpret_cast<u32x4 *>(&xs[buf][0][0] + (size_t)slot * 8) = v;
+                    *reinterpret_cast<u32x4 *>(&xs[buf][0][0] + (size_t)slot * 8) = (AR != 0 || row < a_rows) ? v : (u32x4){0u, 0u, 0u, 0u};
                 }
             }
             asm volatile("s_waitcnt lgkmcnt(0)" ::: "memory");
@@ -539,7 +548,7 @@
 #pragma unroll
     for (int d = 0; d < DEPTH; d++)
         if (d < n_chunks) { if (active) load_w(wr[d], d); stage_x(d, d, d); }
-    if constexpr (AR == 8) {
+    if constexpr (AR != 16) {
         if (!stager) {
 #pragma unroll
             for (int bz = 0; bz < NB; bz++) *reinterpret_cast<u32x4 *>(&xs[bz][0][0] + (size_t)tid * 8) = (u32x4){0u, 0u, 0u, 0u};
@@ -576,6 +585,7 @@
 #pragma unroll
             for (int r = 0; r < 4; r++) {
                 const int m = 16 * mt + 4 * g + r;
+                if (AR == 0 && m >= a_rows) continue;
                 const float gf = (float)(E)acc[mt][r], uf = (float)(E)ex[((w >> 1) * R + m) * 16 + n];
                 const E sv = (E)(gf / (1.f + __expf(-gf)));
                 out[(size_t)m * inter + col] = (E)((float)sv * uf);
@@ -583,14 +593,18 @@
     }
 }
 
-template <typename TT, int ROWS, bool EARLY = false>
+template <int V> struct GemmInt { static constexpr int value = V; };
+template <typename TT, int ROWS, bool EARLY = false, bool NV = false>
 __global__ __launch_bounds__(64 * GEMM_WAVES, 2) void k_gemm_cs_residual(const typename TT::elem *__restrict__ A, const typename TT::elem *__restrict__ W,
                                                                            typename TT::elem *__restrict__ x, float *__restrict__ ssq, int K, int N, int n_chunks,
                                                                            const int *__restrict__ counter = nullptr, int *__restrict__ epoch = nullptr,
-                                                                           int arrivals = 0) {
+                                                                           int arrivals = 0, const int *__restrict__ d_n = nullptr, int rows_cap = ROWS) {
     typedef typename TT::elem E;
     typedef typename TT::vec8 V8;
     constexpr int CSD = 2;
+    static_assert(!NV || (ROWS == 16 && !EARLY), "");
+    int nv = ROWS;
+    if constexpr (NV) nv = d_n[0];
     extern __shared__ __attribute__((aligned(1024))) char gemm_lds[];
     const int tid = threadIdx.x, w = __builtin_amdgcn_readfirstlane(tid >> 6), l = tid & 63, n = l & 15, g = l >> 4;
     E *xs = reinterpret_cast<E *>(gemm_lds) + (size_t)w * CSD * 16 * GEMM_KC;
@@ -618,19 +632,23 @@
             for (int j = 0; j < 2; j++)
                 asm volatile("global_load_dwordx4 %0, %1, %2 nt" : "=v"(dst[b][j]) : "v"(wlane), "s"(p + 1024 * (2 * b + j)) : "memory");
     };
-    auto issue_a = [&](int c, int buf) {
-#pragma unroll
-        for (int i = 0; i < AL; i++) {
+    auto issue_a = [&](int c, int buf, auto alc) {
+        constexpr int NA = decltype(alc)::value;
+#pragma unroll
+        for (int i = 0; i < NA; i++) {
             const int slot = l + 64 * i, row = slot >> 5, pos = slot & 31, unit = pos ^ (row & 15);
             const E *src = A + (size_t)row * K + (size_t)c * GEMM_KC + 8 * unit;
             E *dst_l = xs + (size_t)buf * 16 * GEMM_KC + (size_t)(64 * i) * 8;
-            __builtin_amdgcn_global_load_lds((gptr_t)src, (lptr_t)dst_l, 16, 0, 0);
-            asm volatile("" ::: "memory");
-        }
-    };
-    auto issue = [&](u32x4 (&dst)[4][2], int c, int buf) { issue_w(dst, c); issue_a(c, buf); };
-    auto phase = [&](u32x4 (&cur)[4][2], int c, int buf, bool more) {
-        if (more) { if constexpr (EARLY) asm volatile("s_waitcnt vmcnt(%0)" : : "n"(AL) : "memory"); else asm volatile("s_waitcnt vmcnt(%0)" : : "n"(8 + AL) : "memory"); }
+            if (!NV || i + 1 < NA || row < nv) {
+                __builtin_amdgcn_global_load_lds((gptr_t)src, (lptr_t)dst_l, 16, 0, 0);
+                asm volatile("" ::: "memory");
+            }
+        }
+    };
+    auto issue = [&](u32x4 (&dst)[4][2], int c, int buf, auto alc) { issue_w(dst, c); issue_a(c, buf, alc); };
+    auto phase = [&](u32x4 (&cur)[4][2], int c, int buf, bool more, bool w_first, auto alc) {
+        constexpr int NA = decltype(alc)::value;
+        if (more) { if (w_first) asm volatile("s_waitcnt vmcnt(%0)" : : "n"(NA) : "memory"); else asm volatile("s_waitcnt vmcnt(%0)" : : "n"(8 + NA) : "memory"); }
         else asm volatile("s_waitcnt vmcnt(0)" ::: "memory");
         const uint32_t xbase = lds_base + (uint32_t)buf * (16 * GEMM_KC * 2) + (uint32_t)n * (GEMM_KC * 2);
 #pragma unroll
@@ -658,29 +676,53 @@
         }
         __syncthreads();
         __builtin_amdgcn_fence(__ATOMIC_ACQUIRE, "agent");
-        if (mine > 0) issue_a(w, 0);
-        if (mine > 1) issue_a(w + GEMM_WAVES, 1);
-        if (mine > 0) phase(wr[0], w, 0, mine > 1);
-        if (mine > 1) phase(wr[1], w + GEMM_WAVES, 1, false);
+        if (mine > 0) issue_a(w, 0, GemmInt<AL>{});
+        if (mine > 1) issue_a(w + GEMM_WAVES, 1, GemmInt<AL>{});
+        if (mine > 0) phase(wr[0], w, 0, mine > 1, true, GemmInt<AL>{});
+        if (mine > 1) phase(wr[1], w + GEMM_WAVES, 1, false, true, GemmInt<AL>{});
         if (tid == 0) epoch[blockIdx.x] = my_epoch + 1;
     } else {
-        if (mine > 0) issue(wr[0], w, 0);
-        if (mine > 1) issue(wr[1], w + GEMM_WAVES, 1);
-        for (int i = 0; i < mine; i += 2) {
-            phase(wr[0], w + GEMM_WAVES * i, 0, i + 1 < mine);
-            if (i + 2 < mine) issue(wr[0], w + GEMM_WAVES * (i + 2), 0);
-            if (i + 1 < mine) {
-                phase(wr[1], w + GEMM_WAVES * (i + 1), 1, i + 2 < mine);
-                if (i + 3 < mine) issue(wr[1], w + GEMM_WAVES * (i + 3), 1);
-            }
-        }
+        auto stream = [&](bool w_ahead, auto alc) {
+            if (w_ahead) { if (mine > 0) issue_a(w, 0, alc); if (mine > 1) issue_a(w + GEMM_WAVES, 1, alc); }
+            else { if (mine > 0) issue(wr[0], w, 0, alc); if (mine > 1) issue(wr[1], w + GEMM_WAVES, 1, alc); }
+            for (int i = 0; i < mine; i += 2) {
+                phase(wr[0], w + GEMM_WAVES * i, 0, i + 1 < mine, w_ahead && i == 0, alc);
+                if (i + 2 < mine) issue(wr[0], w + GEMM_WAVES * (i + 2), 0, alc);
+                if (i + 1 < mine) {
+                    phase(wr[1], w + GEMM_WAVES * (i + 1), 1, i + 2 < mine, false, alc);
+                    if (i + 3 < mine) issue(wr[1], w + GEMM_WAVES * (i + 3), 1, alc);
+                }
+            }
+        };
+        if constexpr (NV) {
+            if (mine > 0) issue_w(wr[0], w);
+            if (mine > 1) issue_w(wr[1], w + GEMM_WAVES);
+            nv = nv < 0 ? 0 : (nv > rows_cap ? rows_cap : nv);
+#pragma unroll
+            for (int buf = 0; buf < CSD; buf++)
+#pragma unroll
+                for (int i = 0; i < 8; i++)
+                    if (((64 * i + l) >> 5) >= nv) *reinterpret_cast<u32x4 *>(xs + (size_t)buf * 16 * GEMM_KC + (size_t)(64 * i + l) * 8) = (u32x4){0u, 0u, 0u, 0u};
+            asm volatile("s_waitcnt lgkmcnt(0)" ::: "memory");
+            switch ((nv + 1) >> 1) {
+            case 0: stream(true, GemmInt<0>{}); break;
+            case 1: stream(true, GemmInt<1>{}); break;
+            case 2: stream(true, GemmInt<2>{}); break;
+            case 3: stream(true, GemmInt<3>{}); break;
+            case 4: stream(true, GemmInt<4>{}); break;
+            case 5: stream(true, GemmInt<5>{}); break;
+            case 6: stream(true, GemmInt<6>{}); break;
+            case 7: stream(true, GemmInt<7>{}); break;
+            default: stream(true, GemmInt<8>{}); break;
+            }
+        } else stream(false, GemmInt<AL>{});
     }
     __syncthreads();
     float *ex = reinterpret_cast<float *>(gemm_lds);
 #pragma unroll
     for (int r = 0; r < 4; r++) ex[(w * 16 + 4 * g + r) * 16 + n] = acc[r];
     __syncthreads();
-    if (tid < 16 * ROWS) {
+    if (tid < 16 * nv) {
         const int row = tid >> 4, col = tid & 15;
         float sum = 0.f;
 #pragma unroll
@@ -744,7 +786,7 @@
 
 template <typename TT, int RT, int DEPTH, int CG, bool NORM = false, int AR = 16>
 static hipError_t qkv_rope_launch(hipStream_t st, const void *A, const void *W, int K, int tiles, const float *cs, const int *d_L, const int *d_n, void *q, void *k, void *v,
-                                  int H, int Hkv, long long max_len, int v_t, NormArgs na = NormArgs{nullptr, nullptr, 0, 0.f, 0.f}) {
+                                  int H, int Hkv, long long max_len, int v_t, NormArgs na = NormArgs{nullptr, nullptr, 0, 0.f, 0.f}, int rows_cap = 16) {
     constexpr int lds_a = (DEPTH + 1) * 16 * RT * GEMM_KC * 2, lds_e = 2 * 16 * RT * 16 * CG * 4, lds = lds_a > lds_e ? lds_a : lds_e;
     if constexpr (lds > 60000) {
         static unsigned long long done = 0ull;
@@ -752,13 +794,13 @@
         if (attr != hipSuccess) return attr;
     }
     hipLaunchKernelGGL((k_gemm_qkv_rope<TT, RT, DEPTH, CG, NORM, AR>), dim3(tiles), dim3(64 * GEMM_WAVES), lds, st, (const typename TT::elem *)A, (const typename TT::elem *)W, K, K / GEMM_KC,
-                       cs, d_L, d_n, (typename TT::elem *)q, (typename TT::elem *)k, (typename TT::elem *)v, H, Hkv, max_len, na, v_t);
+                       cs, d_L, d_n, (typename TT::elem *)q, (typename TT::elem *)k, (typename TT::elem *)v, H, Hkv, max_len, na, v_t, rows_cap);
     return hipSuccess;
 }
 
 template <typename TT, int RT, int DEPTH, bool NORM = false, int AR = 16>
 static hipError_t pairs_silu_launch(hipStream_t st, int grid, const void *A, const void *W, void *out, int K, int inter, int n_pairs,
-                                    NormArgs na = NormArgs{nullptr, nullptr, 0, 0.f, 0.f}) {
+                                    NormArgs na = NormArgs{nullptr, nullptr, 0, 0.f, 0.f}, const int *d_n = nullptr, int rows_cap = 16) {
     constexpr int lds_a = (DEPTH + 1) * 16 * RT * GEMM_KC * 2, lds_e = 4 * 16 * RT * 16 * 4, lds = lds_a > lds_e ? lds_a : lds_e;
     if constexpr (lds > 60000) {
         static unsigned long long done = 0ull;
@@ -766,7 +808,7 @@
         if (attr != hipSuccess) return attr;
     }
     hipLaunchKernelGGL((k_gemm_pairs_silu<TT, RT, DEPTH, NORM, AR>), dim3(grid), dim3(64 * GEMM_WAVES), lds, st, (const typename TT::elem *)A, (const typename TT::elem *)W,
-                       (typename TT::elem *)out, K, inter, K / GEMM_KC, n_pairs, na);
+                       (typename TT::elem *)out, K, inter, K / GEMM_KC, n_pairs, na, d_n, rows_cap);
     return hipSuccess;
 }
 
@@ -817,8 +859,8 @@
     return SAMD_OK;
 }
 
-int samd_gemm_pairs_silu_norm(const void *d_x, const float *d_ssq, const void *d_norm_weight, float eps, const void *d_Wg, int32_t rows_pad, int32_t inter, int32_t K,
-                              void *d_out, int32_t dtype, void *stream) {
+static int gemm_pairs_silu_norm_impl(const void *d_x, const float *d_ssq, const void *d_norm_weight, float eps, const void *d_Wg, int32_t rows_pad, int32_t inter, int32_t K,
+                                     void *d_out, int32_t dtype, void *stream, const int32_t *d_n) {
     if (!d_x || !d_ssq || !d_norm_weight || !d_Wg || !d_out || (rows_pad != 16 && rows_pad != 8) || inter < 16 || inter % 16 != 0 || K < GEMM_KC || K % GEMM_KC != 0 ||
         K / 16 > 32 * NORM_NS || (dtype != SAMD_F16 && dtype != SAMD_BF16)) {
         samd_set_error("samd_gemm_pairs_silu_norm: unsupported shape (8 or 16 rows, inter %% 16 == 0, K %% 256 == 0, K <= 8192, f16/bf16) or null pointer"); return SAMD_E_INVALID;
@@ -829,7 +871,10 @@
     while ((n_pairs + grid - 1) / grid > 4) grid += n_cu;
     const NormArgs na{d_ssq, d_norm_weight, K / 16, 1.f / (float)K, eps};
     hipStream_t st = (hipStream_t)stream;
-    const hipError_t e = rows_pad == 8
+    const hipError_t e = d_n
+        ? (dtype == SAMD_F16 ? pairs_silu_launch<GF16, 1, 3, true, 0>(st, grid, d_x, d_Wg, d_out, K, inter, n_pairs, na, d_n, rows_pad)
+                             : pairs_silu_launch<GBF16, 1, 3, true, 0>(st, grid, d_x, d_Wg, d_out, K, inter, n_pairs, na, d_n, rows_pad))
+        : rows_pad == 8
         ? (dtype == SAMD_F16 ? pairs_silu_launch<GF16, 1, 3, true, 8>(st, grid, d_x, d_Wg, d_out, K, inter, n_pairs, na)
                              : pairs_silu_launch<GBF16, 1, 3, true, 8>(st, grid, d_x, d_Wg, d_out, K, inter, n_pairs, na))
         : (dtype == SAMD_F16 ? pairs_silu_launch<GF16, 1, 3, true>(st, grid, d_x, d_Wg, d_out, K, inter, n_pairs, na)
@@ -839,22 +884,45 @@
     return SAMD_OK;
 }
 
-int samd_gemm_cs_residual(const void *d_A, const void *d_Wg, int32_t rows_pad, int32_t N, int32_t K, void *d_x, float *d_ssq, int32_t dtype, void *stream) {
+int samd_gemm_pairs_silu_norm(const void *d_x, const float *d_ssq, const void *d_norm_weight, float eps, const void *d_Wg, int32_t rows_pad, int32_t inter, int32_t K,
+                              void *d_out, int32_t dtype, void *stream) {
+    return gemm_pairs_silu_norm_impl(d_x, d_ssq, d_norm_weight, eps, d_Wg, rows_pad, inter, K, d_out, dtype, stream, nullptr);
+}
+
+int samd_gemm_pairs_silu_norm_n(const void *d_x, const float *d_ssq, const void *d_norm_weight, float eps, const void *d_Wg, int32_t rows_pad, int32_t inter, int32_t K,
+                                const int32_t *d_n, void *d_out, int32_t dtype, void *stream) {
+    if (!d_n) { samd_set_error("samd_gemm_pairs_silu_norm_n: null d_n"); return SAMD_E_INVALID; }
+    return gemm_pairs_silu_norm_impl(d_x, d_ssq, d_norm_weight, eps, d_Wg, rows_pad, inter, K, d_out, dtype, stream, d_n);
+}
+
+static int gemm_cs_residual_impl(const void *d_A, const void *d_Wg, int32_t rows_pad, int32_t N, int32_t K, void *d_x, float *d_ssq, int32_t dtype, void *stream,
+                                 const int32_t *d_n) {
     if (!d_A || !d_Wg || !d_x || !d_ssq || (rows_pad != 16 && rows_pad != 8) || N < 16 || N % 16 != 0 || K < GEMM_KC || K % GEMM_KC != 0 || (dtype != SAMD_F16 && dtype != SAMD_BF16)) {
         samd_set_error("samd_gemm_cs_residual: unsupported shape (8 or 16 rows, N %% 16 == 0, K %% 256 == 0, f16/bf16) or null pointer"); return SAMD_E_INVALID;
     }
     constexpr int lds = GEMM_WAVES * 2 * 16 * GEMM_KC * 2;
     hipStream_t st = (hipStream_t)stream;
     hipError_t e = hipSuccess;
-#define GO(TT, ROWS, ET) do { static unsigned long long done = 0ull; \
-        e = samd_reserve_lds((const void *)k_gemm_cs_residual<TT, ROWS>, lds, &done); \
-        if (e == hipSuccess) hipLaunchKernelGGL((k_gemm_cs_residual<TT, ROWS>), dim3(N / 16), dim3(64 * GEMM_WAVES), lds, st, (const ET *)d_A, (const ET *)d_Wg, (ET *)d_x, d_ssq, K, N, K / GEMM_KC, (const int *)nullptr, (int *)nullptr, 0); } while (0)
-    if (dtype == SAMD_F16) { if (rows_pad == 8) GO(GF16, 8, _Float16); else GO(GF16, 16, _Float16); }
-    else { if (rows_pad == 8) GO(GBF16, 8, __bf16); else GO(GBF16, 16, __bf16); }
+#define GO(TT, ROWS, NV, ET) do { static unsigned long long done = 0ull; \
+        e = samd_reserve_lds((const void *)k_gemm_cs_residual<TT, ROWS, false, NV>, lds, &done); \
+        if (e == hipSuccess) hipLaunchKernelGGL((k_gemm_cs_residual<TT, ROWS, false, NV>), dim3(N / 16), dim3(64 * GEMM_WAVES), lds, st, (const ET *)d_A, (const ET *)d_Wg, (ET *)d_x, d_ssq, K, N, K / GEMM_KC, (const int *)nullptr, (int *)nullptr, 0, (const int *)d_n, (int)rows_pad); } while (0)
+    if (d_n) { if (dtype == SAMD_F16) GO(GF16, 16, true, _Float16); else GO(GBF16, 16, true, __bf16); }
+    else if (dtype == SAMD_F16) { if (rows_pad == 8) GO(GF16, 8, false, _Float16); else GO(GF16, 16, false, _Float16); }
+    else { if (rows_pad == 8) GO(GBF16, 8, false, __bf16); else GO(GBF16, 16, false, __bf16); }
 #undef GO
     if (e != hipSuccess) { samd_set_error("samd_gemm_cs_residual: %s", hipGetErrorString(e)); return SAMD_E_HIP; }
     LAUNCHCHK();
     return SAMD_OK;
+}
+
+int samd_gemm_cs_residual(const void *d_A, const void *d_Wg, int32_t rows_pad, int32_t N, int32_t K, void *d_x, float *d_ssq, int32_t dtype, void *stream) {
+    return gemm_cs_residual_impl(d_A, d_Wg, rows_pad, N, K, d_x, d_ssq, dtype, stream, nullptr);
+}
+
+int samd_gemm_cs_residual_n(const void *d_A, const void *d_Wg, int32_t rows_pad, int32_t N, int32_t K, const int32_t *d_n, void *d_x, float *d_ssq, int32_t dtype,
+                            void *stream) {
+    if (!d_n) { samd_set_error("samd_gemm_cs_residual_n: null d_n"); return SAMD_E_INVALID; }
+    return gemm_cs_residual_impl(d_A, d_Wg, rows_pad, N, K, d_x, d_ssq, dtype, stream, d_n);
 }
 
 int samd_gemm_cs_residual_early(const void *d_A, const void *d_Wg, int32_t N, int32_t K, void *d_x, float *d_ssq, int32_t dtype, const int32_t *d_counter,
@@ -962,7 +1030,7 @@
 
 static int gemm_qkv_rope_norm_impl(const void *d_x, const float *d_ssq, const void *d_norm_weight, float eps, const void *d_W64, int32_t rows_pad, int32_t K,
                                    const float *d_cs, const int32_t *d_cache_length, const int32_t *d_n, void *d_q_out, void *d_k_cache, void *d_v_cache,
-                                   int32_t n_heads, int32_t n_kv_heads, int32_t head_dim, int64_t max_len, int32_t dtype, void *stream, int v_t) {
+                                   int32_t n_heads, int32_t n_kv_heads, int32_t head_dim, int64_t max_len, int32_t dtype, void *stream, int v_t, int rows_n) {
     if (!d_x || !d_ssq || !d_norm_weight || !d_W64 || !d_cs || !d_cache_length || !d_n || !d_q_out || !d_k_cache || !d_v_cache || head_dim != 128 || n_heads < 1 ||
         n_kv_heads < 1 || (rows_pad != 16 && rows_pad != 8) || K < GEMM_KC || K % GEMM_KC != 0 || K / 16 > 32 * NORM_NS || (dtype != SAMD_F16 && dtype != SAMD_BF16)) {
         samd_set_error("samd_gemm_qkv_rope_norm: unsupported shape (8 or 16 rows, head_dim 128, K %% 256 == 0, K <= 8192, f16/bf16) or null pointer"); return SAMD_E_INVALID;
@@ -972,8 +1040,11 @@
     const NormArgs na{d_ssq, d_norm_weight, K / 16, 1.f / (float)K, eps};
     hipStream_t st = (hipStream_t)stream;
     hipError_t e = hipSuccess;
-#define GO(TT, CG, AR) e = qkv_rope_launch<TT, 1, 4, CG, true, AR>(st, d_x, d_W64, K, tiles, d_cs, d_cache_length, d_n, d_q_out, d_k_cache, d_v_cache, n_heads, n_kv_heads, (long long)max_len, v_t, na)
-    if (rows_pad == 8) {
+#define GO(TT, CG, AR) e = qkv_rope_launch<TT, 1, 4, CG, true, AR>(st, d_x, d_W64, K, tiles, d_cs, d_cache_length, d_n, d_q_out, d_k_cache, d_v_cache, n_heads, n_kv_heads, (long long)max_len, v_t, na, rows_pad)
+    if (rows_n) {
+        if (groups == 3) { if (dtype == SAMD_F16) GO(GF16, 3, 0); else GO(GBF16, 3, 0); }
+        else { if (dtype == SAMD_F16) GO(GF16, 4, 0); else GO(GBF16, 4, 0); }
+    } else if (rows_pad == 8) {
         if (groups == 3) { if (dtype == SAMD_F16) GO(GF16, 3, 8); else GO(GBF16, 3, 8); }
         else { if (dtype == SAMD_F16) GO(GF16, 4, 8); else GO(GBF16, 4, 8); }
     } else {
@@ -990,14 +1061,28 @@
                             const float *d_cs, const int32_t *d_cache_length, const int32_t *d_n, void *d_q_out, void *d_k_cache, void *d_v_cache,
                             int32_t n_heads, int32_t n_kv_heads, int32_t head_dim, int64_t max_len, int32_t dtype, void *stream) {
     return gemm_qkv_rope_norm_impl(d_x, d_ssq, d_norm_weight, eps, d_W64, rows_pad, K, d_cs, d_cache_length, d_n, d_q_out, d_k_cache, d_v_cache, n_heads, n_kv_heads, head_dim,
-                                   max_len, dtype, stream, 0);
+                                   max_len, dtype, stream, 0, 0);
 }
 
 int samd_gemm_qkv_rope_norm_vt(const void *d_x, const float *d_ssq, const void *d_norm_weight, float eps, const void *d_W64, int32_t rows_pad, int32_t K,
                                const float *d_cs, const int32_t *d_cache_length, const int32_t *d_n, void *d_q_out, void *d_k_cache, void *d_vt_cache,
                                int32_t n_heads, int32_t n_kv_heads, int32_t head_dim, int64_t max_len, int32_t dtype, void *stream) {
     return gemm_qkv_rope_norm_impl(d_x, d_ssq, d_norm_weight, eps, d_W64, rows_pad, K, d_cs, d_cache_length, d_n, d_q_out, d_k_cache, d_vt_cache, n_heads, n_kv_heads, head_dim,
-                                   max_len, dtype, stream, 1);
+                                   max_len, dtype, stream, 1, 0);
+}
+
+int samd_gemm_qkv_rope_norm_n(const void *d_x, const float *d_ssq, const void *d_norm_weight, float eps, const void *d_W64, int32_t rows_pad, int32_t K,
+                              const float *d_cs, const int32_t *d_cache_length, const int32_t *d_n, void *d_q_out, void *d_k_cache, void *d_v_cache,
+                              int32_t n_heads, int32_t n_kv_heads, int32_t head_dim, int64_t max_len, int32_t dtype, void *stream) {
+    return gemm_qkv_rope_norm_impl(d_x, d_ssq, d_norm_weight, eps, d_W64, rows_pad, K, d_cs, d_cache_length, d_n, d_q_out, d_k_cache, d_v_cache, n_heads, n_kv_heads, head_dim,
+                                   max_len, dtype, stream, 0, 1);
+}
+
+int samd_gemm_qkv_rope_norm_n_vt(const void *d_x, const float *d_ssq, const void *d_norm_weight, float eps, const void *d_W64, int32_t rows_pad, int32_t K,
+                                 const float *d_cs, const int32_t *d_cache_length, const int32_t *d_n, void *d_q_out, void *d_k_cache, void *d_vt_cache,
+                                 int32_t n_heads, int32_t n_kv_heads, int32_t head_dim, int64_t max_len, int32_t dtype, void *stream) {
+    return gemm_qkv_rope_norm_impl(d_x, d_ssq, d_norm_weight, eps, d_W64, rows_pad, K, d_cs, d_cache_length, d_n, d_q_out, d_k_cache, d_vt_cache, n_heads, n_kv_heads, head_dim,
+                                   max_len, dtype, stream, 1, 1);
 }
 
 int samd_gemm_skinny(const void *d_A, const void *d_W, int32_t rows_pad, int32_t N, int32_t K, int32_t splits, float *d_partial,
diff --git a/sam-decoding_amd/samd_hip/__init__.py b/sam-decoding_amd/samd_hip/__init__.py
--- a/sam-decoding_amd/samd_hip/__init__.py
+++ b/sam-decoding_amd/samd_hip/__init__.py
@@ -105,6 +105,10 @@
     "samd_gemm_qkv_rope_norm_vt": (C.c_int, [_VP, _VP, _VP, C.c_float, _VP, _I32, _I32, _VP, _VP, _VP, _VP, _VP, _VP, _I32, _I32, _I32, _I64, _I32, _VP]),
     "samd_gemm_pairs_silu_norm": (C.c_int, [_VP, _VP, _VP, C.c_float, _VP, _I32, _I32, _I32, _VP, _I32, _VP]),
     "samd_gemm_cs_residual": (C.c_int, [_VP, _VP, _I32, _I32, _I32, _VP, _VP, _I32, _VP]),
+    "samd_gemm_qkv_rope_norm_n": (C.c_int, [_VP, _VP, _VP, C.c_float, _VP, _I32, _I32, _VP, _VP, _VP, _VP, _VP, _VP, _I32, _I32, _I32, _I64, _I32, _VP]),
+    "samd_gemm_qkv_rope_norm_n_vt": (C.c_int, [_VP, _VP, _VP, C.c_float, _VP, _I32, _I32, _VP, _VP, _VP, _VP, _VP, _VP, _I32, _I32, _I32, _I64, _I32, _VP]),
+    "samd_gemm_pairs_silu_norm_n": (C.c_int, [_VP, _VP, _VP, C.c_float, _VP, _I32, _I32, _I32, _VP, _VP, _I32, _VP]),
+    "samd_gemm_cs_residual_n": (C.c_int, [_VP, _VP, _I32, _I32, _I32, _VP, _VP, _VP, _I32, _VP]),
     "samd_gemm_cs_residual_early": (C.c_int, [_VP, _VP, _I32, _I32, _VP, _VP, _I32, _VP, _VP, _I32, _VP]),
     "samd_tree_attention_signal": (C.c_int, [_VP, _VP, _VP, _VP, _I32, _I32, _I32, _I32, _I32, _I64, _VP, _VP, _VP, _F32, _VP, _I64, _VP, _VP]),
     "samd_session_report_target": (C.c_int, [_VP, C.POINTER(_VP)]),
diff --git a/sam-decoding_amd/samd_hip/llama.py b/sam-decoding_amd/samd_hip/llama.py
--- a/sam-decoding_amd/samd_hip/llama.py
+++ b/sam-decoding_amd/samd_hip/llama.py
@@ -150,6 +150,7 @@
         if quant or moe:
             self.native_gemm_max_rows = TILE_ROWS
         self.layer_hook = None
+        self.rows_n = os.environ.get("SAMD_ROWS_N", "1") != "0"
         self.warm_kb = int(os.environ.get("SAMD_L2_WARM_KB", 0))
         self.warm_delay = int(os.environ.get("SAMD_L2_WARM_DELAY", 0))
         self.warm_where = int(os.environ.get("SAMD_L2_WARM_WHERE", 0))
@@ -787,6 +788,8 @@
             check(L.samd_rope_rows(_ptr(d_relpos), _ptr(d_L), _ptr(self.cos), _ptr(self.sin), _ptr(b["cs"]), R, s.head_dim, self.rope_rows, st))
         attn2d = b["attn"].view(b["attn"].shape[0], -1)
         qkv_launch = L.samd_gemm_qkv_rope_norm_vt if self.v_transposed else L.samd_gemm_qkv_rope_norm
+        if self.rows_n:
+            qkv_launch = L.samd_gemm_qkv_rope_norm_n_vt if self.v_transposed else L.samd_gemm_qkv_rope_norm_n
         attn_launch = L.samd_tree_attention_vt if self.v_transposed else L.samd_tree_attention_warm
         for li, (w, wp) in enumerate(zip(self.w["layers"], self.wp["layers"])):
             if self.layer_hook is not None:
@@ -796,6 +799,12 @@
             check(attn_launch(_ptr(b["q"]), _ptr(self.kv[li, 0]), _ptr(self.kv[li, 1]), _ptr(b["attn"]), dt, R, s.heads,
                               s.kv_heads, s.head_dim, self.max_len, _ptr(d_mask), _ptr(d_L), _ptr(d_n), self.scale,
                               _ptr(b["ws"]), b["ws_bytes"], None, st))
+            if self.rows_n:
+                check(L.samd_gemm_cs_residual_n(_ptr(attn2d), _ptr(wp["wo_g"]), rows_cs, s.hidden, attn2d.shape[1], _ptr(d_n), _ptr(x), _ptr(ssq), dt, st))
+                check(L.samd_gemm_pairs_silu_norm_n(_ptr(x), _ptr(ssq), _ptr(w["ln2"]), s.eps, _ptr(wp["wgu"]), rows_a, s.inter, s.hidden, _ptr(d_n),
+                                                    _ptr(b["act"]), dt, st))
+                check(L.samd_gemm_cs_residual_n(_ptr(b["act"]), _ptr(wp["wdown_g"]), rows_cs, s.hidden, s.inter, _ptr(d_n), _ptr(x), _ptr(ssq), dt, st))
+                continue
             check(L.samd_gemm_cs_residual(_ptr(attn2d), _ptr(wp["wo_g"]), rows_cs, s.hidden, attn2d.shape[1], _ptr(x), _ptr(ssq), dt, st))
             check(L.samd_gemm_pairs_silu_norm(_ptr(x), _ptr(ssq), _ptr(w["ln2"]), s.eps, _ptr(wp["wgu"]), rows_a, s.inter, s.hidden, _ptr(b["act"]), dt, st))
             check(L.samd_gemm_cs_residual(_ptr(b["act"]), _ptr(wp["wdown_g"]), rows_cs, s.hidden, s.inter, _ptr(x), _ptr(ssq), dt, st))
```

New measurement: 820.0 (median of 6 runs). Within noise of the previous version (+0.7%).
